# NeuroDiffGym/neurodiffeq

Measured on AMD Instinct MI355X. Metric: collocation-points/sec (residual+bwd), 2D Laplace 65k pts, 1/2/4/8 GPU, higher is better.
Workload: dtype f32; 1 GPU; C2: Solver2D 2D Laplace, DirichletBVP2D, FCNN(2-32-32-1, tanh), Generator2D 256x256 = 65536 noisy-grid points per GPU per step, Adam(1e-3), run_train_epoch() with n_batches_train=1, n_batches_valid=0; points_per_gpu=65536, global_batch=65536, parallelism=dp1 (shard-by-batch, one all-reduce of [P+1] fp32 per step), allreduce=none (single process), inputs=pre-sampled in the reference's RNG order, resident in HBM

## Files before the change

### include/ndq.h

```cpp
#ifndef NDQ_H
#define NDQ_H
#include <stddef.h>
#ifdef __cplusplus
extern "C" {
#endif

#define NDQ_EUNSUPPORTED (-1)
#define NDQ_EINVAL (-2)

#define NDQ_ACT_TANH 0
#define NDQ_ACT_SIN 1
#define NDQ_ACT_SIGMOID 2
#define NDQ_ACT_SWISH 3
#define NDQ_ACT_APTX 4
#define NDQ_ACT_ELU 5
#define NDQ_ACT_SOFTPLUS 6
#define NDQ_ACT_GELU 7

#define NDQ_MAX_HIDDEN 512
typedef struct ndq_mlp_desc {
  int d;
  int first;
  int mask2;
  int hidden;
  int layers;
  int act;
  int n_out;
  int lap;
  int skip;
  int mask3;
  int actp;
  int widths;
  int mono;
  int mask4;
} ndq_mlp_desc;

typedef struct ndq_mlp_kernels {
  ndq_mlp_desc desc;
  int n_streams, n_params;
  int bwd_waves;
  int lds_bytes;
  int (*fwd)(const float* coords, int ldc, int n, const float* params, float* jets, int ldj, void* stream);
  int (*bwd)(const float* coords, int ldc, int n, const float* params, const float* gbar, int ldj, float* partials,
             int blocks, void* stream);
} ndq_mlp_kernels;
int ndq_mlp_register(const ndq_mlp_kernels* kernels);

int ndq_mlp_supported(const ndq_mlp_desc* desc);
int ndq_mlp_num_streams(const ndq_mlp_desc* desc);
int ndq_mlp_num_params(const ndq_mlp_desc* desc);
int ndq_mlp_bwd_blocks(const ndq_mlp_desc* desc, int n);

int ndq_mlp_jet_fwd(const ndq_mlp_desc* desc, const float* coords, int ldc, int n, const float* params, float* jets,
                    int ldj, void* stream);

int ndq_mlp_jet_bwd(const ndq_mlp_desc* desc, const float* coords, int ldc, int n, const float* params,
                    const float* gbar, int ldj, float* partials, void* stream);

int ndq_reduce_partials(const float* partials, int nparts, int len, float* out, int accumulate, float scale,
                        void* stream);

int ndq_adam_step(float* params, const float* grad, float* exp_avg, float* exp_avg_sq, int len, float lr, float beta1,
                  float beta2, float eps, float weight_decay, int step, void* stream);

int ndq_reduce_grad_loss(const float* partials, int nparts, int len, float* out, int accumulate,
                         const float* loss_partials, int n_loss_parts, float* loss_out, float loss_scale, void* stream);

int ndq_epoch_tail(float* params, const float* grad, float* exp_avg, float* exp_avg_sq, int len, float lr, float beta1,
                   float beta2, float eps, float weight_decay, int step, const float* loss_slots, int n_batches,
                   float* loss_hist, int hist_index, float* best_loss, int parity, float* best_flat, int write_scalars,
                   void* stream);

#define NDQ_SAMPLE_UNIFORM 0
#define NDQ_SAMPLE_GRID 1
#define NDQ_SAMPLE_SPHERICAL 2
typedef struct ndq_sampler_desc {
  int kind;
  int d;
  int n[3];
  float lo[3], hi[3];
  float noise_std[3];
  int radial;
} ndq_sampler_desc;
int ndq_sample(const ndq_sampler_desc* desc, unsigned long long seed, unsigned long long draw, unsigned stream_id,
               float* coords, int ldc, void* stream);

#define NDQ_TABLE_MAX_AXES 6
#define NDQ_AXIS_NORMAL 0
#define NDQ_AXIS_CHEB2_NOISY 1
typedef struct ndq_table_sampler_desc {
  int d;
  int n[NDQ_TABLE_MAX_AXES];
  int law[NDQ_TABLE_MAX_AXES];
  int abs_value;
  const float* mean[NDQ_TABLE_MAX_AXES];
  const float* std[NDQ_TABLE_MAX_AXES];
  float lo[NDQ_TABLE_MAX_AXES], hi[NDQ_TABLE_MAX_AXES];
} ndq_table_sampler_desc;
int ndq_sample_table(const ndq_table_sampler_desc* desc, unsigned long long seed, unsigned long long draw,
                     unsigned stream_id, float* coords , int ldc, void* stream);

#define NDQ_PLAN_MAX_LEAVES 8
#define NDQ_LEAF_SIMPLE 0
#define NDQ_LEAF_TABLE 1
#define NDQ_LEAF_DATA 2
#define NDQ_SEG_LEAF 0
#define NDQ_SEG_ENSEMBLE 1
#define NDQ_SEG_MESH 2
typedef struct ndq_plan_leaf {
  int kind;
  int row0;
  int rows;
  int n;
  union {
    ndq_sampler_desc simple;
    ndq_table_sampler_desc table;
    const float* data[NDQ_TABLE_MAX_AXES];
  } u;
} ndq_plan_leaf;
typedef struct ndq_plan_segment {
  int mode;
  int first, count;
  int offset, size;
} ndq_plan_segment;
typedef struct ndq_plan_sampler_desc {
  int d;
  int n_leaves;
  int n_segments;
  int reserved;
  ndq_plan_leaf leaf[NDQ_PLAN_MAX_LEAVES];
  ndq_plan_segment seg[NDQ_PLAN_MAX_LEAVES];
} ndq_plan_sampler_desc;
int ndq_sample_plan(const ndq_plan_sampler_desc* desc, unsigned long long seed, unsigned long long draw,
                    unsigned stream_id, float* coords , int ldc, void* stream);

#define NDQ_INDEX_NONE 0
#define NDQ_INDEX_PERMUTE 1
#define NDQ_INDEX_REPLACE 2
typedef struct ndq_plan_index_desc {
  int mode;
  int m;
  int batch;
  int reserved;
} ndq_plan_index_desc;
int ndq_sample_plan_indexed(const ndq_plan_sampler_desc* desc, const ndq_plan_index_desc* index, unsigned long long seed,
                            unsigned long long draw, unsigned stream_id, float* coords , int ldc, void* stream);

typedef int (*ndq_fused_launch_fn)(const float* coords, int ldc, int n, const float* params, float* partials,
                                   float* loss_partials, float* funcs, float* resid, int ldj, float seed, int train,
                                   void* stream);

typedef int (*ndq_allreduce_fn)(const void* sendbuf, void* recvbuf, size_t count, int dtype, int op, void* comm,
                                void* stream);

typedef struct ndq_fused_step {
  ndq_fused_launch_fn launch;
  int n, ldc, ldj, blocks, n_params;
  float seed;
  float* params;
  float* partials;
  float* loss_partials;
  float* grad;
  float* loss_slot;
  float* adam_m;
  float* adam_v;
  float lr, beta1, beta2, eps, weight_decay;
  float* loss_hist;
  float* best_loss;
  float* best_flat;
  ndq_allreduce_fn allreduce;
  void* comm;
  const struct ndq_sampler_desc* next_sampler;
  unsigned long long next_seed, next_draw;
  unsigned next_stream;
  float* next_coords;
  int next_ldc;
} ndq_fused_step;
int ndq_fused_step_run(const ndq_fused_step* s, const float* coords, int adam_step, int hist_index, int parity,
                       void* stream);

typedef int (*ndq_fused_launch_multi_fn)(const float* coords, int ldc, int n, const float* const* params,
                                         float* const* partials, float* loss_partials, float* funcs, float* resid,
                                         int ldj, float seed, int train, void* stream);
int ndq_fused_multi_step_run(const ndq_fused_step* steps, int n_nets, ndq_fused_launch_multi_fn launch,
                             const float* coords, int adam_step, int hist_index, int parity, void* stream);

typedef int (*ndq_fused_launch_tv_fn)(const float* coords, int ldc, int n, const float* const* params,
                                      float* const* partials, float* loss_partials, float seed,
                                      const float* valid_coords, int valid_ldc, int valid_n,
                                      float* valid_loss_partials, const void* pull, void* stream);
typedef int (*ndq_fused_launch_loop_fn)(const float* coords, int ldc, int n, float seed, const float* vcoords, int vldc,
                                        int vn, const void* loop, void* stream);
typedef struct ndq_fused_fit {
  ndq_fused_launch_tv_fn launch;
  int n_nets;
  ndq_fused_step net[4];
  const float* valid_coords;
  int valid_n, valid_ldc, valid_blocks;
  float valid_scale;
  float* valid_loss_partials;
  float* valid_hist;
  int track_best;
  int pull_ok;
  float* alt_params[4];
  float* alt_m[4];
  float* alt_v[4];
  float* alt_partials[4];
  float* alt_loss_partials;
  float* alt_valid_loss_partials;
  ndq_fused_launch_loop_fn launch_loop;
  int loop_ok;
} ndq_fused_fit;
int ndq_fused_fit_run(const ndq_fused_fit* f, int n_epochs, const float* const* train_coords, int adam_step,
                      int hist_index, int valid_index, int parity, void* stream);

typedef int (*ndq_pointwise_fn)(const float* coords, int ldc, int n, const float* const* jets,
                                float* const* gbar, int ldj, float* funcs, float* resid, float* loss_partials,
                                float seed_scale, void* stream);
typedef int (*ndq_pw_blocks_fn)(int n);
typedef void (*ndq_bind_theta_fn)(const float* theta, float* theta_partials);

typedef struct ndq64_mlp_kernels {
  ndq_mlp_desc desc;
  int n_streams, n_params;
  int bwd_waves;
  int lds_bytes;
  int (*fwd)(const double* coords, int ldc, int n, const double* params, double* jets, int ldj, void* stream);
  int (*bwd)(const double* coords, int ldc, int n, const double* params, const double* gbar, int ldj, double* partials,
             int blocks, void* stream);
} ndq64_mlp_kernels;
int ndq64_mlp_register(const ndq64_mlp_kernels* kernels);
int ndq64_mlp_supported(const ndq_mlp_desc* desc);
int ndq64_mlp_num_streams(const ndq_mlp_desc* desc);
int ndq64_mlp_num_params(const ndq_mlp_desc* desc);
int ndq64_mlp_bwd_blocks(const ndq_mlp_desc* desc, int n);
int ndq64_mlp_jet_fwd(const ndq_mlp_desc* desc, const double* coords, int ldc, int n, const double* params, double* jets,
                      int ldj, void* stream);
int ndq64_mlp_jet_bwd(const ndq_mlp_desc* desc, const double* coords, int ldc, int n, const double* params,
                      const double* gbar, int ldj, double* partials, void* stream);
int ndq64_reduce_partials(const double* partials, int nparts, int len, double* out, int accumulate, double scale,
                          void* stream);
int ndq64_adam_step(double* params, const double* grad, double* exp_avg, double* exp_avg_sq, int len, double lr,
                    double beta1, double beta2, double eps, double weight_decay, int step, void* stream);

int ndq64_epoch_tail(double* params, const double* grad, double* exp_avg, double* exp_avg_sq, int len, double lr,
                     double beta1, double beta2, double eps, double weight_decay, int step, const double* loss_slots,
                     int n_batches, double* loss_hist, int hist_index, double* best_loss, int parity, double* best_flat,
                     int write_scalars, void* stream);

typedef int (*ndq64_fused_launch_multi_fn)(const double* coords, int ldc, int n, const double* const* params,
                                           double* const* partials, double* loss_partials, double* funcs, double* resid,
                                           int ldj, double seed, int train, void* stream);
typedef struct ndq64_fused_step {
  int n, ldc, ldj, blocks, n_params;
  double seed;
  double* params;
  double* partials;
  double* loss_partials;
  double* grad;
  double* loss_slot;
  double* adam_m;
  double* adam_v;
  double lr, beta1, beta2, eps, weight_decay;
  double* loss_hist;
  double* best_loss;
  double* best_flat;
} ndq64_fused_step;
int ndq64_fused_step_bytes(void);
int ndq64_reduce_tail(const ndq64_fused_step* steps, int n_nets, int adam_step, int hist_index, int parity, void* stream);
int ndq64_fused_step_run(const ndq64_fused_step* steps, int n_nets, ndq64_fused_launch_multi_fn launch,
                         const double* coords, int adam_step, int hist_index, int parity, void* stream);

int ndq_oneshot_create(int rank, int world_size, int max_len, void** ctx, unsigned char* handle64);
int ndq_oneshot_connect(void* ctx, const unsigned char* handles);
int ndq_oneshot_allreduce(const void* send, void* recv, size_t count, int dtype, int op, void* ctx, void* stream);
int ndq_oneshot_status(void* ctx);
int ndq_oneshot_destroy(void* ctx);

#ifdef __cplusplus
}
#endif
#endif
```

### neurodiffeq_amd/_build.py

```python
import os

from . import _hipcc

HERE = os.path.dirname(os.path.abspath(__file__))
CSRC = os.path.join(HERE, "csrc")
LIB = os.path.join(HERE, "libndq.so")
SOURCES = [os.path.join(CSRC, "ndq_api.hip")]
HEADERS = [os.path.join(CSRC, h) for h in ("ndq_mlp.h", "ndq_tail.h", "ndq_launch.h", "ndq_wide.h", "ndq_deep.h", "ndq_sample.h", "ndq_oneshot.h")] + \
    [os.path.join(HERE, "..", "include", "ndq.h"), os.path.join(HERE, "_hipcc.py")]
LIB64 = os.path.join(HERE, "libndq64.so")
SOURCES64 = [os.path.join(CSRC, "ndq_api64.hip")]
FLAGS = []
_EXTRA = os.environ.get("NDQ_LIB_FLAGS", "").split()
if _EXTRA:
    import hashlib
    LIB = os.path.join(HERE, "libndq_" + hashlib.sha1(" ".join(_EXTRA).encode()).hexdigest()[:8] + ".so")
    FLAGS = FLAGS + _EXTRA


def is_stale():
    if not os.path.exists(LIB):
        return True
    t = os.path.getmtime(LIB)
    return any(os.path.exists(p) and os.path.getmtime(p) > t for p in SOURCES + HEADERS)


def build_lib(force=False, verbose=False):
    if not force and not is_stale():
        return LIB
    _hipcc.compile_shared(SOURCES, LIB, FLAGS, verbose=verbose)
    return LIB


def is_stale64():
    if not os.path.exists(LIB64):
        return True
    t = os.path.getmtime(LIB64)
    return any(os.path.exists(p) and os.path.getmtime(p) > t for p in SOURCES64 + HEADERS)


def build_lib64(force=False, verbose=False):
    if not force and not is_stale64():
        return LIB64
    _hipcc.compile_shared(SOURCES64, LIB64, [], verbose=verbose)
    return LIB64


if __name__ == "__main__":
    print(build_lib(force=True, verbose=True))
```

### neurodiffeq_amd/_lib.py

```python
import ctypes
import os

from . import _build

NDQ_ACT_TANH, NDQ_ACT_SIN, NDQ_ACT_SIGMOID, NDQ_ACT_SWISH, NDQ_ACT_APTX = 0, 1, 2, 3, 4
NDQ_ACT_ELU, NDQ_ACT_SOFTPLUS, NDQ_ACT_GELU = 5, 6, 7


class MlpDesc(ctypes.Structure):
    _fields_ = [("d", ctypes.c_int), ("first", ctypes.c_int), ("mask2", ctypes.c_int), ("hidden", ctypes.c_int),
                ("layers", ctypes.c_int), ("act", ctypes.c_int), ("n_out", ctypes.c_int), ("lap", ctypes.c_int),
                ("skip", ctypes.c_int), ("mask3", ctypes.c_int), ("actp", ctypes.c_int), ("widths", ctypes.c_int), ("mono", ctypes.c_int),
                ("mask4", ctypes.c_int)]

    def key(self):
        return (self.d, self.first, self.mask2, self.hidden, self.layers, self.act, self.n_out, self.lap, self.skip,
                self.mask3, self.actp, self.widths, self.mono, self.mask4)


NDQ_SAMPLE_UNIFORM, NDQ_SAMPLE_GRID, NDQ_SAMPLE_SPHERICAL = 0, 1, 2


class SamplerDesc(ctypes.Structure):
    _fields_ = [("kind", ctypes.c_int), ("d", ctypes.c_int), ("n", ctypes.c_int * 3), ("lo", ctypes.c_float * 3),
                ("hi", ctypes.c_float * 3), ("noise_std", ctypes.c_float * 3), ("radial", ctypes.c_int)]


NDQ_TABLE_MAX_AXES = 6
NDQ_AXIS_NORMAL, NDQ_AXIS_CHEB2_NOISY = 0, 1


class TableSamplerDesc(ctypes.Structure):
    _fields_ = [("d", ctypes.c_int), ("n", ctypes.c_int * 6), ("law", ctypes.c_int * 6), ("abs_value", ctypes.c_int),
                ("mean", ctypes.c_void_p * 6), ("std", ctypes.c_void_p * 6), ("lo", ctypes.c_float * 6),
                ("hi", ctypes.c_float * 6)]


NDQ_PLAN_MAX_LEAVES = 8
NDQ_LEAF_SIMPLE, NDQ_LEAF_TABLE, NDQ_LEAF_DATA = 0, 1, 2
NDQ_SEG_LEAF, NDQ_SEG_ENSEMBLE, NDQ_SEG_MESH = 0, 1, 2
NDQ_INDEX_NONE, NDQ_INDEX_PERMUTE, NDQ_INDEX_REPLACE = 0, 1, 2


class _PlanLaw(ctypes.Union):
    _fields_ = [("simple", SamplerDesc), ("table", TableSamplerDesc), ("data", ctypes.c_void_p * 6)]


class PlanLeaf(ctypes.Structure):
    _fields_ = [("kind", ctypes.c_int), ("row0", ctypes.c_int), ("rows", ctypes.c_int), ("n", ctypes.c_int), ("u", _PlanLaw)]


class PlanSegment(ctypes.Structure):
    _fields_ = [("mode", ctypes.c_int), ("first", ctypes.c_int), ("count", ctypes.c_int), ("offset", ctypes.c_int),
                ("size", ctypes.c_int)]


class PlanSamplerDesc(ctypes.Structure):
    _fields_ = [("d", ctypes.c_int), ("n_leaves", ctypes.c_int), ("n_segments", ctypes.c_int), ("reserved", ctypes.c_int),
                ("leaf", PlanLeaf * 8), ("seg", PlanSegment * 8)]


class PlanIndexDesc(ctypes.Structure):
    _fields_ = [("mode", ctypes.c_int), ("m", ctypes.c_int), ("batch", ctypes.c_int), ("reserved", ctypes.c_int)]


FUSED_LAUNCH_FN = ctypes.CFUNCTYPE(ctypes.c_int, ctypes.c_void_p, ctypes.c_int, ctypes.c_int, ctypes.c_void_p,
                                   ctypes.c_void_p, ctypes.c_void_p, ctypes.c_void_p, ctypes.c_void_p, ctypes.c_int,
                                   ctypes.c_float, ctypes.c_int, ctypes.c_void_p)


class FusedStep(ctypes.Structure):
    _fields_ = [("launch", ctypes.c_void_p),
                ("n", ctypes.c_int), ("ldc", ctypes.c_int), ("ldj", ctypes.c_int), ("blocks", ctypes.c_int),
                ("n_params", ctypes.c_int), ("seed", ctypes.c_float),
                ("params", ctypes.c_void_p), ("partials", ctypes.c_void_p), ("loss_partials", ctypes.c_void_p),
                ("grad", ctypes.c_void_p), ("loss_slot", ctypes.c_void_p), ("adam_m", ctypes.c_void_p),
                ("adam_v", ctypes.c_void_p),
                ("lr", ctypes.c_float), ("beta1", ctypes.c_float), ("beta2", ctypes.c_float), ("eps", ctypes.c_float),
                ("weight_decay", ctypes.c_float),
                ("loss_hist", ctypes.c_void_p), ("best_loss", ctypes.c_void_p), ("best_flat", ctypes.c_void_p),
                ("allreduce", ctypes.c_void_p), ("comm", ctypes.c_void_p),
                ("next_sampler", ctypes.c_void_p), ("next_seed", ctypes.c_ulonglong), ("next_draw", ctypes.c_ulonglong),
                ("next_stream", ctypes.c_uint), ("next_coords", ctypes.c_void_p), ("next_ldc", ctypes.c_int)]


class FusedStep64(ctypes.Structure):
    _fields_ = [("n", ctypes.c_int), ("ldc", ctypes.c_int), ("ldj", ctypes.c_int), ("blocks", ctypes.c_int),
                ("n_params", ctypes.c_int), ("seed", ctypes.c_double),
                ("params", ctypes.c_void_p), ("partials", ctypes.c_void_p), ("loss_partials", ctypes.c_void_p),
                ("grad", ctypes.c_void_p), ("loss_slot", ctypes.c_void_p), ("adam_m", ctypes.c_void_p),
                ("adam_v", ctypes.c_void_p),
                ("lr", ctypes.c_double), ("beta1", ctypes.c_double), ("beta2", ctypes.c_double), ("eps", ctypes.c_double),
                ("weight_decay", ctypes.c_double),
                ("loss_hist", ctypes.c_void_p), ("best_loss", ctypes.c_void_p), ("best_flat", ctypes.c_void_p)]


class FusedFit(ctypes.Structure):
    _fields_ = [("launch", ctypes.c_void_p), ("n_nets", ctypes.c_int), ("net", FusedStep * 4),
                ("valid_coords", ctypes.c_void_p), ("valid_n", ctypes.c_int), ("valid_ldc", ctypes.c_int),
                ("valid_blocks", ctypes.c_int), ("valid_scale", ctypes.c_float),
                ("valid_loss_partials", ctypes.c_void_p), ("valid_hist", ctypes.c_void_p), ("track_best", ctypes.c_int),
                ("pull_ok", ctypes.c_int), ("alt_params", ctypes.c_void_p * 4), ("alt_m", ctypes.c_void_p * 4),
                ("alt_v", ctypes.c_void_p * 4), ("alt_partials", ctypes.c_void_p * 4),
                ("alt_loss_partials", ctypes.c_void_p), ("alt_valid_loss_partials", ctypes.c_void_p),
                ("launch_loop", ctypes.c_void_p), ("loop_ok", ctypes.c_int)]


class NdqError(RuntimeError):
    pass


_LIB = None


def lib():
    global _LIB
    if _LIB is not None:
        return _LIB
    path = _build.LIB
    if _build.is_stale():
        try:
            _build.build_lib()
        except Exception as e:
            if not os.path.exists(path):
                raise NdqError(f"libndq.so is missing and could not be built: {e}") from e
    L = ctypes.CDLL(path)
    vp, ci, cf = ctypes.c_void_p, ctypes.c_int, ctypes.c_float
    dp = ctypes.POINTER(MlpDesc)
    L.ndq_mlp_supported.argtypes = [dp]
    L.ndq_mlp_num_streams.argtypes = [dp]
    L.ndq_mlp_num_params.argtypes = [dp]
    L.ndq_mlp_bwd_blocks.argtypes = [dp, ci]
    L.ndq_mlp_jet_fwd.argtypes = [dp, vp, ci, ci, vp, vp, ci, vp]
    L.ndq_mlp_jet_bwd.argtypes = [dp, vp, ci, ci, vp, vp, ci, vp, vp]
    L.ndq_reduce_partials.argtypes = [vp, ci, ci, vp, ci, cf, vp]
    L.ndq_adam_step.argtypes = [vp, vp, vp, vp, ci, cf, cf, cf, cf, cf, ci, vp]
    L.ndq_reduce_grad_loss.argtypes = [vp, ci, ci, vp, ci, vp, ci, vp, cf, vp]
    L.ndq_epoch_tail.argtypes = [vp, vp, vp, vp, ci, cf, cf, cf, cf, cf, ci, vp, ci, vp, ci, vp, ci, vp, ci, vp]
    L.ndq_fused_step_run.argtypes = [ctypes.POINTER(FusedStep), vp, ci, ci, ci, vp]
    L.ndq_fused_multi_step_run.argtypes = [ctypes.POINTER(FusedStep), ci, vp, vp, ci, ci, ci, vp]
    L.ndq_fused_fit_run.argtypes = [ctypes.POINTER(FusedFit), ci, vp, ci, ci, ci, ci, vp]
    L.ndq_mlp_register.argtypes = [vp]
    L.ndq_sample.argtypes = [ctypes.POINTER(SamplerDesc), ctypes.c_ulonglong, ctypes.c_ulonglong, ctypes.c_uint, vp, ci, vp]
    L.ndq_sample_table.argtypes = [ctypes.POINTER(TableSamplerDesc), ctypes.c_ulonglong, ctypes.c_ulonglong, ctypes.c_uint, vp, ci,
                                   vp]
    L.ndq_sample_plan.argtypes = [ctypes.POINTER(PlanSamplerDesc), ctypes.c_ulonglong, ctypes.c_ulonglong, ctypes.c_uint, vp, ci, vp]
    L.ndq_sample_plan_indexed.argtypes = [ctypes.POINTER(PlanSamplerDesc), ctypes.POINTER(PlanIndexDesc), ctypes.c_ulonglong,
                                          ctypes.c_ulonglong, ctypes.c_uint, vp, ci, vp]
    L.ndq_oneshot_create.argtypes = [ci, ci, ci, ctypes.POINTER(vp), ctypes.c_char_p]
    L.ndq_oneshot_connect.argtypes = [vp, ctypes.c_char_p]
    L.ndq_oneshot_allreduce.argtypes = [vp, vp, ctypes.c_size_t, ci, ci, vp, vp]
    L.ndq_oneshot_status.argtypes = [vp]
    L.ndq_oneshot_destroy.argtypes = [vp]
    for name in ("ndq_mlp_supported", "ndq_mlp_num_streams", "ndq_mlp_num_params", "ndq_mlp_bwd_blocks",
                 "ndq_mlp_jet_fwd", "ndq_mlp_jet_bwd", "ndq_reduce_partials", "ndq_adam_step", "ndq_reduce_grad_loss",
                 "ndq_epoch_tail", "ndq_fused_step_run", "ndq_sample", "ndq_sample_table", "ndq_sample_plan", "ndq_sample_plan_indexed", "ndq_mlp_register",
                 "ndq_fused_multi_step_run", "ndq_fused_fit_run", "ndq_oneshot_create", "ndq_oneshot_connect",
                 "ndq_oneshot_allreduce", "ndq_oneshot_status",
                 "ndq_oneshot_destroy"):
        getattr(L, name).restype = ci
    _LIB = L
    return L


_LIB64 = None


def lib64():
    global _LIB64
    if _LIB64 is not None:
        return _LIB64
    if _build.is_stale64():
        try:
            _build.build_lib64()
        except Exception as e:
            if not os.path.exists(_build.LIB64):
                raise NdqError(f"libndq64.so is missing and could not be built: {e}") from e
    L = ctypes.CDLL(_build.LIB64)
    vp, ci = ctypes.c_void_p, ctypes.c_int
    dp = ctypes.POINTER(MlpDesc)
    L.ndq64_mlp_supported.argtypes = [dp]
    L.ndq64_mlp_num_streams.argtypes = [dp]
    L.ndq64_mlp_num_params.argtypes = [dp]
    L.ndq64_mlp_bwd_blocks.argtypes = [dp, ci]
    L.ndq64_mlp_jet_fwd.argtypes = [dp, vp, ci, ci, vp, vp, ci, vp]
    L.ndq64_mlp_jet_bwd.argtypes = [dp, vp, ci, ci, vp, vp, ci, vp, vp]
    L.ndq64_reduce_partials.argtypes = [vp, ci, ci, vp, ci, ctypes.c_double, vp]
    L.ndq64_mlp_register.argtypes = [vp]
    cd = ctypes.c_double
    L.ndq64_adam_step.argtypes = [vp, vp, vp, vp, ci, cd, cd, cd, cd, cd, ci, vp]
    L.ndq64_epoch_tail.argtypes = [vp, vp, vp, vp, ci, cd, cd, cd, cd, cd, ci, vp, ci, vp, ci, vp, ci, vp, ci, vp]
    L.ndq64_fused_step_bytes.argtypes = []
    L.ndq64_reduce_tail.argtypes = [ctypes.POINTER(FusedStep64), ci, ci, ci, ci, vp]
    L.ndq64_fused_step_run.argtypes = [ctypes.POINTER(FusedStep64), ci, vp, vp, ci, ci, ci, vp]
    for name in EXPORTS64:
        getattr(L, name).restype = ci
    _LIB64 = L
    return L


EXPORTS64 = ("ndq64_mlp_register", "ndq64_mlp_supported", "ndq64_mlp_num_streams", "ndq64_mlp_num_params",
             "ndq64_mlp_bwd_blocks", "ndq64_mlp_jet_fwd", "ndq64_mlp_jet_bwd", "ndq64_reduce_partials", "ndq64_adam_step",
             "ndq64_epoch_tail", "ndq64_fused_step_bytes", "ndq64_reduce_tail", "ndq64_fused_step_run")

EXPORTS = ("ndq_mlp_supported", "ndq_mlp_num_streams", "ndq_mlp_num_params", "ndq_mlp_bwd_blocks", "ndq_mlp_jet_fwd",
           "ndq_mlp_jet_bwd", "ndq_reduce_partials", "ndq_adam_step", "ndq_reduce_grad_loss", "ndq_epoch_tail",
           "ndq_fused_step_run", "ndq_sample", "ndq_sample_table", "ndq_sample_plan", "ndq_sample_plan_indexed", "ndq_mlp_register",
           "ndq_fused_multi_step_run", "ndq_fused_fit_run", "ndq_oneshot_create", "ndq_oneshot_connect", "ndq_oneshot_allreduce", "ndq_oneshot_status",
           "ndq_oneshot_destroy")


def check(rc, what):
    if rc != 0:
        raise NdqError(f"{what} failed with code {rc}" + (" (no kernel for this descriptor)" if rc == -1 else ""))
```

### neurodiffeq_amd/csrc/ndq_api.hip

```cpp
#include <cstdlib>
#include <vector>
#include "ndq_launch.h"
#include "ndq_sample.h"
#include "ndq_oneshot.h"
#include "ndq_tail.h"

extern "C" int ndq_oneshot_allreduce(const void* send, void* recv, size_t count, int dtype, int op, void* comm, void* stream);

namespace ndq {

#ifndef NDQ_CFG_TABLE
#define NDQ_CFG_TABLE(X)      \
  X(1, 0, 0, 2, 2, ACT_SIN, 1, 0)   \
  X(1, 1, 0, 2, 2, ACT_SIN, 1, 0)   \
  X(1, 1, 1, 2, 2, ACT_SIN, 1, 0)   \
  X(1, 0, 0, 2, 2, ACT_TANH, 1, 0)  \
  X(1, 1, 0, 2, 2, ACT_TANH, 1, 0)  \
  X(1, 1, 1, 2, 2, ACT_TANH, 1, 0)  \
  X(2, 0, 0, 2, 2, ACT_TANH, 1, 0)  \
  X(2, 1, 0, 2, 2, ACT_TANH, 1, 0)  \
  X(2, 1, 1, 2, 2, ACT_TANH, 1, 0)  \
  X(2, 1, 5, 2, 2, ACT_TANH, 1, 0)  \
  X(2, 1, 7, 2, 2, ACT_TANH, 1, 0)  \
  X(2, 0, 0, 4, 3, ACT_TANH, 1, 0)  \
  X(2, 1, 0, 4, 3, ACT_TANH, 1, 0)  \
  X(2, 1, 1, 4, 3, ACT_TANH, 1, 0)  \
  X(2, 1, 5, 4, 3, ACT_TANH, 1, 0)  \
  X(1, 0, 0, 2, 2, ACT_TANH, 25, 0) \
  X(1, 1, 1, 2, 2, ACT_TANH, 25, 0) \
  X(2, 1, 5, 2, 2, ACT_TANH, 3, 0)  \
  X(2, 1, 5, 2, 2, ACT_TANH, 1, 1)  \
  X(2, 1, 5, 4, 3, ACT_TANH, 1, 1)  \
  X(3, 0, 0, 2, 2, ACT_TANH, 1, 0)  \
  X(3, 1, 0, 2, 2, ACT_TANH, 1, 0)  \
  X(3, 1, 1, 2, 2, ACT_TANH, 1, 0)  \
  X(3, 1, 41, 2, 2, ACT_TANH, 1, 0) \
  X(3, 1, 41, 2, 2, ACT_TANH, 1, 1) \
  X(3, 1, 63, 2, 2, ACT_TANH, 1, 0)  \
  X(1, 0, 0, 2, 2, ACT_SIGMOID, 1, 0) \
  X(1, 1, 0, 2, 2, ACT_SIGMOID, 1, 0) \
  X(1, 1, 1, 2, 2, ACT_SIGMOID, 1, 0) \
  X(2, 0, 0, 2, 2, ACT_SIGMOID, 1, 0) \
  X(2, 1, 0, 2, 2, ACT_SIGMOID, 1, 0) \
  X(2, 1, 1, 2, 2, ACT_SIGMOID, 1, 0) \
  X(2, 1, 5, 2, 2, ACT_SIGMOID, 1, 0) \
  X(2, 1, 7, 2, 2, ACT_SIGMOID, 1, 0) \
  X(2, 1, 5, 2, 2, ACT_SIGMOID, 1, 1) \
  X(1, 0, 0, 2, 2, ACT_SWISH, 1, 0) \
  X(1, 1, 0, 2, 2, ACT_SWISH, 1, 0) \
  X(1, 1, 1, 2, 2, ACT_SWISH, 1, 0) \
  X(2, 0, 0, 2, 2, ACT_SWISH, 1, 0) \
  X(2, 1, 0, 2, 2, ACT_SWISH, 1, 0) \
  X(2, 1, 1, 2, 2, ACT_SWISH, 1, 0) \
  X(2, 1, 5, 2, 2, ACT_SWISH, 1, 0) \
  X(2, 1, 7, 2, 2, ACT_SWISH, 1, 0) \
  X(2, 1, 5, 2, 2, ACT_SWISH, 1, 1)
#endif

#define NDQ_ENTRY(D, F, M, NB, L, A, O, LP) make_kernels<Cfg<D, F, M, NB, L, A, O, LP>>(),

static const ndq_mlp_kernels kTable[] = {NDQ_CFG_TABLE(NDQ_ENTRY)};
static std::vector<const ndq_mlp_kernels*> g_registered;

static const ndq_mlp_kernels* find(const ndq_mlp_desc* d) {
  if (!d || d->hidden < 1 || d->hidden > NDQ_MAX_HIDDEN) return nullptr;
  for (const ndq_mlp_kernels& e : kTable)
    if (same_desc(e.desc, *d)) return &e;
  for (const ndq_mlp_kernels* e : g_registered)
    if (same_desc(e->desc, *d)) return e;
  return nullptr;
}

__global__ __launch_bounds__(256) void reduce_partials_kernel(const float* __restrict__ part, int nparts, int len,
                                                              float* __restrict__ out, int accumulate, float scale) {
  const int i = blockIdx.x * blockDim.x + threadIdx.x;
  if (i >= len) return;
  double s0 = 0., s1 = 0., s2 = 0., s3 = 0.;
  int r = 0;
#pragma unroll 4
  for (; r + 3 < nparts; r += 4) {
    s0 += (double)part[(size_t)r * len + i];
    s1 += (double)part[(size_t)(r + 1) * len + i];
    s2 += (double)part[(size_t)(r + 2) * len + i];
    s3 += (double)part[(size_t)(r + 3) * len + i];
  }
  for (; r < nparts; ++r) s0 += (double)part[(size_t)r * len + i];
  const float s = (float)(((s0 + s1) + (s2 + s3)) * (double)scale);
  out[i] = accumulate ? out[i] + s : s;
}

struct Reduce2Args {
  const float* part; int nparts, len; float* out; int accumulate;
  const float* lpart; int nlparts; float* lout; float lscale;
};

struct ColumnRows {
  float v[16];
  __device__ __forceinline__ void issue(const float* __restrict__ part, int nparts, int len, int col, int rg) {
    const int cc = col < len ? col : len - 1;
#pragma unroll
    for (int j = 0; j < 16; ++j) {
      const int r = rg + 16 * j;
      v[j] = part[(size_t)(r < nparts ? r : nparts - 1) * len + cc];
    }
  }
  __device__ __forceinline__ float finish(const float* __restrict__ part, int nparts, int len, int col, int rg) const {
    float x[16];
#pragma unroll
    for (int j = 0; j < 16; ++j) x[j] = v[j];
    asm volatile("" : "+v"(x[0]), "+v"(x[1]), "+v"(x[2]), "+v"(x[3]), "+v"(x[4]), "+v"(x[5]), "+v"(x[6]), "+v"(x[7]), "+v"(x[8]),
                      "+v"(x[9]), "+v"(x[10]), "+v"(x[11]), "+v"(x[12]), "+v"(x[13]), "+v"(x[14]), "+v"(x[15]));
#pragma unroll
    for (int j = 0; j < 16; ++j) x[j] = (rg + 16 * j < nparts && col < len) ? x[j] : 0.f;
    float s0 = 0.f, s1 = 0.f, s2 = 0.f, s3 = 0.f;
#pragma unroll
    for (int it = 0; it < 4; ++it) {
      if (rg + 64 * it + 48 < nparts) { s0 += x[4 * it]; s1 += x[4 * it + 1]; s2 += x[4 * it + 2]; s3 += x[4 * it + 3]; }
      else { s0 += x[4 * it]; s0 += x[4 * it + 1]; s0 += x[4 * it + 2]; s0 += x[4 * it + 3]; }
    }
    if (nparts > 256 && col < len) {
      int r = rg + 256;
      for (; r + 48 < nparts; r += 64) {
        s0 += part[(size_t)r * len + col];
        s1 += part[(size_t)(r + 16) * len + col];
        s2 += part[(size_t)(r + 32) * len + col];
        s3 += part[(size_t)(r + 48) * len + col];
      }
      for (; r < nparts; r += 16) s0 += part[(size_t)r * len + col];
    }
    return (s0 + s1) + (s2 + s3);
  }
};

__device__ __forceinline__ float column_sum_1024(const float* __restrict__ part, int nparts, int len, int col, int rg,
                                                 float* sm ) {
  ColumnRows rows;
  rows.issue(part, nparts, len, col, rg);
  sm[rg * 64 + (threadIdx.x & 63)] = rows.finish(part, nparts, len, col, rg);
  __syncthreads();
  float s = 0.f;
  if (rg == 0) {
#pragma unroll
    for (int g = 0; g < 16; ++g) s += sm[g * 64 + (threadIdx.x & 63)];
  }
  return s;
}

__device__ __forceinline__ float block_sum_1024(const float* __restrict__ v, int n, float* sm16) {
  float x = 0.f;
  for (int r = threadIdx.x; r < n; r += 1024) x += v[r];
  for (int off = 32; off > 0; off >>= 1) x += __shfl_down(x, off);
  if ((threadIdx.x & 63) == 0) sm16[threadIdx.x >> 6] = x;
  __syncthreads();
  float s = 0.f;
  if (threadIdx.x == 0)
    for (int w = 0; w < 16; ++w) s += sm16[w];
  return s;
}

__global__ __launch_bounds__(1024) void reduce_grad_loss_kernel(Reduce2Args a) {
  __shared__ float sm[16 * 64];
  if (blockIdx.x + 1 < gridDim.x) {
    const int c = threadIdx.x & 63, rg = threadIdx.x >> 6;
    const int i = blockIdx.x * 64 + c;
    const float s = column_sum_1024(a.part, a.nparts, a.len, i, rg, sm);
    if (rg == 0 && i < a.len) a.out[i] = a.accumulate ? a.out[i] + s : s;
  } else {
    const float s = block_sum_1024(a.lpart, a.nlparts, sm);
    if (threadIdx.x == 0) *a.lout = s * a.lscale;
  }
}

using TailArgs = ndq::TailArgsT<float>;

struct ValidArgs {
  const float* part; int nparts; float scale; float* hist; int index;
  int best_on_valid;
};
struct ReduceTailArgs {
  Reduce2Args r;
  TailArgs t;
  int tail_blocks;
  ndq::SampleArgs smp;
  ValidArgs v;
};
#ifndef NDQ_TAIL_COLS
#define NDQ_TAIL_COLS 64
#endif
template <int TC>
__device__ __forceinline__ void reduce_tail_body(const ReduceTailArgs& a) {
  constexpr int TT = TC * 16, WAVES = TT / 64;
  __shared__ float sm[16 * TC];
  __shared__ float smw[16];
  __shared__ float smv[16];
  const int tid = threadIdx.x, c = tid % TC, rg = tid / TC, lane = tid & 63, wave = tid >> 6;
  const int i = blockIdx.x * TC + c;
  const bool col = i < a.r.len;
  const bool has_valid = a.v.part != nullptr;
  const bool has_train = a.r.nparts > 0;
  ColumnRows rows;
  if (has_train) rows.issue(a.r.part, a.r.nparts, a.r.len, i, rg);
  const float lp0 = tid < a.r.nlparts ? a.r.lpart[tid] : 0.f;
  const float vp0 = has_valid && tid < a.v.nparts ? a.v.part[tid] : 0.f;
  const bool upd = (rg == 0) && col;
  const float* p_in = a.t.p_in ? a.t.p_in : a.t.p;
  const float* m_in = a.t.m_in ? a.t.m_in : a.t.m;
  const float* v_in = a.t.v_in ? a.t.v_in : a.t.v;
  float pi = 0.f, m0 = 0.f, v0 = 0.f;
  if (upd) {
    pi = p_in[i];
    if (has_train || a.t.p_in) { m0 = m_in[i]; v0 = v_in[i]; }
  }
  const float best = a.t.best_loss[a.t.parity];
  float lp = lp0, vp = vp0;
  for (int r = tid + TT; r < a.r.nlparts; r += TT) lp += a.r.lpart[r];
  if (has_valid)
    for (int r = tid + TT; r < a.v.nparts; r += TT) vp += a.v.part[r];
  const float colsum = has_train ? rows.finish(a.r.part, a.r.nparts, a.r.len, i, rg) : 0.f;
  for (int off = 32; off > 0; off >>= 1) lp += __shfl_down(lp, off);
  if (has_valid)
    for (int off = 32; off > 0; off >>= 1) vp += __shfl_down(vp, off);
  if (lane == 0) { smw[wave] = lp; smv[wave] = vp; }
  sm[rg * TC + c] = colsum;
  __syncthreads();
  float loss = 0.f, vloss = 0.f;
#pragma unroll
  for (int w = 0; w < WAVES; ++w) loss += smw[w];
  loss *= a.r.lscale;
  if (has_valid) {
#pragma unroll
    for (int w = 0; w < WAVES; ++w) vloss += smv[w];
    vloss *= a.v.scale;
  }
  const bool on_valid = has_valid && a.v.best_on_valid != 0;
  const float cmp = on_valid ? vloss : loss;
  const bool better = (a.t.best_flat != nullptr) && (on_valid || has_train) && (cmp < best);
  if (upd) {
    if (better) a.t.best_flat[i] = pi;
    if (has_train) {
      float g = 0.f;
#pragma unroll
      for (int k = 0; k < 16; ++k) g += sm[k * TC + c];
      a.r.out[i] = g;
      float pn, mi, vi;
      ndq::adam_value(a.t.adam, pi, g, m0, v0, pn, mi, vi);
      a.t.m[i] = mi;
      a.t.v[i] = vi;
      a.t.p[i] = pn;
    } else if (a.t.p_in) {
      a.t.p[i] = pi; a.t.m[i] = m0; a.t.v[i] = v0;
    }
  }
  if (blockIdx.x == 0 && tid == 0 && a.t.write_scalars) {
    if (has_train) {
      *a.r.lout = loss;
      a.t.loss_hist[a.t.hist_index] = loss;
    }
    if (has_valid) a.v.hist[a.v.index] = vloss;
    a.t.best_loss[a.t.parity ^ 1] = better ? cmp : best;
  }
}
__global__ __launch_bounds__(1024) void reduce_tail_kernel(ReduceTailArgs a) {
  if ((int)blockIdx.x >= a.tail_blocks) {
    ndq::sample_point_store(a.smp, ((int)blockIdx.x - a.tail_blocks) * 1024 + (int)threadIdx.x);
    return;
  }
  reduce_tail_body<64>(a);
}

__global__ __launch_bounds__(1024) void reduce_tail_dp_kernel(ReduceTailArgs a, ndq::OneshotDev c, unsigned step) {
  __shared__ float sm[16 * 64];
  __shared__ float smw[16];
  __shared__ float sloss;
  __shared__ int timed_out;
  if (threadIdx.x == 0) timed_out = 0;
  const int tid = threadIdx.x, col = tid & 63, rg = tid >> 6, blk = blockIdx.x;
  const int i = blk * 64 + col;
  const bool incol = i < a.r.len;
  ColumnRows rows;
  rows.issue(a.r.part, a.r.nparts, a.r.len, i, rg);
  const float lp0 = tid < a.r.nlparts ? a.r.lpart[tid] : 0.f;
  const bool upd = (rg == 0) && incol;
  float pi = 0.f, m0 = 0.f, v0 = 0.f;
  if (upd) { pi = a.t.p[i]; m0 = a.t.m[i]; v0 = a.t.v[i]; }
  const float best = a.t.best_loss[a.t.parity];
  float lp = lp0;
  for (int r = tid + 1024; r < a.r.nlparts; r += 1024) lp += a.r.lpart[r];
  const float colsum = rows.finish(a.r.part, a.r.nparts, a.r.len, i, rg);
  for (int off = 32; off > 0; off >>= 1) lp += __shfl_down(lp, off);
  if (col == 0) smw[rg] = lp;
  sm[rg * 64 + col] = colsum;
  __syncthreads();
  const int parity = step & 1u;
  const size_t slot = ((size_t)parity * c.world + c.rank) * c.max_len + (size_t)blk * 65;
  if (rg == 0) {
    float g = 0.f;
#pragma unroll
    for (int k = 0; k < 16; ++k) g += sm[k * 64 + col];
    for (int q = 0; q < c.world; ++q)
      __hip_atomic_store(c.inbox[q] + slot + col, incol ? g : 0.f, __ATOMIC_RELAXED, __HIP_MEMORY_SCOPE_SYSTEM);
    if (col == 0) {
      float loss = 0.f;
#pragma unroll
      for (int w = 0; w < 16; ++w) loss += smw[w];
      loss *= a.r.lscale;
      for (int q = 0; q < c.world; ++q)
        __hip_atomic_store(c.inbox[q] + slot + 64, loss, __ATOMIC_RELAXED, __HIP_MEMORY_SCOPE_SYSTEM);
    }
  }
  __threadfence_system();
  __syncthreads();
  if (tid < c.world) {
    unsigned* f = c.flags[tid] + ((size_t)parity * c.world + c.rank) * c.max_blocks + blk;
    __hip_atomic_store(f, step, __ATOMIC_RELEASE, __HIP_MEMORY_SCOPE_SYSTEM);
    const unsigned* mine = c.flags[c.rank] + ((size_t)parity * c.world + tid) * c.max_blocks + blk;
    if (!ndq::oneshot_wait(mine, step, c.spin_limit, c.status)) timed_out = 1;
  }
  __syncthreads();
  const bool bad = timed_out != 0;
  const float* inbox = c.inbox[c.rank] + (size_t)parity * c.world * c.max_len + (size_t)blk * 65;
  if (tid == 0) {
    float loss = 0.f;
    for (int q = 0; q < c.world; ++q)
      loss += __hip_atomic_load(inbox + (size_t)q * c.max_len + 64, __ATOMIC_RELAXED, __HIP_MEMORY_SCOPE_SYSTEM);
    sloss = bad ? __builtin_nanf("") : loss;
  }
  __syncthreads();
  const float loss = sloss;
  const bool better = (a.t.best_flat != nullptr) && (loss < best);
  if (upd && !bad) {
    float g = 0.f;
    for (int q = 0; q < c.world; ++q)
      g += __hip_atomic_load(inbox + (size_t)q * c.max_len + col, __ATOMIC_RELAXED, __HIP_MEMORY_SCOPE_SYSTEM);
    a.r.out[i] = g;
    if (better) a.t.best_flat[i] = pi;
    float pn, mi, vi;
    ndq::adam_value(a.t.adam, pi, g, m0, v0, pn, mi, vi);
    a.t.m[i] = mi;
    a.t.v[i] = vi;
    a.t.p[i] = pn;
  }
  if (blk == 0 && tid == 0 && a.t.write_scalars) {
    *a.r.lout = loss;
    a.t.loss_hist[a.t.hist_index] = loss;
    a.t.best_loss[a.t.parity ^ 1] = better ? loss : best;
  }
}

struct ReduceTailMultiArgs {
  ReduceTailArgs net[4];
};
template <int TC>
__global__ __launch_bounds__(TC * 16) void reduce_tail_multi_kernel(ReduceTailMultiArgs a) {
  const ReduceTailArgs& mine = a.net[blockIdx.y];
  if ((int)blockIdx.x * TC >= mine.r.len) return;
  reduce_tail_body<TC>(mine);
}
static int launch_tail_multi(ReduceTailMultiArgs& a, int max_params, int n_nets, int max_lparts, void* stream) {
  hipStream_t st = static_cast<hipStream_t>(stream);
  for (int k = n_nets; k < 4; ++k) a.net[k] = a.net[0];
  if (NDQ_TAIL_COLS < 64 && max_lparts <= NDQ_TAIL_COLS * 16)
    hipLaunchKernelGGL(reduce_tail_multi_kernel<NDQ_TAIL_COLS>, dim3((max_params + NDQ_TAIL_COLS - 1) / NDQ_TAIL_COLS, n_nets),
                       dim3(NDQ_TAIL_COLS * 16), 0, st, a);
  else
    hipLaunchKernelGGL(reduce_tail_multi_kernel<64>, dim3((max_params + 63) / 64, n_nets), dim3(1024), 0, st, a);
  return (int)hipGetLastError();
}

}

using namespace ndq;

extern "C" {

int ndq_mlp_supported(const ndq_mlp_desc* desc) { return find(desc) ? 1 : 0; }

int ndq_mlp_register(const ndq_mlp_kernels* k) {
  if (!k || !k->fwd || !k->bwd || k->desc.hidden < 1 || k->desc.hidden > NDQ_MAX_HIDDEN || k->n_streams < 1 || k->n_params < 1 || k->bwd_waves < 1 ||
      k->lds_bytes > 160 * 1024)
    return NDQ_EINVAL;
  if (!find(&k->desc)) g_registered.push_back(k);
  return 0;
}

int ndq_mlp_num_streams(const ndq_mlp_desc* desc) {
  const ndq_mlp_kernels* e = find(desc);
  return e ? e->n_streams : NDQ_EUNSUPPORTED;
}

int ndq_mlp_num_params(const ndq_mlp_desc* desc) {
  const ndq_mlp_kernels* e = find(desc);
  return e ? e->n_params : NDQ_EUNSUPPORTED;
}

int ndq_mlp_bwd_blocks(const ndq_mlp_desc* desc, int n) {
  const ndq_mlp_kernels* e = find(desc);
  if (!e) return NDQ_EUNSUPPORTED;
  if (n <= 0) return NDQ_EINVAL;
  return bwd_blocks(e->bwd_waves, n);
}

int ndq_mlp_jet_fwd(const ndq_mlp_desc* desc, const float* coords, int ldc, int n, const float* params, float* jets,
                    int ldj, void* stream) {
  const ndq_mlp_kernels* e = find(desc);
  if (!e) return NDQ_EUNSUPPORTED;
  if (!coords || !params || !jets || n <= 0 || ldc < n || ldj < n) return NDQ_EINVAL;
  return e->fwd(coords, ldc, n, params, jets, ldj, stream);
}

int ndq_mlp_jet_bwd(const ndq_mlp_desc* desc, const float* coords, int ldc, int n, const float* params,
                    const float* gbar, int ldj, float* partials, void* stream) {
  const ndq_mlp_kernels* e = find(desc);
  if (!e) return NDQ_EUNSUPPORTED;
  if (!coords || !params || !gbar || !partials || n <= 0 || ldc < n || ldj < n) return NDQ_EINVAL;
  return e->bwd(coords, ldc, n, params, gbar, ldj, partials, bwd_blocks(e->bwd_waves, n), stream);
}

int ndq_reduce_partials(const float* partials, int nparts, int len, float* out, int accumulate, float scale,
                        void* stream) {
  if (!partials || !out || nparts <= 0 || len <= 0) return NDQ_EINVAL;
  hipLaunchKernelGGL(reduce_partials_kernel, dim3((len + 255) / 256), dim3(256), 0, static_cast<hipStream_t>(stream),
                     partials, nparts, len, out, accumulate, scale);
  return (int)hipGetLastError();
}

int ndq_reduce_grad_loss(const float* partials, int nparts, int len, float* out, int accumulate,
                         const float* loss_partials, int n_loss_parts, float* loss_out, float loss_scale, void* stream) {
  if (!partials || !out || !loss_partials || !loss_out || nparts <= 0 || len <= 0 || n_loss_parts <= 0) return NDQ_EINVAL;
  Reduce2Args a{partials, nparts, len, out, accumulate, loss_partials, n_loss_parts, loss_out, loss_scale};
  hipLaunchKernelGGL(reduce_grad_loss_kernel, dim3((len + 63) / 64 + 1), dim3(1024), 0, static_cast<hipStream_t>(stream), a);
  return (int)hipGetLastError();
}

int ndq_epoch_tail(float* params, const float* grad, float* exp_avg, float* exp_avg_sq, int len, float lr, float beta1,
                   float beta2, float eps, float weight_decay, int step, const float* loss_slots, int n_batches,
                   float* loss_hist, int hist_index, float* best_loss, int parity, float* best_flat, int write_scalars,
                   void* stream) {
  const bool adam = exp_avg != nullptr;
  if (!params || len <= 0 || !loss_slots || n_batches <= 0 || !loss_hist || !best_loss || hist_index < 0 ||
      (parity != 0 && parity != 1) || (adam && (!grad || !exp_avg_sq || step <= 0)))
    return NDQ_EINVAL;
  TailArgs a{};
  a.p = params; a.g = grad; a.m = exp_avg; a.v = exp_avg_sq; a.len = len;
  a.adam = adam_consts(lr, beta1, beta2, eps, weight_decay, adam ? step : 0);
  a.loss_slots = loss_slots; a.nb = n_batches; a.loss_hist = loss_hist; a.hist_index = hist_index;
  a.best_loss = best_loss; a.parity = parity; a.best_flat = best_flat; a.write_scalars = write_scalars;
  hipLaunchKernelGGL(epoch_tail_kernel<float>, dim3((len + 255) / 256), dim3(256), 0, static_cast<hipStream_t>(stream), a);
  return (int)hipGetLastError();
}

}

static ReduceTailArgs reduce_tail_args(const ndq_fused_step& s, const ndq_fused_step& s0, const float* part, const float* lpart,
                                       int nparts, int adam_step, int hist_index, int parity, int write_scalars,
                                       float* best_flat, const ValidArgs& v = ValidArgs{}, const float* p_in = nullptr,
                                       const float* m_in = nullptr, const float* v_in = nullptr) {
  ReduceTailArgs a{};
  a.r = Reduce2Args{part, nparts, s.n_params, s.grad, 0, lpart, nparts, s.loss_slot, s0.seed};
  a.t.p = s.params; a.t.g = s.grad; a.t.m = s.adam_m; a.t.v = s.adam_v; a.t.len = s.n_params;
  a.t.adam = adam_consts(s.lr, s.beta1, s.beta2, s.eps, s.weight_decay, adam_step);
  a.t.p_in = p_in; a.t.m_in = m_in; a.t.v_in = v_in;
  a.t.loss_slots = s.loss_slot; a.t.nb = 1; a.t.loss_hist = s0.loss_hist; a.t.hist_index = hist_index;
  a.t.best_loss = s0.best_loss; a.t.parity = parity; a.t.best_flat = best_flat; a.t.write_scalars = write_scalars;
  a.tail_blocks = 0x7fffffff;
  a.v = v;
  return a;
}

extern "C" {

int ndq_fused_step_run(const ndq_fused_step* s, const float* coords, int adam_step, int hist_index, int parity,
                       void* stream) {
  if (!s || !s->launch || !coords) return NDQ_EINVAL;
  int rc = s->launch(coords, s->ldc, s->n, s->params, s->partials, s->loss_partials, nullptr, nullptr, s->ldj, s->seed,
                     1, stream);
  if (rc) return rc;
  if (!s->adam_m)
    return ndq_reduce_grad_loss(s->partials, s->blocks, s->n_params, s->grad, 0, s->loss_partials, s->blocks,
                                s->loss_slot, s->seed, stream);
  if (adam_step <= 0 || hist_index < 0 || (parity != 0 && parity != 1) || !s->loss_hist || !s->best_loss) return NDQ_EINVAL;
  const bool oneshot = s->allreduce == reinterpret_cast<ndq_allreduce_fn>(&ndq_oneshot_allreduce) && s->comm &&
                       ((s->n_params + 63) / 64) * 65 <= static_cast<ndq::Oneshot*>(s->comm)->dev.max_len &&
                       (s->n_params + 63) / 64 <= static_cast<ndq::Oneshot*>(s->comm)->dev.max_blocks;
  if (s->allreduce && !oneshot) {
    if (s->loss_slot != s->grad + s->n_params) return NDQ_EINVAL;
    rc = ndq_reduce_grad_loss(s->partials, s->blocks, s->n_params, s->grad, 0, s->loss_partials, s->blocks, s->loss_slot,
                              s->seed, stream);
    if (rc) return rc;
    rc = s->allreduce(s->grad, s->grad, (size_t)s->n_params + 1,  7,  0, s->comm, stream);
    if (rc) return 1000 + rc;
    return ndq_epoch_tail(s->params, s->grad, s->adam_m, s->adam_v, s->n_params, s->lr, s->beta1, s->beta2, s->eps,
                          s->weight_decay, adam_step, s->loss_slot, 1, s->loss_hist, hist_index, s->best_loss, parity,
                          s->best_flat, 1, stream);
  }
  ReduceTailArgs a = reduce_tail_args(*s, *s, s->partials, s->loss_partials, s->blocks, adam_step, hist_index, parity, 1,
                                      s->best_flat);
  int blocks = (s->n_params + 63) / 64;
  if (oneshot) {
    ndq::Oneshot* c = static_cast<ndq::Oneshot*>(s->comm);
    const unsigned step = ++c->step;
    hipLaunchKernelGGL(reduce_tail_dp_kernel, dim3(blocks), dim3(1024), 0, static_cast<hipStream_t>(stream), a, c->dev, step);
    return (int)hipGetLastError();
  }
  a.tail_blocks = blocks;
  if (s->next_sampler) {
    rc = ndq::fill_sample_args(a.smp, s->next_sampler, s->next_seed, s->next_draw, s->next_stream, s->next_coords,
                               s->next_ldc);
    if (rc) return rc;
    blocks += (a.smp.total + 1023) / 1024;
  }
  hipLaunchKernelGGL(reduce_tail_kernel, dim3(blocks), dim3(1024), 0, static_cast<hipStream_t>(stream), a);
  return (int)hipGetLastError();
}

int ndq_fused_multi_step_run(const ndq_fused_step* steps, int n_nets, ndq_fused_launch_multi_fn launch,
                             const float* coords, int adam_step, int hist_index, int parity, void* stream) {
  if (!steps || !launch || !coords || n_nets < 1 || n_nets > 4 || adam_step <= 0 || hist_index < 0 ||
      (parity != 0 && parity != 1))
    return NDQ_EINVAL;
  const ndq_fused_step& s0 = steps[0];
  if (!s0.loss_hist || !s0.best_loss || !s0.loss_partials) return NDQ_EINVAL;
  const float* params[4];
  float* partials[4];
  for (int k = 0; k < n_nets; ++k) {
    if (!steps[k].params || !steps[k].partials || !steps[k].grad || !steps[k].adam_m || !steps[k].adam_v ||
        !steps[k].loss_slot)
      return NDQ_EINVAL;
    params[k] = steps[k].params;
    partials[k] = steps[k].partials;
  }
  int rc = launch(coords, s0.ldc, s0.n, params, partials, s0.loss_partials, nullptr, nullptr, s0.ldj, s0.seed, 1, stream);
  if (rc) return rc;
  ReduceTailMultiArgs a{};
  int max_params = 0;
  for (int k = 0; k < n_nets; ++k) {
    a.net[k] = reduce_tail_args(steps[k], s0, steps[k].partials, s0.loss_partials, s0.blocks, adam_step, hist_index, parity,
                                k == 0 ? 1 : 0, steps[k].best_flat);
    if (steps[k].n_params > max_params) max_params = steps[k].n_params;
  }
  return launch_tail_multi(a, max_params, n_nets, s0.blocks, stream);
}

}

struct FitCall {
  const ndq_fused_fit* f;
  int n_epochs; const float* const* train_coords;
  int adam_step, hist_index, valid_index;
  void* stream;
  bool valid;
  int max_params, max_lparts;
  float* P[2][4]; float* M[2][4]; float* V[2][4]; float* PART[2][4]; float* LP[2]; float* VP[2];
};

static bool fit_tracks(const ndq_fused_fit* f, bool with_train, bool with_valid) {
  return (f->track_best == 1 && with_train) || (f->track_best == 2 && with_valid);
}

static int fit_tail(const FitCall& c, int set, bool with_train, bool with_valid, int adam_step, int hist_index, int vindex,
                    int parity) {
  const ndq_fused_fit* f = c.f;
  const ndq_fused_step& s0 = f->net[0];
  ValidArgs v{};
  if (with_valid) v = ValidArgs{c.VP[set], f->valid_blocks, f->valid_scale, f->valid_hist, vindex, f->track_best == 2 ? 1 : 0};
  const bool track = fit_tracks(f, with_train, with_valid);
  ReduceTailMultiArgs a{};
  for (int k = 0; k < f->n_nets; ++k) {
    const ndq_fused_step& s = f->net[k];
    a.net[k] = reduce_tail_args(s, s0, c.PART[set][k], c.LP[set], with_train ? s0.blocks : 0, with_train ? adam_step : 0,
                                hist_index, parity, k == 0 ? 1 : 0, track ? s.best_flat : nullptr, v,
                                set ? c.P[set][k] : nullptr, set ? c.M[set][k] : nullptr, set ? c.V[set][k] : nullptr);
  }
  return launch_tail_multi(a, c.max_params, f->n_nets, c.max_lparts, c.stream);
}

static int fit_two_launch(const FitCall& c, int parity) {
  const ndq_fused_fit* f = c.f;
  const ndq_fused_step& s0 = f->net[0];
  for (int e = 0; e < c.n_epochs; ++e, parity ^= 1) {
    if (!c.train_coords[e]) return NDQ_EINVAL;
    const bool with_valid = c.valid && e > 0;
    int rc = f->launch(c.train_coords[e], s0.ldc, s0.n, c.P[0], c.PART[0], c.LP[0], s0.seed,
                       with_valid ? f->valid_coords : nullptr, f->valid_ldc, with_valid ? f->valid_n : 0, c.VP[0], nullptr,
                       c.stream);
    if (rc) return rc;
    rc = fit_tail(c, 0, true, with_valid, c.adam_step + e, c.hist_index + e, c.valid_index + e - 1, parity);
    if (rc) return rc;
  }
  if (!c.valid) return 0;
  int rc = f->launch(nullptr, 0, 0, c.P[0], nullptr, nullptr, 0.f, f->valid_coords, f->valid_ldc, f->valid_n, c.VP[0], nullptr,
                     c.stream);
  if (rc) return rc;
  return fit_tail(c, 0, false, true, 0, c.hist_index + c.n_epochs, c.valid_index + (c.n_epochs > 0 ? c.n_epochs - 1 : 0), parity);
}

struct Finishes { int adam_step, hist_index, valid_index; bool with_valid; };
static Finishes launch_finishes(const FitCall& c, int e) {
  const int j = e - 1;
  return {c.adam_step + j, c.hist_index + j, c.valid_index + j - 1, c.valid && j >= 1};
}
static int fit_last_launch(const FitCall& c) { return c.valid ? c.n_epochs : c.n_epochs - 1; }

static int fit_closing_tail(const FitCall& c, int fin, int parity) {
  const Finishes w = launch_finishes(c, fit_last_launch(c) + 1);
  return fit_tail(c, fin, !c.valid, c.valid, w.adam_step, w.hist_index, w.valid_index, parity);
}

static int fit_pull(const FitCall& c, int parity) {
  const ndq_fused_fit* f = c.f;
  const ndq_fused_step& s0 = f->net[0];
  const int last = fit_last_launch(c);
  for (int e = 0; e <= last; ++e) {
    ndq::PullArgs pa{};
    if (e >= 1) {
      const Finishes w = launch_finishes(c, e);
      const int in = (e - 1) & 1, out = e & 1;
      pa.enabled = 1; pa.n_nets = f->n_nets; pa.nparts = s0.blocks;
      pa.lpart = c.LP[in]; pa.nlparts = s0.blocks; pa.lscale = s0.seed;
      pa.loss_hist = s0.loss_hist; pa.hist_index = w.hist_index; pa.loss_slot = s0.loss_slot;
      pa.vpart = w.with_valid ? c.VP[in] : nullptr; pa.nvparts = f->valid_blocks; pa.vscale = f->valid_scale;
      pa.valid_hist = f->valid_hist; pa.valid_index = w.valid_index; pa.best_on_valid = f->track_best == 2 ? 1 : 0;
      pa.best_loss = s0.best_loss; pa.parity = parity;
      const bool track = fit_tracks(f, true, w.with_valid);
      for (int k = 0; k < f->n_nets; ++k) {
        const ndq_fused_step& s = f->net[k];
        ndq::PullNet& n = pa.net[k];
        n.part = c.PART[in][k];
        n.p_in = c.P[in][k]; n.m_in = c.M[in][k]; n.v_in = c.V[in][k];
        n.p_out = c.P[out][k]; n.m_out = c.M[out][k]; n.v_out = c.V[out][k];
        n.grad = s.grad; n.best_flat = track ? s.best_flat : nullptr; n.len = s.n_params;
        n.adam = adam_consts(s.lr, s.beta1, s.beta2, s.eps, s.weight_decay, w.adam_step);
      }
      parity ^= 1;
    }
    const bool train_part = e < c.n_epochs, valid_part = c.valid && e >= 1;
    if (train_part && !c.train_coords[e]) return NDQ_EINVAL;
    int rc = f->launch(train_part ? c.train_coords[e] : nullptr, s0.ldc, train_part ? s0.n : 0, c.P[e & 1],
                       train_part ? c.PART[e & 1] : nullptr, c.LP[e & 1], s0.seed, valid_part ? f->valid_coords : nullptr,
                       f->valid_ldc, valid_part ? f->valid_n : 0, c.VP[e & 1], &pa, c.stream);
    if (rc) return rc;
  }
  return fit_closing_tail(c, last & 1, parity);
}

static int fit_loop(const FitCall& c, long long stride, int parity) {
  const ndq_fused_fit* f = c.f;
  const ndq_fused_step& s0 = f->net[0];
  const int last = fit_last_launch(c);
  int in = 0;
  for (int e0 = 0; e0 <= last; e0 += ndq::kLoopMaxLaunches, in ^= 1) {
    const int e1 = e0 + ndq::kLoopMaxLaunches <= last + 1 ? e0 + ndq::kLoopMaxLaunches : last + 1;
    const int out = in ^ 1;
    ndq::LoopArgs L{};
    L.e0 = e0; L.e1 = e1; L.n_epochs = c.n_epochs; L.has_valid = c.valid ? 1 : 0; L.track_best = f->track_best;
    L.hist_index = c.hist_index; L.valid_index = c.valid_index; L.parity = parity; L.coord_stride = stride;
    L.lp_in = c.LP[in]; L.vp_in = c.VP[in]; L.lp_out = c.LP[out]; L.vp_out = c.VP[out];
    L.lscale = s0.seed; L.vscale = f->valid_scale;
    L.loss_hist = s0.loss_hist; L.loss_slot = s0.loss_slot; L.valid_hist = f->valid_hist; L.best_loss = s0.best_loss;
    for (int k = 0; k < f->n_nets; ++k) {
      const ndq_fused_step& s = f->net[k];
      ndq::LoopNet& n = L.net[k];
      n.p_in = c.P[in][k]; n.m_in = c.M[in][k]; n.v_in = c.V[in][k]; n.part_in = c.PART[in][k];
      n.p_out = c.P[out][k]; n.m_out = c.M[out][k]; n.v_out = c.V[out][k]; n.part_out = c.PART[out][k];
      n.grad = s.grad; n.best_flat = s.best_flat;
      n.lr = s.lr; n.b1 = s.beta1; n.b2 = s.beta2; n.eps = s.eps; n.wd = s.weight_decay;
      for (int e = e0 > 1 ? e0 : 1; e < e1; ++e) {
        const ndq::AdamConsts a = adam_consts(s.lr, s.beta1, s.beta2, s.eps, s.weight_decay, launch_finishes(c, e).adam_step);
        n.bc1[e - e0] = a.bc1; n.bc2s[e - e0] = a.bc2s;
      }
    }
    int rc = f->launch_loop(c.train_coords[0], s0.ldc, s0.n, s0.seed, c.valid ? f->valid_coords : nullptr, f->valid_ldc,
                            c.valid ? f->valid_n : 0, &L, c.stream);
    if (rc) return rc;
  }
  return fit_closing_tail(c, in, parity ^ (last & 1));
}

extern "C" {

int ndq_fused_fit_run(const ndq_fused_fit* f, int n_epochs, const float* const* train_coords, int adam_step,
                      int hist_index, int valid_index, int parity, void* stream) {
  if (!f || !f->launch || f->n_nets < 1 || f->n_nets > 4 || n_epochs < 0 || (n_epochs > 0 && (!train_coords || adam_step <= 0)) ||
      hist_index < 0 || valid_index < 0 || (parity != 0 && parity != 1) || f->track_best < 0 || f->track_best > 2)
    return NDQ_EINVAL;
  const ndq_fused_step& s0 = f->net[0];
  const bool valid = f->valid_coords != nullptr;
  if (!valid && n_epochs == 0) return NDQ_EINVAL;
  if (!s0.best_loss || (n_epochs > 0 && (!s0.loss_hist || !s0.loss_partials || s0.n <= 0 || s0.blocks <= 0))) return NDQ_EINVAL;
  if (valid && (!f->valid_loss_partials || !f->valid_hist || f->valid_n <= 0 || f->valid_blocks <= 0)) return NDQ_EINVAL;
  if (f->track_best == 2 && !valid) return NDQ_EINVAL;
  FitCall c{f, n_epochs, train_coords, adam_step, hist_index, valid_index, stream, valid};
  c.max_lparts = s0.blocks > f->valid_blocks ? s0.blocks : f->valid_blocks;
  c.LP[0] = s0.loss_partials; c.LP[1] = f->alt_loss_partials;
  c.VP[0] = f->valid_loss_partials; c.VP[1] = f->alt_valid_loss_partials;
  bool pull = f->pull_ok != 0 && n_epochs >= 2 && s0.blocks * f->n_nets <= ndq::kPullMaxWork && f->alt_loss_partials &&
              (!valid || f->alt_valid_loss_partials);
  for (int k = 0; k < f->n_nets; ++k) {
    const ndq_fused_step& s = f->net[k];
    if (!s.params || s.n_params <= 0 || (f->track_best && !s.best_flat)) return NDQ_EINVAL;
    if (n_epochs > 0 && (!s.partials || !s.grad || !s.adam_m || !s.adam_v || !s.loss_slot)) return NDQ_EINVAL;
    if (s.n_params > c.max_params) c.max_params = s.n_params;
    c.P[0][k] = s.params; c.M[0][k] = s.adam_m; c.V[0][k] = s.adam_v; c.PART[0][k] = s.partials;
    c.P[1][k] = f->alt_params[k]; c.M[1][k] = f->alt_m[k]; c.V[1][k] = f->alt_v[k]; c.PART[1][k] = f->alt_partials[k];
    pull = pull && c.P[1][k] && c.M[1][k] && c.V[1][k] && c.PART[1][k];
  }
  if (!pull) return fit_two_launch(c, parity);
  bool loop = f->loop_ok != 0 && f->launch_loop && s0.blocks == 1 && (!valid || f->valid_blocks == 1) &&
              f->n_nets <= ndq::kLoopMaxNets;
  long long stride = 0;
  if (loop) {
    if (!train_coords[0] || !train_coords[1]) return NDQ_EINVAL;
    stride = train_coords[1] - train_coords[0];
    for (int e = 2; e < n_epochs && loop; ++e) {
      if (!train_coords[e]) return NDQ_EINVAL;
      loop = train_coords[e] - train_coords[0] == stride * e;
    }
  }
  return loop ? fit_loop(c, stride, parity) : fit_pull(c, parity);
}

int ndq_adam_step(float* params, const float* grad, float* exp_avg, float* exp_avg_sq, int len, float lr, float beta1,
                  float beta2, float eps, float weight_decay, int step, void* stream) {
  if (!params || !grad || !exp_avg || !exp_avg_sq || len <= 0 || step <= 0) return NDQ_EINVAL;
  hipLaunchKernelGGL(adam_kernel<float>, dim3((len + 255) / 256), dim3(256), 0, static_cast<hipStream_t>(stream), params, grad,
                     exp_avg, exp_avg_sq, len, adam_consts(lr, beta1, beta2, eps, weight_decay, step));
  return (int)hipGetLastError();
}

int ndq_sample(const ndq_sampler_desc* desc, unsigned long long seed, unsigned long long draw, unsigned stream_id,
               float* coords, int ldc, void* stream) {
  return ndq::launch_sample(desc, seed, draw, stream_id, coords, ldc, (hipStream_t)stream);
}

int ndq_sample_table(const ndq_table_sampler_desc* desc, unsigned long long seed, unsigned long long draw,
                     unsigned stream_id, float* coords, int ldc, void* stream) {
  return ndq::launch_sample_table(desc, seed, draw, stream_id, coords, ldc, (hipStream_t)stream);
}

int ndq_sample_plan(const ndq_plan_sampler_desc* desc, unsigned long long seed, unsigned long long draw,
                    unsigned stream_id, float* coords, int ldc, void* stream) {
  return ndq::launch_sample_plan(desc, seed, draw, stream_id, coords, ldc, (hipStream_t)stream);
}

int ndq_sample_plan_indexed(const ndq_plan_sampler_desc* desc, const ndq_plan_index_desc* index, unsigned long long seed,
                            unsigned long long draw, unsigned stream_id, float* coords, int ldc, void* stream) {
  return ndq::launch_sample_plan_indexed(desc, index, seed, draw, stream_id, coords, ldc, (hipStream_t)stream);
}

}

extern "C" {

int ndq_oneshot_create(int rank, int world, int max_len, void** out, unsigned char* handle64) {
  if (!out || !handle64 || world < 1 || world > ndq::kOneshotMaxRanks || rank < 0 || rank >= world || max_len < 1)
    return NDQ_EINVAL;
  ndq::Oneshot* c = new (std::nothrow) ndq::Oneshot();
  if (!c) return NDQ_EINVAL;
  std::memset(c, 0, sizeof(*c));
  int max_blocks = 0;
  const size_t bytes = ndq::oneshot_layout(world, max_len, &c->inbox_bytes, &c->flag_bytes, &max_blocks);
  hipError_t e = hipExtMallocWithFlags(&c->base, bytes, hipDeviceMallocUncached);
  if (e != hipSuccess) e = hipExtMallocWithFlags(&c->base, bytes, hipDeviceMallocFinegrained);
  if (e != hipSuccess) { delete c; return (int)e; }
  e = hipMemset(c->base, 0, bytes);
  if (e == hipSuccess) e = hipDeviceSynchronize();
  hipIpcMemHandle_t h;
  if (e == hipSuccess) e = hipIpcGetMemHandle(&h, c->base);
  if (e != hipSuccess) { (void)hipFree(c->base); delete c; return (int)e; }
  static_assert(sizeof(hipIpcMemHandle_t) == 64, "HIP IPC handles are 64 bytes");
  std::memcpy(handle64, &h, 64);
  c->dev.rank = rank; c->dev.world = world; c->dev.max_len = max_len; c->dev.max_blocks = max_blocks;
  c->dev.spin_limit = ndq::kOneshotSpinLimit;
  if (const char* e = std::getenv("NDQ_ONESHOT_SPIN_LIMIT")) c->dev.spin_limit = std::strtoull(e, nullptr, 10);
  c->dev.status = reinterpret_cast<unsigned*>(static_cast<char*>(c->base) + c->inbox_bytes + c->flag_bytes);
  c->step = 0;
  *out = c;
  return 0;
}

int ndq_oneshot_connect(void* ctx, const unsigned char* handles) {
  ndq::Oneshot* c = static_cast<ndq::Oneshot*>(ctx);
  if (!c || !handles) return NDQ_EINVAL;
  for (int q = 0; q < c->dev.world; ++q) {
    void* p = c->base;
    if (q != c->dev.rank) {
      hipIpcMemHandle_t h;
      std::memcpy(&h, handles + 64 * q, 64);
      hipError_t e = hipIpcOpenMemHandle(&p, h, hipIpcMemLazyEnablePeerAccess);
      if (e != hipSuccess) return (int)e;
      c->peer_base[q] = p;
    }
    c->dev.inbox[q] = static_cast<float*>(p);
    c->dev.flags[q] = reinterpret_cast<unsigned*>(static_cast<char*>(p) + c->inbox_bytes);
  }
  return 0;
}

int ndq_oneshot_allreduce(const void* send, void* recv, size_t count, int dtype, int op, void* comm, void* stream) {
  ndq::Oneshot* c = static_cast<ndq::Oneshot*>(comm);
  if (!c || !send || !recv || dtype != 7 || op != 0 || count == 0 || (long)count > c->dev.max_len) return NDQ_EINVAL;
  const unsigned step = ++c->step;
  const int blocks = ((int)count + ndq::kOneshotChunk - 1) / ndq::kOneshotChunk;
  hipLaunchKernelGGL(ndq::oneshot_allreduce_kernel, dim3(blocks), dim3(1024), 0, static_cast<hipStream_t>(stream), c->dev,
                     static_cast<const float*>(send), static_cast<float*>(recv), (int)count, step);
  return (int)hipGetLastError();
}

int ndq_oneshot_status(void* ctx) {
  ndq::Oneshot* c = static_cast<ndq::Oneshot*>(ctx);
  if (!c) return NDQ_EINVAL;
  unsigned v = 0;
  if (hipDeviceSynchronize() != hipSuccess) return -1;
  if (hipMemcpy(&v, c->dev.status, sizeof(v), hipMemcpyDeviceToHost) != hipSuccess) return -1;
  return (int)v;
}

int ndq_oneshot_destroy(void* ctx) {
  ndq::Oneshot* c = static_cast<ndq::Oneshot*>(ctx);
  if (!c) return NDQ_EINVAL;
  (void)hipDeviceSynchronize();
  for (int q = 0; q < c->dev.world; ++q)
    if (q != c->dev.rank && c->peer_base[q]) (void)hipIpcCloseMemHandle(c->peer_base[q]);
  (void)hipFree(c->base);
  delete c;
  return 0;
}

}
```

### neurodiffeq_amd/engine.py

```python
import ctypes
import functools
import os

import torch

from . import _lib, codegen, generators
from .networks import FlatParams, describe
from .symbolic import Graph, Sym, TraceUnsupported, trace_scope

_c_vp = ctypes.c_void_p


def _ptr(t):
    return _c_vp(t.data_ptr())


_raw_stream = getattr(torch._C, "_cuda_getCurrentRawStream", None) or \
    (lambda idx: torch.cuda.current_stream(idx).cuda_stream)


def _round_up(n, m):
    return (n + m - 1) // m * m


class _Lib64:

    def __init__(self):
        self._lib = _lib.lib64()

    def __getattr__(self, name):
        return getattr(self._lib, name.replace("ndq_", "ndq64_", 1))


def _ends(c):
    n = c.numel()
    if n == 0:
        return ()
    if c.is_contiguous():
        p, e = c.data_ptr(), c.element_size()
        return (ctypes.string_at(p, e), ctypes.string_at(p + (n - 1) * e, e))
    f = c.detach().reshape(-1)
    return (f[0].item(), f[-1].item())


class library_code:
    __slots__ = ("ctx",)

    def __enter__(self):
        self.ctx = torch._C.DisableTorchFunction() if torch._C._len_torch_function_stack() else None
        if self.ctx is not None:
            self.ctx.__enter__()
        return self

    def __exit__(self, *exc):
        if self.ctx is not None:
            self.ctx.__exit__(*exc)
            self.ctx = None
        return False

    def user_code(self):
        return _UserCode(self)


class _UserCode:
    __slots__ = ("lc", "was")

    def __init__(self, lc):
        self.lc = lc

    def __enter__(self):
        self.was = self.lc.ctx is not None
        if self.was:
            self.lc.ctx.__exit__(None, None, None)
            self.lc.ctx = None

    def __exit__(self, *exc):
        if self.was:
            self.lc.ctx = torch._C.DisableTorchFunction()
            self.lc.ctx.__enter__()
        return False


def trace_system(nets, conditions, diff_eqs, n_coords, compute_func_val=None, loss="l2", metrics=(), f64=False,
                 volatile=frozenset()):
    L = _Lib64() if f64 else _lib.lib()
    all_nets, conditions = list(nets), list(conditions)
    nets = []
    for n in all_nets:
        if not any(n is m for m in nets):
            nets.append(n)
    from .networks import track_structure
    for n in nets:
        track_structure(n)
    infos = [describe(n, dtype=torch.float64 if f64 else torch.float32) for n in nets]
    if any(i is None for i in infos):
        raise TraceUnsupported("a network is not an FCNN the gfx950 kernels support")
    g = Graph(n_coords)
    g.f64 = bool(f64)
    g.volatile = frozenset() if f64 else frozenset(volatile)
    if f64 and any(i.get("skip_sym") is not None for i in infos):
        raise TraceUnsupported("a skip connection above 64 hidden units on the fp64 pipeline (its weights are kernel arguments: fp32 only)")
    g.register_nets(nets, [i["n_out"] for i in infos], skips=[i.get("skip_sym") for i in infos])
    cfv = compute_func_val or (lambda net, cond, *coords: cond.enforce(net, *coords))
    with trace_scope(g):
        coords = [Sym(g, g.coord(i), leaf=True) for i in range(n_coords)]
        funcs = [cfv(n, c, *coords) for n, c in zip(all_nets, conditions)]
        res = diff_eqs(*funcs, *coords) if diff_eqs is not None else []
        if isinstance(res, Sym):
            res = [res]
        def column(r):
            if isinstance(r, Sym):
                return r
            try:
                return Sym(g, g.const(float(r)))
            except (TypeError, ValueError, RuntimeError):
                raise TraceUnsupported(f"an equation returned {type(r).__name__}, not a traced (N, 1) column or a scalar")
        res = [column(r) for r in res]
        eq_ext = list(g.ext_log)
        from .symbolic import SymMat
        func_columns = []
        for f in funcs:
            if isinstance(f, Sym):
                func_columns.append([f])
            elif isinstance(f, SymMat) and all(isinstance(c, Sym) for c in f.cols):
                func_columns.append(list(f.cols))
            else:
                raise TraceUnsupported(f"a condition returned {type(f).__name__}, not traced (N, k) values")
        eq_nodes = tuple(c.i for cols in func_columns for c in cols) + ("|",) + tuple(r.i for r in res)

        def eq_probe():
            n_captured = len(g.captured)
            twins_before = set(getattr(g, "twins", ()))
            n_vcoords, n_sites, known_sites = len(g.vcoords), len(g.site_net), dict(g._sites)
            g._vreplay = 0
            g.ext_log = []
            eq_probe.last_ext = None
            try:
                with trace_scope(g):
                    f2 = [cfv(n, c, *coords) for n, c in zip(all_nets, conditions)]
                    r2 = diff_eqs(*f2, *coords) if diff_eqs is not None else []
                    if isinstance(r2, Sym):
                        r2 = [r2]
                    r2 = [column(r) for r in r2]
                cols = []
                for f in f2:
                    if isinstance(f, Sym):
                        cols.append(f.i)
                    elif isinstance(f, SymMat) and all(isinstance(c, Sym) for c in f.cols):
                        cols.extend(c.i for c in f.cols)
                    else:
                        return False
                eq_probe.last_ext = list(g.ext_log)
                return tuple(cols) + ("|",) + tuple(r.i for r in r2) == eq_nodes
            except Exception as e:
                if not getattr(eq_probe, "warned", False):
                    eq_probe.warned = True
                    import warnings
                    warnings.warn(f"neurodiffeq_amd: re-tracing the equations raised {type(e).__name__}: {e}; the system is "
                                  "rebuilt from a fresh trace.  (On the fused path diff_eqs / the conditions run on symbolic "
                                  "columns, once per re-trace: they should be free of side effects.)", RuntimeWarning)
                return False
            finally:
                g._vreplay = None
                for idx in [i for i in g.vcoords if i >= n_coords + n_vcoords]:
                    del g.vcoords[idx]
                del g.site_net[n_sites:]
                for key in [k for k in g._sites if k not in known_sites]:
                    g.net_deps.pop(g._sites[key], None)
                    g.net_nout.pop(g._sites[key], None)
                    del g._sites[key]
                del g.captured[n_captured:]
                for key in [k for k in getattr(g, "twins", ()) if k not in twins_before]:
                    del g.twins[key]

        def suggest_volatile():
            last = getattr(eq_probe, "last_ext", None)
            if last is None or len(last) != len(eq_ext):
                return frozenset(g.volatile)
            return frozenset(g.volatile) | {i for i, (a, b) in enumerate(zip(eq_ext, last)) if a != b and (a == a or b == b)}

        loss_term = None
        loss_probe = None
        if callable(loss):
            from .symbolic import SymMat, SymScalar
            loss_callable = loss
            val = loss(SymMat(res) if res else Sym(g, g.const(0.0)), list(funcs), list(coords))
            if not isinstance(val, SymScalar):
                raise TraceUnsupported(f"the loss function returned {type(val).__name__}, not a batch mean of traced values")
            loss_term, loss = val.term.i, "custom"

            def loss_probe():
                with trace_scope(g):
                    again = loss_callable(SymMat(res) if res else Sym(g, g.const(0.0)), list(funcs), list(coords))
                return isinstance(again, SymScalar) and again.term.i == loss_term
        metric_terms = []
        for fn in metrics:
            from .symbolic import MetricTraceUnsupported, SymScalar
            try:
                val = fn(*funcs, *coords)
            except Exception as e:
                raise MetricTraceUnsupported(f"a metric could not be traced ({type(e).__name__}: {e})") from e
            if not isinstance(val, SymScalar):
                raise MetricTraceUnsupported(f"a metric returned {type(val).__name__}, not a batch mean of traced values")
            metric_terms.append(val.term)
        metric_fns = list(metrics)

        def metric_probe():
            with trace_scope(g):
                for fn, term in zip(metric_fns, metric_terms):
                    again = fn(*funcs, *coords)
                    if not (isinstance(again, SymScalar) and again.term.i == term.i):
                        return False
            return True
    for k, info in enumerate(infos):
        g.net_deps.setdefault(k, tuple(range(info["d"])))
        g.net_nout.setdefault(k, info["n_out"])
    descs = {}

    def allow_lap(k, coords):
        info = infos[g.site_net[k]]
        deps = g.net_deps[k]
        if os.environ.get("NDQ_NO_LAP") or any(c not in deps for c in coords) or info["n_out"] != 1:
            return False
        mask2 = 0
        for c in coords:
            a = deps.index(c)
            mask2 |= 1 << codegen.pair_list(len(deps)).index((a, a))
        d = _lib.MlpDesc(len(deps), 1, mask2, info["hidden"], info["layers"], info["act"], info["n_out"], 1, info["skip"], 0, info["actp"], info["widths"], info["mono"])
        return codegen.ensure_mlp_kernels(d, f64=f64)

    def widen(k, st):
        info = infos[g.site_net[k]]
        if st.d != info["d"]:
            raise TraceUnsupported("network input width differs from the number of coordinates fed to it")
        if st.lap:
            descs[k] = _lib.MlpDesc(st.d, 1, st.mask2, info["hidden"], info["layers"], info["act"], info["n_out"], 1, info["skip"], 0, info["actp"], info["widths"], info["mono"])
            codegen.ensure_mlp_kernels(descs[k], f64=f64)
            return
        exact = _lib.MlpDesc(st.d, 1 if (st.first or st.mask2) else 0, st.mask2, info["hidden"], info["layers"],
                             info["act"], info["n_out"], 0, info["skip"], st.mask3, info["actp"], info["widths"], info["mono"],
                             getattr(st, "mask4", 0))
        if codegen.ensure_mlp_kernels(exact, f64=f64):
            st.first, st.mask2 = exact.first, exact.mask2
            descs[k] = exact
            return
        if st.mask3 or getattr(st, "mask4", 0):
            raise TraceUnsupported(f"no gfx950 kernel for third- / fourth-order streams of FCNN d={st.d} hidden={info['hidden']} "
                                   f"layers={info['layers']} act={info['act']} (mask3={st.mask3:#b})")
        npair = st.d * (st.d + 1) // 2
        best = None
        for first in ((1,) if st.first else (0, 1)):
            for mask2 in range(1 << npair):
                if (mask2 & st.mask2) != st.mask2 or (mask2 and not first):
                    continue
                d = _lib.MlpDesc(st.d, first, mask2, info["hidden"], info["layers"], info["act"], info["n_out"], 0,
                                 info["skip"], 0, info["actp"], info["widths"], info["mono"])
                if L.ndq_mlp_supported(ctypes.byref(d)):
                    cost = first * st.d + bin(mask2).count("1")
                    if best is None or cost < best[0]:
                        best = (cost, d)
        if best is None:
            raise TraceUnsupported(f"no gfx950 kernel for FCNN d={st.d} hidden={info['hidden']} layers="
                                   f"{info['layers']} streams(first={st.first}, mask2={st.mask2:#b})")
        st.first, st.mask2 = best[1].first, best[1].mask2
        descs[k] = best[1]

    unify = functools.partial(codegen.unify, site_net=g.site_net, n_coords=n_coords, vcoords=g.vcoords, infos=infos, f64=f64)
    program = codegen.PointwiseProgram(g, [r.i for r in res],
                                       [c.i for cols in func_columns for c in cols] + [m.i for m in metric_terms],
                                       len(nets), widen=widen, allow_lap=allow_lap, unify=unify, loss=loss,
                                       loss_term=loss_term)
    program.n_metrics = len(metric_terms)
    program.func_widths = [len(cols) for cols in func_columns]
    program.loss_probe = loss_probe
    program.metric_probe = metric_probe if metric_terms else None
    program.eq_probe = eq_probe
    program.suggest_volatile = suggest_volatile
    program.unique_nets = nets
    return program, descs


def wants_closure(program, descs, f64):
    if not f64:
        return codegen.can_fuse(program, descs)
    if os.environ.get("NDQ_F64_CLOSURE", "1") == "0":
        return False
    return codegen.can_fuse_f64(program, descs) or codegen.can_fuse_multi_f64(program, descs)


def f64_fused_tail_switch(environ=None):
    environ = os.environ if environ is None else environ
    return environ.get("NDQ_F64_FUSED_TAIL", "0") == "1"


class FusedSystem:
    def __init__(self, nets, conditions, diff_eqs, n_coords, device, compute_func_val=None, single_kernel=True,
                 loss="l2", metrics=(), dtype=torch.float32, volatile=frozenset()):
        self.device = torch.device(device)
        if self.device.type != "cuda":
            raise _lib.NdqError("the fused path needs an MI355X (device 'cuda'); no CPU fallback exists for it")
        from . import _canary
        _canary.check()
        self.dt = dtype
        self.f64 = dtype == torch.float64
        self.esize = 8 if self.f64 else 4
        self.L = _Lib64() if self.f64 else _lib.lib()
        self.f64_fused_tail = self.f64 and f64_fused_tail_switch()
        self.nets, self.conditions, self.n_coords = list(nets), list(conditions), n_coords
        self.program, self.descs = trace_system(self.nets, self.conditions, diff_eqs, n_coords, compute_func_val, loss,
                                                metrics, f64=self.f64, volatile=volatile)
        self.nets = list(self.program.unique_nets)
        self.n_eq, self.n_funcs = len(self.program.residuals), len(self.program.funcs)
        self.n_metrics = self.program.n_metrics
        self.n_user_funcs = self.n_funcs - self.n_metrics
        self.loss_norm = self.program.loss_norm
        self.theta_params = list(self.program.g.params)
        self.theta_frozen = sorted(self.program.g.frozen)
        self._theta_trainable = [j for j in range(len(self.theta_params)) if j not in self.program.g.frozen]
        self._theta_frozen_seen = None
        self.data_cols = list(self.program.g.data)
        self.n_theta, self.n_data = len(self.theta_params), len(self.data_cols)
        self.n_rows = n_coords + self.n_data
        if (self.n_theta or self.n_data) and self.f64:
            raise TraceUnsupported("trainable equation coefficients / data columns on the fp64 pipeline")
        from . import _hipcc
        want_fused = single_kernel and wants_closure(self.program, self.descs, self.f64)
        with _hipcc.deferred():
            pw_so = codegen.build(self.program, f64=self.f64)
            fused_so = codegen.build_fused(self.program, self.descs[0], f64=self.f64) if want_fused else None
        self.kernel = codegen.PointwiseKernel(pw_so, self.f64)
        self.fusedk = None
        self.fusedk_wide = None if (os.environ.get("NDQ_FUSED_WIDE", "1") != "0" and not _canary.STATUS["refuse_two_waves"]
                                    and not self.f64) else False
        self._self_check = os.environ.get("NDQ_SELF_CHECK", "1") != "0"
        self._verified = set()
        if fused_so is not None:
            fk = codegen.FusedKernel(fused_so, self.f64)
            if fk.lib.ndq_fused_lds_bytes() <= 160 * 1024:
                self.fusedk = fk
        self.flat = [FlatParams(n, self.device, dtype) for n in self.nets]
        self.site_net = list(self.program.site_net)
        self.n_sites = len(self.site_net)
        self.vcoords = dict(self.program.g.vcoords)
        self.ns = [self.program.streams[k].n_streams * self.program.streams[k].n_out for k in range(self.n_sites)]
        self.site_deps = [tuple(self.program.streams[k].deps) for k in range(self.n_sites)]
        self.coord0 = [d[0] if all(c < n_coords for c in d) and list(d) == list(range(d[0], d[0] + len(d))) else None
                       for d in self.site_deps]
        for k in range(self.n_sites):
            assert self.L.ndq_mlp_num_params(ctypes.byref(self.descs[k])) == self.flat[self.site_net[k]].numel
        self._bufs = {}
        self._resident_cache = {}
        self._static, self._static_seen = {}, {}
        self._dev_index = self.device.index if self.device.index is not None else torch.cuda.current_device()
        self.loss_buf = torch.zeros(64, dtype=dtype, device=self.device)
        if self.n_theta:
            self.theta_buf = torch.zeros(self.n_theta, dtype=dtype, device=self.device)
            self.gtheta = torch.zeros(self.n_theta, dtype=dtype, device=self.device)
            self.kernel.lib.ndq_pw_bind_theta.argtypes = [_c_vp, _c_vp]
            self.kernel.lib.ndq_pw_bind_theta.restype = None

    def set_batch_size(self, n_global):
        t = getattr(self.program.g, "_nbatch_t", None)
        if t is not None:
            t.fill_(float(n_global))

    def refresh_theta(self):
        if self.n_theta:
            with torch.no_grad():
                def value(p):
                    v = p[0].detach().reshape(-1)[p[1]] if isinstance(p, tuple) else p.detach().reshape(())
                    return v.to(self.device, self.dt)
                if not self.theta_frozen:
                    self.theta_buf.copy_(torch.stack([value(p) for p in self.theta_params]))
                    return
                if self._theta_trainable:
                    live = torch.stack([value(self.theta_params[j]) for j in self._theta_trainable])
                    self.theta_buf[self._theta_trainable] = live
                values = tuple(float(self.theta_params[j]) for j in self.theta_frozen)
                if values != self._theta_frozen_seen:
                    self._theta_frozen_seen = values
                    self.theta_buf[self.theta_frozen] = torch.tensor(values, dtype=self.dt).to(self.device)

    def _bind_theta(self, b, lib, fused):
        if self.n_theta:
            fn = lib.ndq_fused_bind_theta if fused else lib.ndq_pw_bind_theta
            fn(_ptr(self.theta_buf), _ptr(b["theta_partials"]))

    def reduce_theta(self, b, blocks, stream, accumulate):
        if self.n_theta:
            rc = self.L.ndq_reduce_partials(_ptr(b["theta_partials"]), blocks, self.n_theta, _ptr(self.gtheta),
                                            1 if accumulate else 0, 1.0, stream)
            _lib.check(rc, "ndq_reduce_partials(theta)")

    def attach_theta_grads(self):
        for j, p in enumerate(self.theta_params):
            if j in self.program.g.frozen:
                continue
            if isinstance(p, tuple):
                t, k = p
                if t.grad is None:
                    t.grad = torch.zeros_like(t)
                t.grad.reshape(-1)[k] = self.gtheta[j].to(t.device, t.dtype)
                continue
            g = self.gtheta[j].reshape(p.shape).to(p.device, p.dtype)
            if p.grad is not None and p.grad.shape == g.shape and p.grad.data_ptr() != self.gtheta[j].data_ptr():
                p.grad.copy_(g)
            else:
                p.grad = g.clone()

    def _resident_ld(self, batch):
        if self.n_data or any(c.dtype != self.dt or not c.is_contiguous() for c in batch):
            return 0
        p0 = batch[0].data_ptr()
        if len(batch) == 1:
            return _round_up(batch[0].numel(), 64) if p0 % 16 == 0 else 0
        step = batch[1].data_ptr() - p0
        if step <= 0 or step % self.esize or step // self.esize < batch[0].numel():
            return 0
        if any(c.data_ptr() != p0 + i * step for i, c in enumerate(batch)):
            return 0
        return step // self.esize

    MAX_BUFFER_SETS = 8
    WIDE_MIN_POINTS = int(os.environ.get("NDQ_FUSED_WIDE_MIN", 0))

    def _wide_possible(self):
        mode = codegen.MODES.get(codegen.fuse_mode(self.program, self.descs))
        if mode is not None and not mode.eight_wave:
            return False
        if mode is not None and mode.eight_wave_opt_in:
            return os.environ.get(mode.eight_wave_opt_in, "0") == "1"
        d = self.descs[0]
        nb, layers = (d.hidden + 15) // 16, d.layers
        ns = self.L.ndq_mlp_num_streams(ctypes.byref(d))
        return nb * nb * (layers - 1) + nb * ns * layers <= 40

    @staticmethod
    def prefers_wide(n):
        tiles = (n + 15) // 16
        r4, r8 = -(-tiles // 1024), -(-tiles // 2048)
        return 0.37 + 1.63 * r8 < r4

    def needs_check(self, n):
        fk = self.fused_variant(n) if self._self_check else None
        return fk is not None and id(fk) not in self._verified

    select_n = None

    def fused_variant(self, n):
        if self.fusedk is None:
            return None
        n = self.select_n or n
        memo = self.__dict__.get("_variant_memo")
        if memo is not None and memo[0] == n and memo[1] is self.fusedk_wide:
            return memo[2]
        fk = self._fused_variant(n)
        if self.fusedk_wide is not None:
            self._variant_memo = (n, self.fusedk_wide, fk)
        return fk

    def _fused_variant(self, n):
        if n >= self.WIDE_MIN_POINTS and self.prefers_wide(n) and self.fusedk_wide is not False:
            if self.fusedk_wide is None and not self._wide_possible():
                self.fusedk_wide = False
            if self.fusedk_wide is None:
                wide = codegen.FusedKernel(codegen.build_fused(self.program, self.descs[0], threads=512))
                ok = wide.threads > self.fusedk.threads and wide.lib.ndq_fused_lds_bytes() <= 160 * 1024
                self.fusedk_wide = wide if ok else False
            if self.fusedk_wide is not False:
                return self.fusedk_wide
        return self.fusedk

    def buffers(self, n, ld=None):
        key = (n, ld)
        b = self._bufs.get(key)
        if b is not None:
            self._bufs[key] = self._bufs.pop(key)
            return b
        while len(self._bufs) >= self.MAX_BUFFER_SETS:
            old = self._bufs.pop(next(iter(self._bufs)))
            fs = getattr(self, "_fast", None)
            if fs is not None:
                for k in [k for k in fs["structs"] if k[2] == id(old)]:
                    del fs["structs"][k]
            self._resident_cache = {k: v for k, v in self._resident_cache.items() if v[1] is not old}
        ld = ld or _round_up(n, 64)
        dev, f32 = self.device, self.dt
        b = dict(ld=ld,
                 coords_own=torch.zeros(self.n_rows, ld, dtype=f32, device=dev),
                 pinned=[torch.zeros(self.n_rows, ld, dtype=f32, device="cpu").pin_memory() for _ in range(4)],
                 pin_events=[None] * 4, pin_next=0,
                 jets=[torch.zeros(ns, ld, dtype=f32, device=dev) for ns in self.ns],
                 gbar=[torch.zeros(ns, ld, dtype=f32, device=dev) for ns in self.ns],
                 funcs=torch.zeros(self.n_funcs, ld, dtype=f32, device=dev),
                 resid=torch.zeros(max(self.n_eq, 1), ld, dtype=f32, device=dev),
                 pw_blocks=self.kernel.blocks(n))
        b["loss_partials"] = torch.zeros(b["pw_blocks"], dtype=f32, device=dev)
        b["bwd_blocks"] = [self.L.ndq_mlp_bwd_blocks(ctypes.byref(self.descs[k]), n) for k in range(self.n_sites)]
        b["partials"] = [torch.empty(nb, self.flat[self.site_net[k]].numel, dtype=f32, device=dev)
                         for k, nb in enumerate(b["bwd_blocks"])]
        b["site_coords"] = {}
        for k, deps in enumerate(self.site_deps):
            if self.coord0[k] is None:
                blk = torch.zeros(len(deps), ld, dtype=f32, device=dev)
                for row, c in enumerate(deps):
                    if c in self.vcoords:
                        blk[row].fill_(self.vcoords[c])
                b["site_coords"][k] = blk
        fk = b["fusedk"] = self.fused_variant(n)
        if fk is not None:
            b["fused_launch"] = ctypes.cast(fk.lib.ndq_fused_launch, ctypes.c_void_p).value
            b["fused_launch_multi"] = ctypes.cast(fk.lib.ndq_fused_launch_multi, ctypes.c_void_p).value
            b["fused_blocks"] = fk.blocks(n)
            b["fused_partials_all"] = [torch.empty(b["fused_blocks"], fp.numel, dtype=f32, device=dev) for fp in self.flat]
            b["fused_partials"] = b["fused_partials_all"][0]
            b["fused_partials_pp"] = (_c_vp * len(self.nets))(*[t.data_ptr() for t in b["fused_partials_all"]])
            b["fused_loss_partials"] = torch.zeros(b["fused_blocks"], dtype=f32, device=dev)
        if self.n_theta:
            rows = max(b["pw_blocks"], b.get("fused_blocks", 0))
            b["theta_partials"] = torch.zeros(rows, self.n_theta, dtype=f32, device=dev)
        b["jets_pp"] = (_c_vp * self.n_sites)(*[t.data_ptr() for t in b["jets"]])
        b["gbar_pp"] = (_c_vp * self.n_sites)(*[t.data_ptr() for t in b["gbar"]])
        b["coords"], b["coords_rows"] = b["coords_own"], None
        self._bufs[key] = b
        return b

    def upload(self, batch, lo=0, hi=None):
        n_all = batch[0].numel()
        hi = n_all if hi is None else hi
        n = hi - lo
        if batch[0].device.type == "cuda" and lo == 0 and hi == n_all:
            hit = self._resident_cache.get(id(batch))
            if hit is not None and hit[0] is batch:
                b = hit[1]
                b["coords_rows"] = hit[2]
                return b, n
            ld = self._resident_ld(batch)
            if ld:
                b = self.buffers(n, ld=ld)
                b["coords"] = batch[0].reshape(-1)
                b["coords_rows"] = [c.reshape(-1) for c in batch]
                if len(self._resident_cache) < 64:
                    self._resident_cache[id(batch)] = (batch, b, b["coords_rows"])
                return b, n
        if batch[0].device.type != "cuda" and not self.n_data:
            hit = self._static_batch(batch, lo, hi, n)
            if hit is not None:
                return hit, n
        b = self.buffers(n)
        b["coords"], b["coords_rows"] = b["coords_own"], None
        if self.n_data:
            for col in self.data_cols:
                if col.numel() != n_all:
                    raise _lib.NdqError(f"a per-point data column of the equations has {col.numel()} entries, the batch "
                                        f"{n_all} points: data columns must be aligned with the generator's points")
            batch = list(batch) + [col.detach().to(batch[0].device) for col in self.data_cols]
        if batch[0].device.type == "cuda":
            for i, c in enumerate(batch):
                b["coords_own"][i, :n].copy_(c.detach().reshape(-1)[lo:hi])
        else:
            k = b["pin_next"]
            b["pin_next"] = (k + 1) % len(b["pinned"])
            if b["pin_events"][k] is not None:
                b["pin_events"][k].synchronize()
            pinned = b["pinned"][k]
            for i, c in enumerate(batch):
                pinned[i, :n].copy_(c.detach().reshape(-1)[lo:hi])
            b["coords_own"].copy_(pinned, non_blocking=True)
            ev = b["pin_events"][k] or torch.cuda.Event()
            ev.record(self._stream_obj())
            b["pin_events"][k] = ev
        return b, n

    def _stream(self):
        return _c_vp(_raw_stream(self._dev_index))

    def _stream_obj(self):
        raw = _raw_stream(self._dev_index)
        c = self.__dict__.get("_stream_cache")
        if c is None or c[0] != raw:
            c = self._stream_cache = (raw, torch.cuda.current_stream(self.device))
        return c[1]

    @staticmethod
    def static_key(batch):
        if batch[0].device.type == "cuda":
            return None
        return tuple((c.untyped_storage().data_ptr(), c.storage_offset(), c.numel(), c._version) + _ends(c) for c in batch)

    def _static_batch(self, batch, lo, hi, n):
        key = self.static_key(batch) + (lo, hi)
        hit = self._static.get(key)
        if hit is not None:
            b = self.buffers(n, ld=hit[1].shape[1])
            b["coords"], b["coords_rows"] = hit[2][0], hit[2]
            return b
        if key in self._static_seen and len(self._static) < 16:
            ld = _round_up(n, 64)
            block = torch.zeros(self.n_coords, ld, dtype=self.dt, device=self.device)
            host = torch.stack([c.detach().reshape(-1)[lo:hi].to(self.dt) for c in batch])
            block[:, :n].copy_(host)
            rows = [block[i] for i in range(self.n_coords)]
            self._static[key] = (list(batch), block, rows)
            b = self.buffers(n, ld=ld)
            b["coords"], b["coords_rows"] = rows[0], rows
            return b
        self._static_seen[key] = list(batch)
        while len(self._static_seen) > 8:
            self._static_seen.pop(next(iter(self._static_seen)))
        return None

    def static_block(self, batch):
        n = batch[0].numel()
        key = self.static_key(batch) + (0, n)
        hit = self._static.get(key)
        if hit is None:
            while len(self._static) >= 16:
                self._static.pop(next(iter(self._static)))
            ld = _round_up(n, 64)
            block = torch.zeros(self.n_coords, ld, dtype=self.dt, device=self.device)
            block[:, :n].copy_(torch.stack([c.detach().reshape(-1).to(self.dt) for c in batch]))
            hit = self._static[key] = (list(batch), block, [block[i] for i in range(self.n_coords)])
        return hit[2][0].data_ptr(), n, hit[1].shape[1]

    def _coord_ptr(self, b, row):
        if b["coords_rows"] is not None:
            return _c_vp(b["coords_rows"][row].data_ptr())
        return _c_vp(b["coords_own"][row].data_ptr())

    def coord_columns(self, b, n):
        if b["coords_rows"] is not None:
            return [c[:n].view(-1, 1) for c in b["coords_rows"]]
        return [b["coords_own"][i, :n].view(-1, 1) for i in range(self.n_coords)]

    def split_functions(self, rows):
        out, r = [], 0
        for k in self.program.func_widths:
            out.append(rows[r].reshape(-1, 1) if k == 1 else rows[r:r + k].t())
            r += k
        return out

    def func_columns(self, b, n):
        return self.split_functions(b["funcs"][:self.n_user_funcs, :n])

    def metric_sums(self, b, n):
        return b["funcs"][self.n_user_funcs:self.n_funcs, :n].sum(dim=1)

    def _site_coords(self, b, k, n, refresh):
        if self.coord0[k] is not None:
            return self._coord_ptr(b, self.coord0[k])
        blk = b["site_coords"][k]
        if refresh:
            for row, c in enumerate(self.site_deps[k]):
                if c not in self.vcoords:
                    src = b["coords_rows"][c] if b["coords_rows"] is not None else b["coords_own"][c]
                    blk[row, :n].copy_(src[:n])
        return _c_vp(blk.data_ptr())

    def forward(self, b, n, stream):
        for fp in self.flat:
            fp.sync()
        for k in range(self.n_sites):
            fp = self.flat[self.site_net[k]]
            rc = self.L.ndq_mlp_jet_fwd(ctypes.byref(self.descs[k]), self._site_coords(b, k, n, True), b["ld"], n,
                                        _ptr(fp.flat), _ptr(b["jets"][k]), b["ld"], stream)
            _lib.check(rc, "ndq_mlp_jet_fwd")

    def evaluate(self, coords):
        b, n = self.upload([c.reshape(-1) for c in coords])
        stream = self._stream()
        self.set_batch_size(n)
        self.refresh_theta()
        self.forward(b, n, stream)
        self.pointwise(b, n, stream, False, n, want_funcs=True)
        return b["funcs"][:self.n_user_funcs, :n]

    def residuals(self, coords):
        b, n = self.upload([c.reshape(-1) for c in coords])
        stream = self._stream()
        self.set_batch_size(n)
        self.refresh_theta()
        self.forward(b, n, stream)
        self.pointwise(b, n, stream, False, n, want_resid=True)
        return b["resid"][:, :n]

    def pointwise(self, b, n, stream, train, n_global, want_funcs=False, want_resid=False):
        seed = 1.0 / (float(n_global) * self.loss_norm)
        self._bind_theta(b, self.kernel.lib, False)
        rc = self.kernel.lib.ndq_pw_launch(self._coord_ptr(b, 0), b["ld"], n, b["jets_pp"],
                                           b["gbar_pp"] if train else None, b["ld"],
                                           _ptr(b["funcs"]) if want_funcs else None,
                                           _ptr(b["resid"]) if want_resid else None,
                                           _ptr(b["loss_partials"]), seed, stream)
        _lib.check(rc, "ndq_pw_launch")
        return seed

    def backward(self, b, n, stream, accumulate, after_forward=False):
        seen = set()
        for k in range(self.n_sites):
            net = self.site_net[k]
            fp = self.flat[net]
            ext = codegen.mlp_ext_module(self.descs[k], self.f64) if after_forward else None
            hint = getattr(ext, "ndq_ext_reuse_forward", None) if ext is not None else None
            if hint is not None:
                hint(1)
            rc = self.L.ndq_mlp_jet_bwd(ctypes.byref(self.descs[k]), self._site_coords(b, k, n, False), b["ld"], n,
                                        _ptr(fp.flat), _ptr(b["gbar"][k]), b["ld"], _ptr(b["partials"][k]), stream)
            if hint is not None:
                hint(0)
            _lib.check(rc, "ndq_mlp_jet_bwd")
            rc = self.L.ndq_reduce_partials(_ptr(b["partials"][k]), b["bwd_blocks"][k], fp.numel, _ptr(fp.grad),
                                            1 if (accumulate or net in seen) else 0, 1.0, stream)
            _lib.check(rc, "ndq_reduce_partials")
            seen.add(net)

    def reduce_loss(self, b, stream, seed, slot):
        rc = self.L.ndq_reduce_partials(_ptr(b["loss_partials"]), b["pw_blocks"], 1,
                                        _c_vp(self.loss_buf.data_ptr() + self.esize * slot), 0, seed, stream)
        _lib.check(rc, "ndq_reduce_partials(loss)")

    def verify_fused(self, b, n, n_global=None):
        fk = b.get("fusedk")
        if fk is None or not self._self_check or id(fk) in self._verified:
            return True
        self._verified.add(id(fk))
        n_global = n if n_global is None else n_global
        stream = self._stream()
        keep = [fp.grad_loss.clone() for fp in self.flat], self.loss_buf[:1].clone()

        def grads():
            return (torch.cat([fp.grad for fp in self.flat] + ([self.gtheta] if self.n_theta else [])).clone(),
                    self.loss_buf[:1].clone())
        runs = []
        for _ in range(2):
            self.fused_closure(b, n, stream, True, n_global, 0, False)
            runs.append(grads())
        tv_same = self._tv_matches_plain(b, n, n_global, stream) if (self.FIT_RUN and not self.n_theta and not self.f64) else True
        pipe = []
        for _ in range(2):
            self.forward(b, n, stream)
            seed = self.pointwise(b, n, stream, True, n_global, False, False)
            self.backward(b, n, stream, False)
            self.reduce_theta(b, b["pw_blocks"], stream, False)
            self.reduce_loss(b, stream, seed, 0)
            pipe.append(grads())
        for fp, g in zip(self.flat, keep[0]):
            fp.grad_loss.copy_(g)
        self.loss_buf[:1].copy_(keep[1])
        if not all(bool(torch.isfinite(x).all()) for pair in runs + pipe for x in pair):
            self._verified.discard(id(fk))
            self.fused_check = dict(inconclusive="non-finite gradients / loss on the batch at hand")
            return True
        same = bool(torch.equal(runs[0][0], runs[1][0]) and torch.equal(runs[0][1], runs[1][1]))
        pipe_same = bool(torch.equal(pipe[0][0], pipe[1][0]) and torch.equal(pipe[0][1], pipe[1][1]))
        ref = pipe[0][0].double()
        err = float((runs[0][0].double() - ref).norm() / ref.norm().clamp_min(1e-30))
        lerr = float((runs[0][1] - pipe[0][1]).abs() / pipe[0][1].abs().clamp_min(1e-30))
        self.fused_check = dict(reproducible=same, pipeline_reproducible=pipe_same, grad_rel_l2=err, loss_rel=lerr,
                                train_valid_launch_identical=tv_same)
        same = same and tv_same
        if os.environ.get("NDQ_SELF_CHECK_LOG"):
            import json
            with open(os.environ["NDQ_SELF_CHECK_LOG"], "a") as fh:
                fh.write(json.dumps(dict(self.fused_check, n=n, threads=fk.threads, nets=len(self.flat))) + "\n")
        if not pipe_same:
            raise _lib.NdqError(f"the three-kernel pipeline of this system is not bit-reproducible ({self.fused_check}); "
                                "refusing to train on it")
        if same and err < self.SELF_CHECK_TOL and lerr < self.SELF_CHECK_TOL:
            return True
        import warnings
        if fk is self.fusedk_wide:
            warnings.warn(f"8-wave closure kernel rejected by its self-check ({self.fused_check}); large batches of this "
                          "system use the 4-wave build as well", RuntimeWarning)
        else:
            warnings.warn(f"single-launch closure kernel rejected by its self-check ({self.fused_check}); this system "
                          "continues on the three-kernel pipeline", RuntimeWarning)
            self.fusedk = None
        self.fusedk_wide = False
        self._bufs.clear()
        self._resident_cache.clear()
        self._fast = None
        return False

    def _tv_matches_plain(self, b, n, n_global, stream):
        fk = b["fusedk"]
        dev, f32 = self.device, self.dt
        seed = 1.0 / (float(n_global) * self.loss_norm)
        params_pp = (_c_vp * len(self.flat))(*[fp.flat.data_ptr() for fp in self.flat])
        want_parts = [t.clone() for t in b["fused_partials_all"]]
        want_loss = b["fused_loss_partials"].clone()
        blocks = b["fused_blocks"]
        ev = torch.zeros(blocks, dtype=f32, device=dev)
        rc = fk.lib.ndq_fused_launch_multi(self._coord_ptr(b, 0), b["ld"], n, params_pp, None, _ptr(ev), None, None, b["ld"],
                                           seed, 0, stream)
        _lib.check(rc, "ndq_fused_launch_multi")
        ok = True
        for with_train, with_valid in ((True, True), (True, False), (False, True)):
            parts = [torch.full_like(t, float("nan")) for t in want_parts]
            lp = torch.full_like(want_loss, float("nan"))
            vp = torch.full_like(ev, float("nan"))
            parts_pp = (_c_vp * len(parts))(*[t.data_ptr() for t in parts])
            rc = fk.lib.ndq_fused_launch_tv(self._coord_ptr(b, 0) if with_train else None, b["ld"], n if with_train else 0,
                                            params_pp, parts_pp if with_train else None, _ptr(lp) if with_train else None,
                                            seed, self._coord_ptr(b, 0) if with_valid else None, b["ld"],
                                            n if with_valid else 0, _ptr(vp) if with_valid else None, None, stream)
            _lib.check(rc, "ndq_fused_launch_tv")
            if with_train:
                ok = ok and torch.equal(lp, want_loss) and all(torch.equal(a, w) for a, w in zip(parts, want_parts))
            if with_valid:
                ok = ok and torch.equal(vp, ev)
        return bool(ok)

    SELF_CHECK_TOL = 2e-5

    def reject_fused(self):
        self.fusedk, self.fusedk_wide, self._fast = None, False, None
        self._bufs.clear()
        self._resident_cache.clear()

    def verify_on(self, batch, n_global=None, lo=0, hi=None):
        b, n = self.upload(batch, lo, hi)
        self.set_batch_size(n if n_global is None else n_global)
        self.refresh_theta()
        ok = self.verify_fused(b, n, n_global)
        if batch[0].device.type != "cuda":
            self._static_seen.pop(self.static_key(batch) + (lo, batch[0].numel() if hi is None else hi), None)
        return ok

    def fused_closure(self, b, n, stream, train, n_global, slot, accumulate, want_funcs=False, want_resid=False):
        for fp in self.flat:
            fp.sync()
        seed = 1.0 / (float(n_global) * self.loss_norm)
        params_pp = (_c_vp * len(self.flat))(*[fp.flat.data_ptr() for fp in self.flat])
        self._bind_theta(b, b["fusedk"].lib, True)
        rc = b["fusedk"].lib.ndq_fused_launch_multi(self._coord_ptr(b, 0), b["ld"], n, params_pp,
                                                    b["fused_partials_pp"] if train else None,
                                                    _ptr(b["fused_loss_partials"]),
                                                    _ptr(b["funcs"]) if want_funcs else None,
                                                    _ptr(b["resid"]) if want_resid else None, b["ld"], seed,
                                                    1 if train else 0, stream)
        _lib.check(rc, "ndq_fused_launch_multi")
        if train:
            for fp, part in zip(self.flat, b["fused_partials_all"]):
                rc = self.L.ndq_reduce_partials(_ptr(part), b["fused_blocks"], fp.numel, _ptr(fp.grad),
                                                1 if accumulate else 0, 1.0, stream)
                _lib.check(rc, "ndq_reduce_partials")
            self.reduce_theta(b, b["fused_blocks"], stream, accumulate)
        rc = self.L.ndq_reduce_partials(_ptr(b["fused_loss_partials"]), b["fused_blocks"], 1,
                                        _c_vp(self.loss_buf.data_ptr() + self.esize * slot), 0, seed, stream)
        _lib.check(rc, "ndq_reduce_partials(loss)")

    HIST = 8192

    def fast_ready(self, dist=None):
        return self.fusedk is not None and (len(self.nets) == 1 or dist is None) and not self.f64 and not self.n_theta

    def f64_tail_ready(self):
        return self.f64 and self.f64_fused_tail and self.fusedk is not None and not self.n_theta

    def launches_per_step(self):
        if self.f64_tail_ready():
            return 2
        if self.fusedk is not None and self.f64:
            return 2 + 2 * len(self.flat)
        if self.fusedk is not None:
            return 2
        total = 1 + 1 + len(self.flat)
        for k in range(self.n_sites):
            d = self.descs[k]
            if d.hidden > 64 and d.layers >= 2:
                wide_head = 1 if d.hidden > 128 else 0
                total += (1 + (d.layers - 1) + wide_head) + (wide_head + 2 * (d.layers - 1) + 1) + 1
            else:
                total += 1 + 2
        return total

    def fast_state(self):
        if getattr(self, "_fast", None) is None:
            dev, f32 = self.device, self.dt
            self._fast = dict(loss_hist=torch.zeros(self.HIST, dtype=f32, device=dev),
                              valid_hist=torch.zeros(self.HIST, dtype=f32, device=dev),
                              best_loss=torch.full((2,), float("inf"), dtype=f32, device=dev),
                              best_flat=[torch.zeros_like(fp.grad) for fp in self.flat], parity=0, pending=0,
                              pending_valid=0, structs={})
        return self._fast

    def _fill_step(self, st, k, n, ld, blocks, partials, loss_partials):
        fs, fp = self.fast_state(), self.flat[k]
        st.n, st.ldc, st.ldj, st.blocks, st.n_params = n, ld, ld, blocks, fp.numel
        if partials is not None:
            st.partials, st.loss_partials = partials.data_ptr(), loss_partials.data_ptr()
        st.grad, st.loss_slot = fp.grad.data_ptr(), fp.grad_loss.data_ptr() + self.esize * fp.numel
        st.loss_hist, st.best_loss = fs["loss_hist"].data_ptr(), fs["best_loss"].data_ptr()

    @staticmethod
    def _set_adam(st, m, v, group):
        st.adam_m, st.adam_v = m.data_ptr(), v.data_ptr()
        (st.beta1, st.beta2), st.lr, st.eps, st.weight_decay = group["betas"], group["lr"], group["eps"], group["weight_decay"]

    @staticmethod
    def _tail_args(fp, adam_slot):
        if adam_slot is None:
            return _ptr(fp.flat), None, None, None, fp.numel, 0.0, 0.0, 0.0, 0.0, 0.0, 1
        m, v, group, step = adam_slot
        return (_ptr(fp.flat), _ptr(fp.grad), _ptr(m), _ptr(v), fp.numel, group["lr"], *group["betas"], group["eps"],
                group["weight_decay"], step)

    def epoch_tail(self, kind, n_batches, track_best, adam_slots=None):
        fs = self.fast_state()
        stream = self._stream()
        train = kind == "train"
        hist = fs["loss_hist"] if train else fs["valid_hist"]
        idx = fs["pending"] if train else fs["pending_valid"]
        parity = fs["parity"]
        for k, fp in enumerate(self.flat):
            fp.sync()
            args = self._tail_args(fp, adam_slots[k] if train else None)
            rc = self.L.ndq_epoch_tail(*args, _ptr(self.loss_buf), n_batches, _ptr(hist), idx, _ptr(fs["best_loss"]),
                                       parity, _ptr(fs["best_flat"][k]) if track_best else None, 1 if k == 0 else 0,
                                       stream)
            _lib.check(rc, "ndq_epoch_tail")
        if train:
            fs["pending"] += 1
        else:
            fs["pending_valid"] += 1
        fs["parity"] ^= 1

    def fast_train_epoch_multi(self, batch, adam_slots, track_best):
        fs = self.fast_state()
        b, n = self.upload(batch)
        K = len(self.flat)
        key = (n, b["ld"], id(b), "multi")
        arr = fs["structs"].get(key)
        if arr is None:
            arr = (_lib.FusedStep * K)()
            for k in range(K):
                self._fill_step(arr[k], k, n, b["ld"], b["fused_blocks"], b["fused_partials_all"][k], b["fused_loss_partials"])
            fs["structs"][key] = arr
        step = None
        for k, fp in enumerate(self.flat):
            fp.sync()
            m, v, group, step_k = adam_slots[k]
            step = step_k if step is None else step
            st = arr[k]
            st.params = fp.flat.data_ptr()
            st.seed = 1.0 / (float(n) * self.loss_norm)
            st.best_flat = fs["best_flat"][k].data_ptr() if track_best else None
            self._set_adam(st, m, v, group)
        rc = self.L.ndq_fused_multi_step_run(arr, K, _c_vp(b["fused_launch_multi"]), self._coord_ptr(b, 0), step,
                                             fs["pending"], fs["parity"], self._stream())
        _lib.check(rc, "ndq_fused_multi_step_run")
        fs["pending"] += 1
        fs["parity"] ^= 1

    def fast_train_epoch_f64(self, batch, adam_slots, track_best):
        fs = self.fast_state()
        b, n = self.upload(batch)
        K = len(self.flat)
        key = (n, b["ld"], id(b), "f64")
        arr = fs["structs"].get(key)
        if arr is None:
            arr = (_lib.FusedStep64 * K)()
            for k in range(K):
                self._fill_step(arr[k], k, n, b["ld"], b["fused_blocks"], b["fused_partials_all"][k], b["fused_loss_partials"])
            fs["structs"][key] = arr
        step = adam_slots[0][3]
        for k, fp in enumerate(self.flat):
            fp.sync()
            m, v, group, _ = adam_slots[k]
            st = arr[k]
            st.params = fp.flat.data_ptr()
            st.seed = 1.0 / (float(n) * self.loss_norm)
            st.loss_slot = self.loss_buf.data_ptr()
            st.best_flat = fs["best_flat"][k].data_ptr() if track_best else None
            self._set_adam(st, m, v, group)
        rc = self.L.ndq_fused_step_run(arr, K, _c_vp(b["fused_launch_multi"]), self._coord_ptr(b, 0), step, fs["pending"],
                                       fs["parity"], self._stream())
        _lib.check(rc, "ndq64_fused_step_run")
        fs["pending"] += 1
        fs["parity"] ^= 1

    def fast_train_epoch(self, batch, optimizer, adam_slot, track_best, n_global=None, dist=None):
        fs = self.fast_state()
        b, n = self.upload(batch)
        fp = self.flat[0]
        fp.sync()
        m, v, group, step = adam_slot
        key = (n, b["ld"], id(b))
        st = fs["structs"].get(key)
        if st is None:
            st = _lib.FusedStep()
            st.launch = b["fused_launch"]
            self._fill_step(st, 0, n, b["ld"], b["fused_blocks"], b["fused_partials"], b["fused_loss_partials"])
            fs["structs"][key] = st
        n_global = n if n_global is None else n_global
        st.params = fp.flat.data_ptr()
        st.seed = 1.0 / (float(n_global) * self.loss_norm)
        st.best_flat = fs["best_flat"][0].data_ptr() if track_best else None
        self._set_adam(st, m, v, group)
        stream = self._stream()
        coords = self._coord_ptr(b, 0)
        hist_index, parity = fs["pending"], fs["parity"]
        src = generators.device_source(batch) if dist is None else None
        if src is not None and src.prefetch and b["coords_rows"] is not None:
            st.next_sampler = ctypes.addressof(src.desc)
            st.next_seed, st.next_draw, st.next_stream = src.seed, src.draw, src.stream_id
            nxt = src.block_of(src.draw)
            st.next_coords, st.next_ldc = nxt.data_ptr(), nxt.shape[1]
        else:
            src, st.next_sampler = None, None
        direct = dist.direct(self.device, fp.numel + 1) if dist is not None else None
        if dist is None or direct is not None:
            st.allreduce, st.comm = direct if direct is not None else (None, None)
            rc = self.L.ndq_fused_step_run(ctypes.byref(st), coords, step, hist_index, parity, stream)
            _lib.check(rc, "ndq_fused_step_run")
            if src is not None:
                src.prefetched = src.draw
        else:
            st.adam_m = st.adam_v = None
            st.allreduce = st.comm = None
            rc = self.L.ndq_fused_step_run(ctypes.byref(st), coords, step, hist_index, parity, stream)
            _lib.check(rc, "ndq_fused_step_run")
            dist.all_reduce_flat(fp.grad_loss)
            rc = self.L.ndq_epoch_tail(*self._tail_args(fp, adam_slot), _c_vp(st.loss_slot), 1, _ptr(fs["loss_hist"]),
                                       hist_index, _ptr(fs["best_loss"]), parity,
                                       _ptr(fs["best_flat"][0]) if track_best else None, 1, stream)
            _lib.check(rc, "ndq_epoch_tail")
        fs["pending"] += 1
        fs["parity"] ^= 1

    FIT_RUN = os.environ.get("NDQ_FIT_RUN", "1") != "0"
    FIT_PULL = os.environ.get("NDQ_FIT_PULL", "1") != "0"
    FIT_LOOP = os.environ.get("NDQ_FIT_LOOP", "1") != "0"

    def fit_ready(self):
        return self.FIT_RUN and self.fusedk is not None and not self.f64 and not self.n_theta

    def resident_ptr(self, batch):
        if batch[0].device.type != "cuda" or len(batch) != self.n_coords:
            return None
        ld = self._resident_ld(batch)
        return (batch[0].data_ptr(), ld) if ld else None

    def stage_batches(self, host_block, n, reserve=0):
        K = host_block.shape[0]
        ld = _round_up(n, 64)
        st = self.__dict__.setdefault("_stage", dict(pinned=[None, None], events=[None, None], next=0, dev=[None, None]))
        i = st["next"]
        st["next"] ^= 1
        need = K * self.n_coords * ld
        if st["pinned"][i] is None or st["pinned"][i].numel() < need:
            if st["events"][i] is not None:
                st["events"][i].synchronize()
            size = max(need, reserve * self.n_coords * ld)
            for j in (0, 1):
                if st["pinned"][j] is None or st["pinned"][j].numel() < size:
                    if st["events"][j] is not None:
                        st["events"][j].synchronize()
                    st["pinned"][j] = torch.zeros(size, dtype=torch.float32, device="cpu", pin_memory=True)
                    st["dev"][j] = torch.zeros(size, dtype=torch.float32, device=self.device)
        elif st["events"][i] is not None:
            st["events"][i].synchronize()
        pinned = st["pinned"][i][:need].view(K, self.n_coords, ld)
        import numpy as np
        np.copyto(pinned.numpy()[:, :, :n], host_block.detach().numpy(), casting="same_kind")
        dev = st["dev"][i][:need].view(K, self.n_coords, ld)
        dev.copy_(pinned, non_blocking=True)
        ev = st["events"][i] or torch.cuda.Event()
        ev.record()
        st["events"][i] = ev
        return dev, ld

    def fit_run(self, train_ptrs, n, ld, adam_slots, valid=None, track_best=0, n_global=None):
        fs = self.fast_state()
        K = len(train_ptrs)
        if K:
            self._fit_last_n = n
        fk = self.fused_variant(n if K else (getattr(self, "_fit_last_n", None) or valid[1]))
        key = (id(fk), n if K else 0, ld if K else 0, (valid[1], valid[2]) if valid else None)
        cache = fs.setdefault("fit", {})
        ent = cache.get(key)
        if ent is None:
            if len(cache) >= 8:
                cache.pop(next(iter(cache)))
            dev, f32 = self.device, torch.float32
            ff = _lib.FusedFit()
            ff.launch = ctypes.cast(fk.lib.ndq_fused_launch_tv, ctypes.c_void_p).value
            ff.n_nets = len(self.flat)
            keep = []
            blocks = fk.blocks(n) if K else 0
            lparts = torch.zeros(max(blocks, 1), dtype=f32, device=dev)
            keep.append(lparts)
            for k, fp in enumerate(self.flat):
                part = torch.empty(blocks, fp.numel, dtype=f32, device=dev) if K else None
                keep.append(part)
                self._fill_step(ff.net[k], k, *((n, ld, blocks) if K else (0, 0, 0)), part, lparts)
                ff.net[k].best_flat = fs["best_flat"][k].data_ptr()
            if valid is not None:
                vparts = torch.zeros(fk.blocks(valid[1]), dtype=f32, device=dev)
                keep.append(vparts)
                ff.valid_n, ff.valid_ldc, ff.valid_blocks = valid[1], valid[2], vparts.numel()
                ff.valid_scale = 1.0 / (float(valid[1]) * self.loss_norm)
                ff.valid_loss_partials, ff.valid_hist = vparts.data_ptr(), fs["valid_hist"].data_ptr()
            ff.pull_ok = 0
            if K and self.FIT_PULL and 0 < blocks * len(self.flat) <= 16 and fk.lib.ndq_fused_pull_ok():
                ff.pull_ok = 1
                for k, fp in enumerate(self.flat):
                    alt = [torch.zeros(fp.numel, dtype=f32, device=dev) for _ in range(3)]
                    apart = torch.empty(blocks, fp.numel, dtype=f32, device=dev)
                    keep.extend(alt + [apart])
                    ff.alt_params[k], ff.alt_m[k], ff.alt_v[k] = (t.data_ptr() for t in alt)
                    ff.alt_partials[k] = apart.data_ptr()
                alp = torch.zeros(max(blocks, 1), dtype=f32, device=dev)
                keep.append(alp)
                ff.alt_loss_partials = alp.data_ptr()
                if valid is not None:
                    avp = torch.zeros(ff.valid_blocks, dtype=f32, device=dev)
                    keep.append(avp)
                    ff.alt_valid_loss_partials = avp.data_ptr()
                if self.FIT_LOOP and blocks == 1 and (valid is None or ff.valid_blocks == 1) and len(self.flat) <= 2 \
                        and fk.lib.ndq_fused_loop_ok():
                    ff.launch_loop = ctypes.cast(fk.lib.ndq_fused_launch_loop, ctypes.c_void_p).value
                    ff.loop_ok = 1
            ent = cache[key] = (ff, keep, fk, {}, (_c_vp * 1)(), ctypes.byref(ff))
        ff = ent[0]
        step0 = 1
        last = ent[3]
        for k, fp in enumerate(self.flat):
            fp.sync()
            if K:
                m, v, group, step0 = adam_slots[k]
                now = (fp.flat.data_ptr(), n if n_global is None else n_global, m.data_ptr(), v.data_ptr(), group["lr"],
                       group["betas"], group["eps"], group["weight_decay"])
            else:
                now = (fp.flat.data_ptr(),)
            if last.get(k) != now:
                last[k] = now
                st = ff.net[k]
                st.params = now[0]
                if K:
                    st.seed = 1.0 / (float(now[1]) * self.loss_norm)
                    self._set_adam(st, m, v, group)
        vc = valid[0] if valid is not None else None
        if last.get("v") != (vc, track_best):
            last["v"] = (vc, track_best)
            ff.valid_coords = vc
            ff.track_best = track_best
        if K == 1:
            coords = ent[4]
            coords[0] = train_ptrs[0]
        else:
            coords = (_c_vp * max(K, 1))(*train_ptrs) if K else None
        rc = self.L.ndq_fused_fit_run(ent[5], K, coords, step0, fs["pending"], fs["pending_valid"], fs["parity"],
                                      self._stream())
        _lib.check(rc, "ndq_fused_fit_run")
        tails = K + (1 if valid is not None else 0)
        fs["pending"] += K
        if valid is not None:
            fs["pending_valid"] += max(K, 1)
        fs["parity"] ^= tails & 1

    def fast_flush(self):
        fs = getattr(self, "_fast", None)
        if fs is None or (fs["pending"] == 0 and fs["pending_valid"] == 0):
            return [], [], None
        k, kv = fs["pending"], fs["pending_valid"]
        vals = torch.cat([fs["loss_hist"][:k], fs["valid_hist"][:kv],
                          fs["best_loss"][fs["parity"]:fs["parity"] + 1]]).tolist()
        fs["pending"] = fs["pending_valid"] = 0
        return vals[:k], vals[k:k + kv], vals[k + kv]

    def step(self, batch, train, slot=0, accumulate=False, n_global=None, lo=0, hi=None, want_funcs=False,
             want_resid=False):
        b, n = self.upload(batch, lo, hi)
        n_global = n if n_global is None else n_global
        stream = self._stream()
        self.set_batch_size(n_global)
        self.refresh_theta()
        if train and not accumulate and not self.verify_fused(b, n, n_global):
            b, n = self.upload(batch, lo, hi)
        if b["fusedk"] is not None:
            self.fused_closure(b, n, stream, train, n_global, slot, accumulate, want_funcs, want_resid)
            return b, n
        self.forward(b, n, stream)
        seed = self.pointwise(b, n, stream, train, n_global, want_funcs, want_resid)
        if train:
            self.backward(b, n, stream, accumulate, after_forward=True)
            self.reduce_theta(b, b["pw_blocks"], stream, accumulate)
        self.reduce_loss(b, stream, seed, slot)
        return b, n
```

### neurodiffeq_amd/solvers.py

```python
import inspect
import sys
import warnings
from abc import ABC, abstractmethod
from copy import deepcopy
from itertools import chain

import torch
import torch.nn as nn

from . import _lib
from .conditions import BaseCondition
from .generators import (Generator1D, Generator2D, GeneratorSpherical, SamplerGenerator, draws_are_static,
                         draws_have_fixed_size, device_source, on_default_device)
from . import autograd_ops
from .losses import _losses
from .networks import FCNN, describe
from .neurodiffeq import safe_diff as diff
from .optim import FusedAdam
from .symbolic import MetricTraceUnsupported, TraceUnsupported, captured_unchanged
from .networks import STRUCTURE as _net_structure
import os as _os
_QUICK_KEY = _os.environ.get("NDQ_QUICK_KEY", "1") != "0"
_LC = []


def _library_code():
    if not _LC:
        from .engine import library_code
        _LC.append(library_code)
    return _LC[0]


_CLOSURE_CACHE = {}


def _requires_closure(optimizer):
    cls = type(optimizer)
    r = _CLOSURE_CACHE.get(cls)
    if r is None:
        p = inspect.signature(optimizer.step).parameters.get("closure")
        r = _CLOSURE_CACHE[cls] = bool(p) and p.default == inspect._empty
    return r


def _unique_params(nets):
    seen, out = set(), []
    for p in chain.from_iterable(n.parameters() for n in nets):
        if id(p) not in seen:
            seen.add(id(p))
            out.append(p)
    return out


def sobolev_equations(diff_eqs, n_funcs, semi=False):
    def extended(*variables):
        res = list(diff_eqs(*variables))
        total = res[0]
        for r in res[1:]:
            total = total + r
        grads = [diff(total, x) for x in variables[n_funcs:]]
        return grads if semi else res + grads
    return extended


def _default_l2(residual, funcs, coords):
    return (residual ** 2).mean()


class BaseSolver(ABC):
    EQ_PROBE_EVERY = 1024
    LOSS_PROBE_EVERY = 1

    """See the module docstring; constructor arguments are the reference's (solvers.py:36-140)."""

    fused = "auto"

    def __init__(self, diff_eqs, conditions, nets=None, train_generator=None, valid_generator=None,
                 analytic_solutions=None, optimizer=None, loss_fn=None, n_batches_train=1, n_batches_valid=4,
                 metrics=None, n_input_units=None, n_output_units=None, shuffle=None, batch_size=None,
                 criterion=None):
        attrs_of_the_subclass = frozenset(self.__dict__)
        if criterion is not None:
            warnings.warn("`criterion` is deprecated; use `loss_fn`", FutureWarning)
            loss_fn = criterion if loss_fn is None else loss_fn
        if shuffle:
            warnings.warn("param `shuffle` is deprecated and ignored; shuffling should be performed by generators",
                          FutureWarning)
        if batch_size is not None:
            warnings.warn("param `batch_size` is deprecated and ignored; specify n_batches_train and "
                          "n_batches_valid instead", FutureWarning)
        self.diff_eqs = diff_eqs
        self.conditions = conditions
        self.n_funcs = len(conditions)
        if nets is None:
            self.nets = [FCNN(n_input_units=n_input_units, n_output_units=n_output_units, hidden_units=(32, 32),
                              actv=nn.Tanh) for _ in range(self.n_funcs)]
        else:
            self.nets = nets
        if train_generator is None:
            raise ValueError("train_generator must be specified")
        if valid_generator is None:
            raise ValueError("valid_generator must be specified")

        self.device = torch.device("cuda") if torch.cuda.is_available() else torch.device("cpu")
        if self.device.type == "cuda":
            for n in self.nets:
                n.to(self.device)

        self.metrics_fn = metrics if metrics else {}
        if analytic_solutions:
            warnings.warn("The `analytic_solutions` argument is deprecated and could lead to unstable behavior. "
                          "Pass a `metrics` dict instead.", FutureWarning)

            def analytic_mse(*args):
                x = args[-n_input_units:]
                u_hat = analytic_solutions(*x)
                u = args[:-n_input_units]
                u, u_hat = torch.stack(u), torch.stack(u_hat)
                return ((u - u_hat) ** 2).mean()

            if "analytic_mse" in self.metrics_fn:
                warnings.warn("Ignoring `analytic_solutions` in presence of key 'analytic_mse' in `metrics`",
                              FutureWarning)
            else:
                self.metrics_fn["analytic_mse"] = analytic_mse

        self._history = {"train_loss": [], "valid_loss": []}
        self._history.update({"train__" + name: [] for name in self.metrics_fn})
        self._history.update({"valid__" + name: [] for name in self.metrics_fn})

        self.optimizer = optimizer if optimizer else FusedAdam(_unique_params(self.nets))
        self._set_loss_fn(loss_fn)
        self.generator = {"train": SamplerGenerator(on_default_device(train_generator)),
                          "valid": SamplerGenerator(on_default_device(valid_generator))}
        self.n_batches = {"train": n_batches_train, "valid": n_batches_valid}
        self._batch = {"train": None, "valid": None}
        if self.n_batches["valid"] == 0 and _requires_closure(self.optimizer):
            warnings.warn(f"Setting n_batches_valid=0 will update lowest_loss and best_net with training loss "
                          f"instead of validation loss. This is a problem for {self.optimizer.__class__} optimizer "
                          f"because it updates the parameters before the training loss computed. "
                          f"This leads to potentially worse solution in `best_net`!", RuntimeWarning)
        self._best_nets = None
        self._best_flat = None
        self._lowest_loss = None
        self.local_epoch = 0
        self._max_local_epoch = 0
        self._stop_training = False
        self._phase = None
        self._fused_sys = None
        self._composite_plain = False
        self._loss_probe_count = 0
        self._loss_time_dependent = False
        self._eq_watch = None
        self._eq_probe_countdown = 1
        self._fused_key = None
        self._metrics_follow_state = False
        self._fused_quick = None
        self._fused_quick_parts = None
        self._fast_tracks_best = False
        self.dist = None
        self._own_attrs = (frozenset(self.__dict__) - attrs_of_the_subclass) | {"_own_attrs", "_best_nets_from_device", "_dtype_probe", "_eq_watch_warned", "_lc", "_volatile",
                                                       "_eval_key", "_eval_sys", "_host_metrics", "_resid_key", "_resid_sys", "_autocast_warned"}

    def _set_loss_fn(self, criterion):
        if criterion is None:
            self.loss_fn = _default_l2
        elif isinstance(criterion, nn.modules.loss._Loss):
            self.loss_fn = lambda r, f, x: criterion(r, torch.zeros_like(r))
        elif isinstance(criterion, str):
            self.loss_fn = _losses[criterion.lower()]
        elif callable(criterion):
            self.loss_fn = criterion
        else:
            raise TypeError(f"Unknown type of criterion {type(criterion)}")

    @property
    def metrics_history(self):
        self._flush_device_history()
        return self._history

    @metrics_history.setter
    def metrics_history(self, value):
        self._flush_device_history()
        self._history = value

    @property
    def lowest_loss(self):
        self._flush_device_history()
        return self._lowest_loss

    @lowest_loss.setter
    def lowest_loss(self, value):
        self._flush_device_history()
        self._lowest_loss = value
        if self._fused_sys is not None and getattr(self._fused_sys, "_fast", None) is not None:
            self._fused_sys._fast["best_loss"].fill_(float("inf") if value is None else float(value))

    def _flush_device_history(self):
        system = self._fused_sys
        fs = getattr(system, "_fast", None) if system is not None else None
        if fs is None or (fs["pending"] == 0 and fs["pending_valid"] == 0):
            return
        losses, vlosses, best = system.fast_flush()
        if self.dist is not None:
            self.dist.check()
        self._history["train_loss"].extend(losses)
        self._history["valid_loss"].extend(vlosses)
        if best < float("inf") and (self._lowest_loss is None or best < self._lowest_loss):
            self._lowest_loss = best
            self._best_flat = list(fs["best_flat"])
            self._best_nets = None

    @property
    def global_epoch(self):
        pending = 0
        if self._fused_sys is not None and getattr(self._fused_sys, "_fast", None) is not None:
            pending = self._fused_sys._fast["pending"]
        return len(self._history["train_loss"]) + pending

    @property
    def batch(self):
        return self._batch

    @property
    def _batch_examples(self):
        warnings.warn("`._batch_examples` has been deprecated in favor of `._batch` and will be removed in a future "
                      "version", FutureWarning)
        return self._batch

    @property
    def criterion(self):
        warnings.warn(f"`{self.__class__.__name__}`.criterion is a deprecated alias for `.loss_fn`")
        return self.loss_fn

    @criterion.setter
    def criterion(self, loss_fn):
        warnings.warn(f"`{self.__class__.__name__}`.criterion is a deprecated alias for `.loss_fn`")
        self.loss_fn = loss_fn

    @property
    def best_nets(self):
        self._flush_device_history()
        if self._best_flat is not None:
            nets = deepcopy(self.nets)
            distinct = []
            for n in nets:
                if not any(n is m for m in distinct):
                    distinct.append(n)
            with torch.no_grad():
                for net, flat in zip(distinct, self._best_flat):
                    off = 0
                    for p in describe(net, dtype=flat.dtype)["params"]:
                        p.copy_(flat[off:off + p.numel()].view(p.shape))
                        off += p.numel()
            self._best_nets = nets
            self._best_flat = None
            self._best_nets_from_device = True
        return self._best_nets

    @best_nets.setter
    def best_nets(self, nets):
        self._best_nets, self._best_flat = nets, None

    def compute_func_val(self, net, cond, *coordinates):
        return cond.enforce(net, *coordinates)

    def additional_loss(self, residual, funcs, coords):
        return 0.0

    def _do_optimizer_step(self, closure=None):
        if closure is None:
            self.optimizer.step()
        else:
            self.optimizer.step(closure=closure)

    def _update_history(self, value, metric_type, key):
        self._phase = key
        self._flush_device_history()
        if metric_type == "loss":
            self._history[f"{key}_{metric_type}"].append(value)
        elif metric_type in self.metrics_fn:
            self._history[f"{key}__{metric_type}"].append(value)
        else:
            raise KeyError(f"metric '{metric_type}' not specified")

    def _update_train_history(self, value, metric_type):
        self._update_history(value, metric_type, key="train")

    def _update_valid_history(self, value, metric_type):
        self._update_history(value, metric_type, key="valid")

    def _generate_batch(self, key):
        self._phase = key
        ex = self.generator[key].get_examples()
        if not (len(ex) and ex[0].dim() == 2 and ex[0].shape[1] == 1):
            ex = [v.reshape(-1, 1) for v in ex]
        self._batch[key] = ex
        return ex

    def _generate_train_batch(self):
        return self._generate_batch("train")

    def _generate_valid_batch(self):
        return self._generate_batch("valid")

    def _fused_system_key(self, cfv):
        reason = None
        loss_kind = "l2" if self.loss_fn is _default_l2 else \
            next((k for k in ("l2", "l1", "infinity", "h1", "h1 semi") if self.loss_fn is _losses[k]), None)
        extra_loss = type(self).additional_loss is not BaseSolver.additional_loss
        if loss_kind is None or extra_loss:
            if loss_kind in ("h1", "h1 semi"):
                reason = "additional_loss override together with a Sobolev loss"
            loss_kind = "custom"
        if _requires_closure(self.optimizer) and self.dist is not None:
            reason = "closure-based optimizer under data parallelism"
        net_ids = tuple(id(n) for n in self.nets)
        probe = self.__dict__.get("_dtype_probe")
        if probe is None or probe[0] != net_ids:
            probe = self._dtype_probe = (net_ids, [p for p in (next(iter(n.parameters()), None) for n in self.nets) if p is not None])
        dtypes = {p.dtype for p in probe[1]}
        sys_dtype = torch.float64 if dtypes == {torch.float64} else torch.float32
        if self._loss_time_dependent:
            reason = "epoch-dependent loss function"
        key = (id(self.diff_eqs), net_ids, tuple(id(c) for c in self.conditions),
               cfv, reason, loss_kind, sys_dtype,
               id(self.loss_fn) if loss_kind == "custom" else None,
               tuple((name, id(fn)) for name, fn in self.metrics_fn.items()), _net_structure[0])
        self._fused_quick_parts = (self.diff_eqs, list(self.nets), list(self.conditions), cfv, self.loss_fn, self.optimizer,
                                   dict(self.metrics_fn), _net_structure[0], self._loss_time_dependent, self.dist, type(self),
                                   [(p, p.dtype) for p in probe[1]])
        return key, reason, loss_kind, sys_dtype

    def _fused_system(self, n_coords):
        if self.fused == "off" or self.device.type != "cuda":
            if self.fused == "require":
                raise _lib.NdqError("fused='require' but no MI355X is visible")
            return None
        if torch.is_autocast_enabled():
            if self.fused == "require":
                raise _lib.NdqError("fused='require' but torch.autocast is enabled: the fused kernels do not change precision with it")
            if not self.__dict__.get("_autocast_warned"):
                self._autocast_warned = True
                warnings.warn("neurodiffeq_amd: torch.autocast is enabled; this solver runs the reference's closure on torch autograd "
                              "while it is (the fused MI355X kernels compute in the networks' own precision).", RuntimeWarning)
            self._flush_device_history()
            return None
        q = self.__dict__.get("_fused_quick") if _QUICK_KEY else None
        cfv = getattr(self.compute_func_val, "__func__", self.compute_func_val)
        if q is not None and self.diff_eqs is q[0] and self.nets == q[1] and self.conditions == q[2] and cfv is q[3] \
                and self.loss_fn is q[4] and self.optimizer is q[5] and self.metrics_fn == q[6] and _net_structure[0] == q[7] \
                and self._loss_time_dependent is q[8] and self.dist is q[9] and type(self) is q[10] and self._fused_key is q[11] \
                and all(p.dtype is dt for p, dt in q[12]):
            key = q[11]
            reason, loss_kind, sys_dtype = key[4], key[5], key[6]
        else:
            key, reason, loss_kind, sys_dtype = self._fused_system_key(cfv)
            self._fused_quick = None
            if key == self._fused_key:
                key = self._fused_key
                parts = self._fused_quick_parts
                self._fused_quick = parts[:11] + (key, parts[11])
        if key == self._fused_key and self._fused_sys is not None and \
                not all(fp.all_trainable() and (not fp.act_state or fp.act_unchanged()) for fp in self._fused_sys.flat):
            self._flush_device_history()
            self._fused_key = None
        if key == self._fused_key and self._fused_sys is not None and not self._equations_unchanged(self._fused_sys):
            self._note_volatile(self._fused_sys)
            self._fused_key = None
        if key == self._fused_key:
            sysm = self._fused_sys
            if sysm is not None and not captured_unchanged(sysm.program.g):
                if self._equations_unchanged(sysm, force=True):
                    sysm.program.g.captured[:] = [(t, t._version, t.item()) for t, _, _ in sysm.program.g.captured]
                else:
                    self._note_volatile(sysm)
            if sysm is None or captured_unchanged(sysm.program.g):
                mprobe = getattr(sysm.program, "metric_probe", None) if sysm is not None else None
                if mprobe is not None:
                    try:
                        same = mprobe()
                    except Exception:
                        same = False
                    if not same:
                        self._metrics_follow_state = True
                        self._flush_device_history()
                        self._fused_key = None
                        return self._fused_system(n_coords)
                probe = getattr(sysm.program, "loss_probe", None) if sysm is not None else None
                if probe is None:
                    return sysm
                self._loss_probe_count += 1
                if self._loss_probe_count != 1 and self._loss_probe_count % self.LOSS_PROBE_EVERY:
                    return sysm
                try:
                    same = probe()
                except Exception:
                    same = False
                if same:
                    return sysm
                self._flush_device_history()
                self._fused_key, self._fused_sys = key, None
                reason = ("the loss function / additional_loss changed between epochs (it depends on solver or Python state, "
                          "which a traced kernel freezes)")
                if self.fused == "require":
                    raise _lib.NdqError(f"fused='require' but the system is outside the fused path: {reason}")
                warnings.warn(f"neurodiffeq_amd: this solver is NOT on the fused MI355X path any more ({reason}); it runs "
                              "the reference's closure on torch autograd instead.", RuntimeWarning)
                self._loss_time_dependent = True
                return None
        self._flush_device_history()
        self._fused_key, self._fused_sys = key, None
        if reason is None:
            try:
                from .engine import FusedSystem
                eqs, kind = self.diff_eqs, loss_kind
                if loss_kind in ("h1", "h1 semi"):
                    eqs, kind = sobolev_equations(self.diff_eqs, len(self.nets), semi=(loss_kind == "h1 semi")), "l2"
                elif loss_kind == "custom":
                    kind = lambda r, f, x: self.loss_fn(r, f, x) + self.additional_loss(r, f, x)
                self._host_metrics = False
                try:
                    if self._metrics_follow_state and self.metrics_fn:
                        raise MetricTraceUnsupported("a metric reads Python state that changes between epochs")
                    self._fused_sys = FusedSystem(self.nets, self.conditions, eqs, n_coords, self.device,
                                                  compute_func_val=self.compute_func_val, loss=kind,
                                                  metrics=list(self.metrics_fn.values()), dtype=sys_dtype,
                                                  volatile=self._volatile_for(key))
                except MetricTraceUnsupported:
                    if self.dist is not None:
                        raise
                    self._fused_sys = FusedSystem(self.nets, self.conditions, eqs, n_coords, self.device,
                                                  compute_func_val=self.compute_func_val, loss=kind, metrics=(),
                                                  dtype=sys_dtype, volatile=self._volatile_for(key))
                    self._host_metrics = True
                self._watch_equations()
                self._refuse_self_mutating_equations()
                if isinstance(self.optimizer, FusedAdam):
                    self.optimizer.bind(self._fused_sys.flat)
            except TraceUnsupported as e:
                reason = str(e)
            except _lib.NdqError:
                raise
            except Exception as e:
                if self.fused == "require":
                    raise
                reason = f"tracing the equations failed with {type(e).__name__}: {e}"
        if self._fused_sys is None:
            if self.fused == "require":
                raise _lib.NdqError(f"fused='require' but the system is outside the fused path: {reason}")
            warnings.warn(f"neurodiffeq_amd: this solver is NOT on the fused MI355X path ({reason}); it runs the "
                          "reference's closure on torch autograd instead -- same results, typically 10-100x slower per "
                          "step.  Pass fused='require' to make this an error.", RuntimeWarning)
        return self._fused_sys

    def _note_volatile(self, sysm):
        suggest = getattr(sysm.program, "suggest_volatile", None)
        if suggest is not None and self._fused_key is not None:
            self._volatile = (self._fused_key[:4], suggest())

    def _volatile_for(self, key):
        held = self.__dict__.get("_volatile")
        return held[1] if held is not None and held[0] == key[:4] else frozenset()

    def _watch_equations(self):
        self._eq_watch = self._new_state_watch()
        self._eq_probe_countdown = 1

    def _refuse_self_mutating_equations(self):
        watch, sysm = self._eq_watch, self._fused_sys
        probe = getattr(sysm.program, "eq_probe", None) if sysm is not None else None
        if watch is None or probe is None or len(watch) == 0:
            return
        try:
            probe()
        except Exception:
            pass
        if watch.dirty():
            self._fused_sys, self._eq_watch = None, None
            raise TraceUnsupported("the equations / conditions change the Python state they read every time they are evaluated "
                                   "(a call counter, a list they append to, ...); only the reference's own closure evaluates "
                                   "them as often as the reference does")

    def _equations_unchanged(self, sysm, force=False):
        watch = self._eq_watch
        dirty = watch is None or watch.dirty()
        blind = watch is not None and not watch.complete
        self._eq_probe_countdown -= 1
        if not (dirty or blind or force or self._eq_probe_countdown <= 0):
            return True
        probe = getattr(sysm.program, "eq_probe", None)
        if probe is None:
            return True
        if blind and not self.__dict__.get("_eq_watch_warned"):
            self._eq_watch_warned = True
            warnings.warn("neurodiffeq_amd: the equations / conditions read state that cannot be compared between epochs ("
                          + "; ".join(watch.incomplete) + "). They are re-traced every epoch instead (about 0.1 - 0.7 ms of host "
                          "time per epoch) and fit() runs epoch by epoch; results are unaffected.", RuntimeWarning)
        if self._eq_probe_countdown <= 0:
            self._eq_probe_countdown = self.EQ_PROBE_EVERY
        same = probe()
        if dirty:
            self._watch_equations_refresh()
        return same

    def _eq_watch_blocks_chunks(self):
        return self._eq_watch is None or not self._eq_watch.complete

    def _watch_equations_refresh(self):
        countdown = self._eq_probe_countdown
        self._eq_watch = self._new_state_watch()
        self._eq_probe_countdown = countdown

    def _new_state_watch(self):
        from ._pystate import StateWatch
        try:
            return StateWatch([self.diff_eqs, self.compute_func_val] + list(self.conditions), skip_modules=self.nets)
        except Exception as e:
            if not self.__dict__.get("_eq_watch_warned"):
                self._eq_watch_warned = True
                warnings.warn(f"neurodiffeq_amd: the Python state read by the equations could not be indexed ({type(e).__name__}: "
                              f"{e}); the equations are re-traced every epoch instead.", RuntimeWarning)
            return None

    @property
    def fused_active(self):
        return self._fused_sys is not None

    def _run_epoch(self, key):
        if self.n_batches[key] <= 0:
            return
        self._phase = key
        library_code = _library_code()
        inner = getattr(self.generator[key], "generator", None)
        if type(inner).__module__ == "neurodiffeq_amd.generators" and type(inner).__name__ in ("DeviceGenerator", "ResidentBatchGenerator") \
                and type(self)._generate_batch is BaseSolver._generate_batch:
            with library_code():
                first_batch = self._generate_batch(key)
        else:
            first_batch = self._generate_batch(key)
        system = self._fused_system(len(first_batch))
        if system is None:
            return self._run_epoch_composite(key, first_batch)
        if self.dist is not None:
            n_all = first_batch[0].shape[0]
            if n_all < self.dist.world_size and not self.dist.presharded:
                raise ValueError(f"a batch of {n_all} points cannot be sharded over {self.dist.world_size} ranks")
            system.select_n = n_all if self.dist.presharded else -(-n_all // self.dist.world_size)
        nb = self.n_batches[key]
        with library_code() as lc:
            self._lc = lc
            empty = first_batch[0].shape[0] == 0
            done = False if empty else self._run_epoch_native(key, system, first_batch)
        if empty:
            return self._run_epoch_composite(key, first_batch)
        if done:
            return
        metric_values = {name: 0.0 for name in self.metrics_fn}
        if system.loss_buf.numel() < nb:
            system.loss_buf = torch.zeros(nb, dtype=system.dt, device=self.device)
        closure_opt = key == "train" and _requires_closure(self.optimizer)
        if key == "train" and not closure_opt:
            self.optimizer.zero_grad()
        shard = self.dist
        for batch_id in range(nb):
            batch = first_batch if batch_id == 0 else self._generate_batch(key)
            n_all = batch[0].shape[0]
            lo, hi = shard.bounds(n_all) if shard else (0, n_all)
            if closure_opt:
                last = {}

                def closure():
                    last["bn"] = system.step(batch, train=True, slot=batch_id, accumulate=False, n_global=n_all,
                                             want_funcs=bool(self.metrics_fn))
                    for fp in system.flat:
                        fp.attach_grads()
                    system.attach_theta_grads()
                    return system.loss_buf[batch_id].clone()
                self._do_optimizer_step(closure=closure)
                b, n = last["bn"]
            else:
                b, n = system.step(batch, train=(key == "train"), slot=batch_id, accumulate=(batch_id > 0),
                                   n_global=shard.global_n(n_all) if shard else n_all, lo=lo, hi=hi,
                                   want_funcs=bool(self.metrics_fn))
            if self.metrics_fn and getattr(self, "_host_metrics", False):
                funcs, coords = system.func_columns(b, n), system.coord_columns(b, n)
                for name, fn in self.metrics_fn.items():
                    metric_values[name] += float(fn(*funcs, *coords))
            elif self.metrics_fn:
                sums = system.metric_sums(b, n)
                if shard:
                    sums = sums.contiguous()
                    shard.all_reduce_flat(sums)
                vals = (sums / float(shard.global_n(n_all) if shard else n_all)).tolist()
                for name, v in zip(self.metrics_fn, vals):
                    metric_values[name] += v
        if key == "train":
            for fp in system.flat:
                fp.attach_grads()
        if shard:
            shard.all_reduce(system, nb, train=(key == "train"))
        if key == "train":
            system.attach_theta_grads()
        epoch_loss = system.loss_buf[:nb].sum().item() / nb
        self._update_history(epoch_loss, "loss", key)
        if key == "valid" or self.n_batches["valid"] == 0:
            self._update_best(key)
        if key == "train" and not closure_opt:
            self._do_optimizer_step()
        for name in self.metrics_fn:
            self._update_history(metric_values[name] / nb, name, key)

    def _native_ok(self):
        cls = type(self)
        return (not self.metrics_fn and isinstance(self.optimizer, FusedAdam)
                and cls._do_optimizer_step is BaseSolver._do_optimizer_step
                and cls._update_best is BaseSolver._update_best
                and cls._update_history is BaseSolver._update_history)

    def _run_epoch_native(self, key, system, first_batch):
        if not self._native_ok() or system._theta_trainable:
            return False
        train = key == "train"
        nb = self.n_batches[key]
        track_best = (not train) or self.n_batches["valid"] == 0
        if train and system.fusedk is not None:
            n_all = first_batch[0].shape[0]
            lo, hi = self.dist.bounds(n_all) if self.dist else (0, n_all)
            if system.needs_check(hi - lo):
                ok = system.verify_on(first_batch, self.dist.global_n(n_all) if self.dist else n_all, lo, hi)
                if self.dist and not self.dist.agree(ok, self.device) and ok:
                    system.reject_fused()
        fs = system.fast_state()
        if max(fs["pending"], fs["pending_valid"]) >= system.HIST:
            self._flush_device_history()
        if fs["pending"] == 0 and fs["pending_valid"] == 0:
            fs["best_loss"].fill_(float("inf") if self._lowest_loss is None else float(self._lowest_loss))
        slots = None
        if train:
            if not all(self.optimizer.bound(fp) for fp in system.flat):
                self.optimizer.bind(system.flat)
                if not all(self.optimizer.bound(fp) for fp in system.flat):
                    return False
            slots = [self.optimizer.fast_slot(fp) for fp in system.flat]
        shard = self.dist
        one_batch = nb == 1 or (not train and draws_are_static(self.generator["valid"]))
        if shard is None and one_batch and system.fit_ready() and self._fit_epoch(key, system, first_batch, slots):
            pass
        elif train and nb == 1 and len(system.flat) > 1 and system.fast_ready(shard) and len({s[3] for s in slots}) == 1:
            system.fast_train_epoch_multi(first_batch, slots, track_best)
        elif train and nb == 1 and shard is None and system.f64_tail_ready() and len({s[3] for s in slots}) == 1:
            system.fast_train_epoch_f64(first_batch, slots, track_best)
        elif train and nb == 1 and len(system.flat) == 1 and system.fast_ready(shard):
            batch = first_batch
            n_all = batch[0].shape[0]
            if shard is not None:
                lo, hi = shard.bounds(n_all)
                if (lo, hi) != (0, n_all):
                    batch = [c[lo:hi] for c in batch]
            system.fast_train_epoch(batch, self.optimizer, slots[0], track_best,
                                    n_global=shard.global_n(n_all) if shard else n_all, dist=shard)
        else:
            if system.loss_buf.numel() < nb:
                system.loss_buf = torch.zeros(nb, dtype=system.dt, device=self.device)
            batches = [first_batch]
            if nb > 1:
                with self._lc.user_code():
                    batches += [self._generate_batch(key) for _ in range(nb - 1)]
            if not train and nb > 1:
                if all(b is batches[0] for b in batches[1:]) and batches[0][0].device.type != "cuda":
                    batches = batches[:1]
                else:
                    k0 = system.static_key(batches[0])
                    if k0 is not None and all(system.static_key(b) == k0 for b in batches[1:]):
                        batches = batches[:1]
            for batch_id, batch in enumerate(batches):
                n_all = batch[0].shape[0]
                lo, hi = shard.bounds(n_all) if shard else (0, n_all)
                system.step(batch, train=train, slot=batch_id, accumulate=(batch_id > 0),
                            n_global=shard.global_n(n_all) if shard else n_all, lo=lo, hi=hi)
            if shard:
                shard.all_reduce(system, len(batches), train=train)
            system.epoch_tail(key, len(batches), track_best, slots)
        if train:
            for fp in system.flat:
                if not fp.grads_attached():
                    fp.attach_grads()
        self._phase = key
        return True

    def _fit_epoch(self, key, system, batch, slots):
        train = key == "train"
        if train:
            if len({s[3] for s in slots}) != 1:
                return False
            src = device_source(batch)
            if src is not None and src.prefetch:
                return False
        n_all = batch[0].shape[0]
        if system.needs_check(n_all):
            return False
        b, n = system.upload(batch)
        ptr = system._coord_ptr(b, 0).value
        if train:
            system.fit_run([ptr], n, b["ld"], slots, None, track_best=1 if self.n_batches["valid"] == 0 else 0)
        else:
            system.fit_run([], 0, 0, None, (ptr, n, b["ld"]), track_best=2)
        return True

    _PER_EPOCH_METHODS = ("run_train_epoch", "run_valid_epoch", "_run_epoch", "_generate_batch", "_generate_train_batch",
                          "_generate_valid_batch")

    FIT_CHUNK = 256

    def _fit_chunk(self, remaining):
        system = self._fused_sys
        if system is None or self.dist is not None or self.n_batches["train"] != 1 or remaining < 2:
            return 0
        if not self._native_ok() or not system.fit_ready() or getattr(system.program, "loss_probe", None) is not None:
            return 0
        if system.n_data:
            return 0
        cls = type(self)
        if any(getattr(cls, m) is not getattr(BaseSolver, m) for m in self._PER_EPOCH_METHODS):
            return 0
        nv = self.n_batches["valid"]
        tg, vg = self.generator["train"], self.generator["valid"]
        if not draws_have_fixed_size(tg) or (nv > 0 and not draws_are_static(vg)):
            return 0
        if type(tg.generator).__name__ == "DeviceGenerator":
            return 0
        if self._fused_system(system.n_coords) is not system:
            return 0
        if self._eq_watch_blocks_chunks():
            return 0
        if not self._equations_unchanged(system, force=True):
            self._fused_key = None
            return 0
        n = tg.size
        if system.needs_check(n):
            return 0
        if not all(self.optimizer.bound(fp) for fp in system.flat):
            return 0
        if len({self.optimizer._steps.get(id(fp)) for fp in system.flat}) != 1:
            return 0
        fs = system.fast_state()
        if max(fs["pending"], fs["pending_valid"]) + 2 > system.HIST:
            self._flush_device_history()
        k_max = min(self.FIT_CHUNK, max(2, (64 << 20) // (4 * system.n_coords * (n + 63))))
        K = min(remaining, k_max, system.HIST - max(fs["pending"], fs["pending_valid"]))
        if K < 2:
            return 0
        if fs["pending"] == 0 and fs["pending_valid"] == 0:
            fs["best_loss"].fill_(float("inf") if self._lowest_loss is None else float(self._lowest_loss))
        valid = None
        if nv > 0:
            vcols = self._generate_batch("valid")
            vres = system.resident_ptr(vcols)
            if vcols[0].shape[0] < 1 or (vres is None and vcols[0].device.type == "cuda"):
                return 0
            valid = (vres[0], vcols[0].shape[0], vres[1]) if vres is not None else system.static_block(vcols)
        self._phase = "train"
        trace = getattr(self, "_fit_trace", None)
        if trace is not None:
            import time
            t0 = time.perf_counter()
        block = tg.generator.bulk_examples(K)
        if trace is not None:
            t1 = time.perf_counter()
        if block is not None:
            tg._last = None
            dev, ld = system.stage_batches(block, n, reserve=k_max)
            stride = 4 * system.n_coords * ld
            ptrs = [dev.data_ptr() + e * stride for e in range(K)]
            self._batch["train"] = [block[-1, i].reshape(-1, 1).clone().requires_grad_(True) for i in range(block.shape[1])]
        else:
            draws = [self._generate_batch("train") for _ in range(K)]
            if any(len(d) != system.n_coords or d[0].shape[0] != n for d in draws):
                raise RuntimeError(f"{tg.generator!r} returned batches of different shapes although its class draws a "
                                   "fixed number of points")
            if all(d is draws[0] for d in draws[1:]) and draws[0][0].device.type != "cuda":
                ptr, _, ld = system.static_block(draws[0])
                ptrs = [ptr] * K
            elif draws[0][0].device.type == "cuda":
                res = [system.resident_ptr(d) for d in draws]
                if any(r is None or r[1] != res[0][1] for r in res):
                    block = torch.stack([torch.stack([c.detach().reshape(-1) for c in d]) for d in draws])
                    dev = block.to(torch.float32)
                    ld = (n + 63) // 64 * 64
                    pad = torch.zeros(K, system.n_coords, ld, dtype=torch.float32, device=dev.device)
                    pad[:, :, :n] = dev
                    system._fit_keep = pad
                    ptrs = [pad.data_ptr() + e * 4 * system.n_coords * ld for e in range(K)]
                else:
                    ld = res[0][1]
                    ptrs = [r[0] for r in res]
            else:
                block = torch.stack([torch.stack([c.detach().reshape(-1) for c in d]) for d in draws])
                dev, ld = system.stage_batches(block, n, reserve=k_max)
                stride = 4 * system.n_coords * ld
                ptrs = [dev.data_ptr() + e * stride for e in range(K)]
        slots = [self.optimizer.fast_slots(fp, K) for fp in system.flat]
        if len({s[3] for s in slots}) != 1:
            raise RuntimeError("the networks of this solver are at different Adam step counts; call fit() with "
                               "callbacks or run epochs one by one")
        if trace is not None:
            t2 = time.perf_counter()
        system.fit_run(ptrs, n, ld, slots, valid, track_best=2 if nv > 0 else 1)
        if trace is not None:
            trace.append((K, t1 - t0, t2 - t1, time.perf_counter() - t2))
        for fp in system.flat:
            if not fp.grads_attached():
                fp.attach_grads()
        self._phase = "valid" if nv > 0 else "train"
        return K

    def _run_epoch_composite(self, key, first_batch):
        epoch_loss, batch_loss = 0.0, 0.0
        metric_values = {name: 0.0 for name in self.metrics_fn}
        closure_opt = _requires_closure(self.optimizer)
        if key == "train" and not closure_opt:
            self.optimizer.zero_grad()
        dev = self.device
        for batch_id in range(self.n_batches[key]):
            batch = first_batch if batch_id == 0 else self._generate_batch(key)
            if batch[0].device != dev:
                batch = [c.detach().to(dev).requires_grad_(True) for c in batch]
                self._batch[key] = batch

            def closure(zero_grad=True):
                if self._composite_plain:
                    with autograd_ops.native_autograd(False):
                        return closure_body(zero_grad)
                try:
                    with autograd_ops.native_autograd(None, coordinate_grads=False):
                        return closure_body(zero_grad)
                except autograd_ops.JetOrderError:
                    self._composite_plain = True
                    with autograd_ops.native_autograd(False):
                        return closure_body(zero_grad)

            def closure_body(zero_grad=True):
                nonlocal batch_loss
                if key == "train" and zero_grad:
                    self.optimizer.zero_grad()
                funcs = [self.compute_func_val(n, c, *batch) for n, c in zip(self.nets, self.conditions)]
                for name in self.metrics_fn:
                    metric_values[name] += self.metrics_fn[name](*funcs, *batch).item()
                residuals = torch.cat(self.diff_eqs(*funcs, *batch), dim=1)
                try:
                    loss = self.loss_fn(residuals, funcs, batch) + self.additional_loss(residuals, funcs, batch)
                except TypeError as e:
                    warnings.warn("You might need to update your code. Since v0.4.0; both `criterion` and "
                                  "`additional_loss` requires three inputs: `residual`, `funcs`, and `coords`.",
                                  FutureWarning)
                    raise e
                if key == "train":
                    loss.backward()
                    batch_loss = loss.item()
                return loss

            if key == "train":
                if closure_opt:
                    self._do_optimizer_step(closure=closure)
                else:
                    closure(zero_grad=False)
                epoch_loss += batch_loss
            else:
                epoch_loss += closure().item()
        self._update_history(epoch_loss / self.n_batches[key], "loss", key)
        if key == "valid" or self.n_batches["valid"] == 0:
            self._update_best(key)
        if key == "train" and not closure_opt:
            self._do_optimizer_step()
        for name in self.metrics_fn:
            self._update_history(metric_values[name] / self.n_batches[key], name, key)

    def run_train_epoch(self):
        self._run_epoch("train")

    def run_valid_epoch(self):
        self._run_epoch("valid")

    def _update_best(self, key):
        current_loss = self.metrics_history[key + "_loss"][-1]
        if (self._lowest_loss is None) or current_loss < self._lowest_loss:
            self._lowest_loss = current_loss
            outside = self._fused_sys is not None and any(isinstance(p, tuple) for p in self._fused_sys.theta_params)
            if self._fused_sys is not None and not outside:
                for fp in self._fused_sys.flat:
                    fp.sync()
                self._best_flat = [fp.flat.clone() for fp in self._fused_sys.flat]
                self._best_nets = None
            else:
                if self._fused_sys is not None:
                    for fp in self._fused_sys.flat:
                        fp.sync()
                self.best_nets = deepcopy(self.nets)

    def fit(self, max_epochs, callbacks=(), tqdm_file=sys.stderr, **kwargs):
        self._stop_training = False
        self._max_local_epoch = max_epochs
        monitor = kwargs.pop("monitor", None)
        if monitor:
            warnings.warn("Passing `monitor` is deprecated, use a MonitorCallback and pass a list of callbacks instead")
            callbacks = [monitor.to_callback()] + list(callbacks)
        if kwargs:
            raise ValueError(f"Unknown keyword argument(s): {list(kwargs.keys())}")
        bar = None
        if tqdm_file is not None:
            try:
                from tqdm.auto import tqdm
                bar = tqdm(total=max_epochs, desc="Training Progress", colour="blue", file=tqdm_file, dynamic_ncols=True)
            except ImportError:
                pass
        done = 0
        try:
            while done < max_epochs and not self._stop_training:
                k = self._fit_chunk(max_epochs - done) if not callbacks else 0
                if k == 0:
                    self.local_epoch = done + 1
                    self.run_train_epoch()
                    self.run_valid_epoch()
                    for cb in callbacks:
                        cb(self)
                    k = 1
                done += k
                self.local_epoch = done
                if bar is not None:
                    bar.update(k)
        finally:
            if bar is not None:
                bar.close()
        self._flush_device_history()

    @abstractmethod
    def get_solution(self, copy=True, best=True):
        pass

    def _solution(self, cls, copy, best):
        nets = self.best_nets if best else self.nets
        conditions = self.conditions
        if copy:
            nets, conditions = deepcopy(nets), deepcopy(conditions)
        return cls(nets, conditions)

    def _get_internal_variables(self):
        return {
            "metrics": self.metrics_fn, "n_batches": self.n_batches, "best_nets": self.best_nets,
            "criterion": self.loss_fn, "loss_fn": self.loss_fn, "conditions": self.conditions,
            "global_epoch": self.global_epoch, "lowest_loss": self.lowest_loss, "n_funcs": self.n_funcs,
            "nets": self.nets, "optimizer": self.optimizer, "diff_eqs": self.diff_eqs, "generator": self.generator,
            "train_generator": self.generator["train"], "valid_generator": self.generator["valid"],
        }

    def get_internals(self, var_names=None, return_type="list", param_names=None):
        if param_names is not None:
            warnings.warn("`param_names` is deprecated; use `var_names`", FutureWarning)
            var_names = param_names
        available = self._get_internal_variables()
        if var_names == "all" or var_names is None:
            return available
        if isinstance(var_names, str):
            return available[var_names]
        if return_type == "list":
            return [available[name] for name in var_names]
        if return_type == "dict":
            return {name: available[name] for name in var_names}
        raise ValueError(f"unrecognized return_type = {return_type}")

    def _fused_residuals(self, coords, best):
        if self.device.type != "cuda" or self.fused == "off" or any(c.dtype not in (torch.float32, torch.float64)
                                                                    for c in coords):
            return None
        nets = self.best_nets if best else self.nets
        if nets is None:
            return None
        key = (tuple(id(n) for n in nets), id(self.diff_eqs), tuple(id(c) for c in self.conditions), len(coords), _net_structure[0])
        volatile = frozenset()
        held = self._resid_sys if getattr(self, "_resid_key", None) == key else None
        if held is not None and not held.program.eq_probe():
            volatile = held.program.suggest_volatile()
            self._resid_key = None
        if getattr(self, "_resid_key", None) != key:
            self._resid_key, self._resid_sys = key, None
            try:
                from .engine import FusedSystem
                self._resid_sys = FusedSystem(nets, self.conditions, self.diff_eqs, len(coords), self.device,
                                              compute_func_val=self.compute_func_val, single_kernel=False, volatile=volatile)
            except TraceUnsupported:
                pass
        if self._resid_sys is None:
            return None
        res = self._resid_sys.residuals([c.detach().to(torch.float32) for c in coords])
        return [res[e].clone() for e in range(res.shape[0])]

    def get_residuals(self, *coords, to_numpy=False, best=True, no_reshape=False):
        coords = [c if isinstance(c, torch.Tensor) else torch.tensor(c) for c in coords]
        original_shape = coords[0].shape
        fused = self._fused_residuals(coords, best)
        if fused is not None:
            residuals = [r.reshape(-1, 1) if no_reshape else r.reshape(*original_shape) for r in fused]
            if to_numpy:
                residuals = [r.cpu().numpy() for r in residuals]
            return residuals if len(residuals) > 1 else residuals[0]
        coords = [c.detach().to(self.device).reshape(-1, 1).requires_grad_() for c in coords]
        solution = self.get_solution(copy=False, best=best)
        funcs = solution(*coords, to_numpy=False, no_reshape=no_reshape)
        if isinstance(funcs, torch.Tensor):
            funcs = [funcs]
        residuals = self.diff_eqs(*funcs, *coords)
        if not no_reshape:
            residuals = [r.reshape(*original_shape) for r in residuals]
        if to_numpy:
            residuals = [r.detach().cpu().numpy() for r in residuals]
        return residuals if len(residuals) > 1 else residuals[0]


class BaseSolution(ABC):

    def __init__(self, nets, conditions):
        if nets is None:
            raise RuntimeError("The nets cannot be None, check if you disabled validation and used `best`=True with "
                               "`get_solution` / `get_residual`")
        self.nets = [nets] * len(conditions) if isinstance(nets, nn.Module) else nets
        self.conditions = conditions

    @abstractmethod
    def _compute_u(self, net, condition, *coords):
        pass

    def __call__(self, *coords, to_numpy=False, no_reshape=False, as_type=None):
        if as_type is not None:
            warnings.warn("`as_type` is deprecated; use `to_numpy`", FutureWarning)
            to_numpy = as_type
        coords = [c if isinstance(c, torch.Tensor) else torch.tensor(c) for c in coords]
        original_shape = coords[0].shape
        try:
            dev = next(self.nets[0].parameters()).device
        except StopIteration:
            dev = coords[0].device
        coords = [c.to(dev).reshape(-1, 1) for c in coords]
        if isinstance(to_numpy, str):
            if to_numpy in ("tf", "torch"):
                to_numpy = False
            elif to_numpy == "np":
                to_numpy = True
            else:
                raise ValueError(f"Unrecognized `as_type` option: '{to_numpy}'")
        us = self._fused_values(coords)
        if us is None:
            us = [self._compute_u(net, con, *coords) for con, net in zip(self.conditions, self.nets)]
        if not no_reshape:
            us = [u.reshape(*original_shape) for u in us]
        if to_numpy:
            us = [u.detach().cpu().numpy() for u in us]
        return us if len(self.nets) > 1 else us[0]


    def _fused_values(self, coords):
        if coords[0].device.type != "cuda" or coords[0].dtype != torch.float32 or coords[0].requires_grad \
                or len(set(id(n) for n in self.nets)) != len(self.nets):
            return None
        key = (tuple(id(n) for n in self.nets), tuple(id(c) for c in self.conditions), len(coords), _net_structure[0])
        volatile = frozenset()
        held = self._eval_sys if getattr(self, "_eval_key", None) == key else None
        if held is not None and not held.program.eq_probe():
            volatile = held.program.suggest_volatile()
            self._eval_key = None
        if getattr(self, "_eval_key", None) != key:
            self._eval_key, self._eval_sys = key, None
            try:
                from .engine import FusedSystem
                self._eval_sys = FusedSystem(self.nets, self.conditions, None, len(coords), coords[0].device,
                                             compute_func_val=self._compute_u, single_kernel=False, volatile=volatile)
            except (TraceUnsupported, _lib.NdqError):
                pass
        if self._eval_sys is None:
            return None
        return [v.clone() for v in self._eval_sys.split_functions(self._eval_sys.evaluate(coords))]


class GenericSolution(BaseSolution):
    def _compute_u(self, net, condition, *coords):
        return condition.enforce(net, *coords)


class Solution1D(GenericSolution):
    pass


class Solution2D(GenericSolution):
    pass


class SolutionSpherical(GenericSolution):
    """u(r, theta, phi) of a network that takes all three coordinates (solvers.py:971-980)."""


class SolutionSphericalHarmonics(SolutionSpherical):

    def __init__(self, nets, conditions, max_degree=None, harmonics_fn=None):
        super().__init__(nets, conditions)
        if harmonics_fn is None and max_degree is None:
            raise ValueError("harmonics_fn should be specified")
        if max_degree is not None:
            warnings.warn("`max_degree` is DEPRECATED; pass `harmonics_fn` instead, which takes precedence",
                          FutureWarning)
            from .function_basis import RealSphericalHarmonics
            self.harmonics_fn = RealSphericalHarmonics(max_degree=max_degree)
        if harmonics_fn is not None:
            self.harmonics_fn = harmonics_fn

    def _compute_u(self, net, condition, rs, thetas, phis):
        return torch.sum(condition.enforce(net, rs) * self.harmonics_fn(thetas, phis), dim=1)


class SolverSpherical(BaseSolver):

    def __init__(self, pde_system, conditions, r_min=None, r_max=None, nets=None, train_generator=None,
                 valid_generator=None, analytic_solutions=None, optimizer=None, loss_fn=None, n_batches_train=1,
                 n_batches_valid=4, metrics=None, enforcer=None, n_output_units=1, shuffle=None, batch_size=None):
        if (train_generator is None or valid_generator is None) and (r_min is None or r_max is None):
            raise ValueError(f"Either generator is not provided, r_min and r_max should be both provided: "
                             f"got r_min={r_min}, r_max={r_max}, train_generator={train_generator}, "
                             f"valid_generator={valid_generator}")
        if train_generator is None:
            train_generator = GeneratorSpherical(512, r_min, r_max, method="equally-spaced-noisy")
        if valid_generator is None:
            valid_generator = GeneratorSpherical(512, r_min, r_max, method="equally-spaced-noisy")
        self.r_min, self.r_max = r_min, r_max
        self.enforcer = enforcer
        super().__init__(diff_eqs=pde_system, conditions=conditions, nets=nets, train_generator=train_generator,
                         valid_generator=valid_generator, analytic_solutions=analytic_solutions, optimizer=optimizer,
                         loss_fn=loss_fn, n_batches_train=n_batches_train, n_batches_valid=n_batches_valid,
                         metrics=metrics, n_input_units=3, n_output_units=n_output_units, shuffle=shuffle,
                         batch_size=batch_size)

    def _auto_enforce(self, net, cond, *coordinates):
        if self.enforcer:
            return self.enforcer(net, cond, coordinates)
        fn = cond.parameterize if cond.__class__.enforce == BaseCondition.enforce else cond.enforce
        n_params = len(inspect.signature(fn).parameters)
        return cond.enforce(net, *coordinates[:n_params - 1])

    def compute_func_val(self, net, cond, *coordinates):
        return self._auto_enforce(net, cond, *coordinates)

    def get_solution(self, copy=True, best=True, harmonics_fn=None):
        nets = self.best_nets if best else self.nets
        conditions = self.conditions
        if copy:
            nets, conditions = deepcopy(nets), deepcopy(conditions)
        if harmonics_fn:
            return SolutionSphericalHarmonics(nets, conditions, harmonics_fn=harmonics_fn)
        return SolutionSpherical(nets, conditions)

    def _get_internal_variables(self):
        d = super()._get_internal_variables()
        d.update(r_min=self.r_min, r_max=self.r_max, enforcer=self.enforcer)
        return d


class GenericSolver(BaseSolver):
    def get_solution(self, copy=True, best=True):
        return self._solution(GenericSolution, copy, best)


class Solver1D(BaseSolver):

    def __init__(self, ode_system, conditions, t_min=None, t_max=None, nets=None, train_generator=None,
                 valid_generator=None, analytic_solutions=None, optimizer=None, loss_fn=None, n_batches_train=1,
                 n_batches_valid=4, metrics=None, n_output_units=1, batch_size=None, shuffle=None):
        if (train_generator is None or valid_generator is None) and (t_min is None or t_max is None):
            raise ValueError(f"Either generator is not provided, t_min and t_max should be both provided: \n"
                             f"got t_min={t_min}, t_max={t_max}, train_generator={train_generator}, "
                             f"valid_generator={valid_generator}")
        if train_generator is None:
            train_generator = Generator1D(32, t_min=t_min, t_max=t_max, method="equally-spaced-noisy")
        if valid_generator is None:
            valid_generator = Generator1D(32, t_min=t_min, t_max=t_max, method="equally-spaced")
        self.t_min, self.t_max = t_min, t_max
        super().__init__(diff_eqs=ode_system, conditions=conditions, nets=nets, train_generator=train_generator,
                         valid_generator=valid_generator, analytic_solutions=analytic_solutions, optimizer=optimizer,
                         loss_fn=loss_fn, n_batches_train=n_batches_train, n_batches_valid=n_batches_valid,
                         metrics=metrics, n_input_units=1, n_output_units=n_output_units, shuffle=shuffle,
                         batch_size=batch_size)

    def get_solution(self, copy=True, best=True):
        return self._solution(Solution1D, copy, best)

    def _get_internal_variables(self):
        d = super()._get_internal_variables()
        d.update(t_min=self.t_min, t_max=self.t_max)
        return d


class BundleSolution1D(GenericSolution):
    pass


class BundleSolver1D(BaseSolver):

    def __init__(self, ode_system, conditions, t_min=None, t_max=None, theta_min=None, theta_max=None,
                 eq_param_index=(), nets=None, train_generator=None, valid_generator=None, analytic_solutions=None,
                 optimizer=None, loss_fn=None, n_batches_train=1, n_batches_valid=4, metrics=None, n_output_units=1,
                 batch_size=None, shuffle=None):
        if (train_generator is None or valid_generator is None) and (t_min is None or t_max is None):
            raise ValueError(f"Either generator is not provided, t_min and t_max should be both provided: \n"
                             f"got t_min={t_min}, t_max={t_max}, train_generator={train_generator}, "
                             f"valid_generator={valid_generator}")
        theta_min = (theta_min,) if isinstance(theta_min, (float, int)) else tuple(theta_min or ())
        theta_max = (theta_max,) if isinstance(theta_max, (float, int)) else tuple(theta_max or ())
        if len(theta_min) != len(theta_max):
            raise ValueError(f"length of theta_min and theta_max must be equal, got {len(theta_min)} != {len(theta_max)}")
        r_min, r_max = (t_min,) + theta_min, (t_max,) + theta_max
        n_input_units = len(r_min)
        if train_generator is None:
            train_generator = Generator1D(32, t_min=t_min, t_max=t_max, method="equally-spaced-noisy")
            for lo, hi in zip(theta_min, theta_max):
                train_generator ^= Generator1D(32, t_min=lo, t_max=hi, method="equally-spaced-noisy")
        if valid_generator is None:
            valid_generator = Generator1D(32, t_min=t_min, t_max=t_max, method="equally-spaced")
            for lo, hi in zip(theta_min, theta_max):
                valid_generator ^= Generator1D(32, t_min=lo, t_max=hi, method="equally-spaced")
        self.r_min, self.r_max = r_min, r_max
        n_funcs, n_coords = len(conditions), 1
        picked = tuple(n_funcs + n_coords + idx for idx in eq_param_index)
        self.eq_param_index = picked

        def bundle_eqs(*variables):
            return ode_system(*variables[:n_funcs + n_coords], *(variables[i] for i in picked))

        super().__init__(diff_eqs=bundle_eqs, conditions=conditions, nets=nets, train_generator=train_generator,
                         valid_generator=valid_generator, analytic_solutions=analytic_solutions, optimizer=optimizer,
                         loss_fn=loss_fn, n_batches_train=n_batches_train, n_batches_valid=n_batches_valid,
                         metrics=metrics, n_input_units=n_input_units, n_output_units=n_output_units, shuffle=shuffle,
                         batch_size=batch_size)

    def get_solution(self, copy=True, best=True):
        return self._solution(BundleSolution1D, copy, best)

    def _get_internal_variables(self):
        d = super()._get_internal_variables()
        d.update(r_min=self.r_min, r_max=self.r_max, eq_param_index=self.eq_param_index)
        return d


class Solver2D(BaseSolver):

    def __init__(self, pde_system, conditions, xy_min=None, xy_max=None, nets=None, train_generator=None,
                 valid_generator=None, analytic_solutions=None, optimizer=None, loss_fn=None, n_batches_train=1,
                 n_batches_valid=4, metrics=None, n_output_units=1, batch_size=None, shuffle=None):
        if (train_generator is None or valid_generator is None) and (xy_min is None or xy_max is None):
            raise ValueError(f"Either generator is not provided, xy_min and xy_max should be both provided: \n"
                             f"got xy_min={xy_min}, xy_max={xy_max}, train_generator={train_generator}, "
                             f"valid_generator={valid_generator}")
        if train_generator is None:
            train_generator = Generator2D((32, 32), xy_min=xy_min, xy_max=xy_max, method="equally-spaced-noisy")
        if valid_generator is None:
            valid_generator = Generator2D((32, 32), xy_min=xy_min, xy_max=xy_max, method="equally-spaced")
        self.xy_min, self.xy_max = xy_min, xy_max
        super().__init__(diff_eqs=pde_system, conditions=conditions, nets=nets, train_generator=train_generator,
                         valid_generator=valid_generator, analytic_solutions=analytic_solutions, optimizer=optimizer,
                         loss_fn=loss_fn, n_batches_train=n_batches_train, n_batches_valid=n_batches_valid,
                         metrics=metrics, n_input_units=2, n_output_units=n_output_units, shuffle=shuffle,
                         batch_size=batch_size)

    def get_solution(self, copy=True, best=True):
        return self._solution(Solution2D, copy, best)

    def _get_internal_variables(self):
        d = super()._get_internal_variables()
        d.update(xy_min=self.xy_min, xy_max=self.xy_max)
        return d
```

Baseline: 3.277 billion collocation-points/s.

## Add persistent native epoch plan to cut per-epoch host dispatch overhead

Introduces an EpochPlan object that validates the fused-fit descriptor once and precomputes the tail kernel arguments and launch geometry. Each later epoch only patches the step, history and parity counters before launching the forward/backward and reduce-tail kernels. On the Python side, run_train_epoch routes single-network training through a cached plan keyed on parameter pointers and optimizer settings, and caches the resident batch pointers. The aim is to remove the repeated ctypes struct refresh, argument validation and batch upload work from each step. The cost is extra cache-invalidation logic that could go stale if the state changes in a way the key does not capture.

```diff
diff --git a/include/ndq.h b/include/ndq.h
--- a/include/ndq.h
+++ b/include/ndq.h
@@ -214,6 +214,12 @@
 int ndq_fused_fit_run(const ndq_fused_fit* f, int n_epochs, const float* const* train_coords, int adam_step,
                       int hist_index, int valid_index, int parity, void* stream);
 
+int ndq_epoch_plan_create(const ndq_fused_fit* f, void* stream, void** plan);
+int ndq_epoch_plan_run(void* plan, const float* train_coords);
+int ndq_epoch_plan_set_counters(void* plan, int adam_step, int hist_index, int parity);
+int ndq_epoch_plan_get_counters(const void* plan, int* adam_step, int* hist_index, int* parity);
+int ndq_epoch_plan_destroy(void* plan);
+
 typedef int (*ndq_pointwise_fn)(const float* coords, int ldc, int n, const float* const* jets,
                                 float* const* gbar, int ldj, float* funcs, float* resid, float* loss_partials,
                                 float seed_scale, void* stream);
diff --git a/neurodiffeq_amd/_build.py b/neurodiffeq_amd/_build.py
--- a/neurodiffeq_amd/_build.py
+++ b/neurodiffeq_amd/_build.py
@@ -6,7 +6,7 @@
 CSRC = os.path.join(HERE, "csrc")
 LIB = os.path.join(HERE, "libndq.so")
 SOURCES = [os.path.join(CSRC, "ndq_api.hip")]
-HEADERS = [os.path.join(CSRC, h) for h in ("ndq_mlp.h", "ndq_tail.h", "ndq_launch.h", "ndq_wide.h", "ndq_deep.h", "ndq_sample.h", "ndq_oneshot.h")] + \
+HEADERS = [os.path.join(CSRC, h) for h in ("ndq_mlp.h", "ndq_tail.h", "ndq_launch.h", "ndq_wide.h", "ndq_deep.h", "ndq_sample.h", "ndq_oneshot.h", "ndq_epoch_plan.h")] + \
     [os.path.join(HERE, "..", "include", "ndq.h"), os.path.join(HERE, "_hipcc.py")]
 LIB64 = os.path.join(HERE, "libndq64.so")
 SOURCES64 = [os.path.join(CSRC, "ndq_api64.hip")]
diff --git a/neurodiffeq_amd/_lib.py b/neurodiffeq_amd/_lib.py
--- a/neurodiffeq_amd/_lib.py
+++ b/neurodiffeq_amd/_lib.py
@@ -140,6 +140,11 @@
     L.ndq_fused_step_run.argtypes = [ctypes.POINTER(FusedStep), vp, ci, ci, ci, vp]
     L.ndq_fused_multi_step_run.argtypes = [ctypes.POINTER(FusedStep), ci, vp, vp, ci, ci, ci, vp]
     L.ndq_fused_fit_run.argtypes = [ctypes.POINTER(FusedFit), ci, vp, ci, ci, ci, ci, vp]
+    L.ndq_epoch_plan_create.argtypes = [ctypes.POINTER(FusedFit), vp, ctypes.POINTER(vp)]
+    L.ndq_epoch_plan_run.argtypes = [vp, vp]
+    L.ndq_epoch_plan_set_counters.argtypes = [vp, ci, ci, ci]
+    L.ndq_epoch_plan_get_counters.argtypes = [vp, ctypes.POINTER(ci), ctypes.POINTER(ci), ctypes.POINTER(ci)]
+    L.ndq_epoch_plan_destroy.argtypes = [vp]
     L.ndq_mlp_register.argtypes = [vp]
     L.ndq_sample.argtypes = [ctypes.POINTER(SamplerDesc), ctypes.c_ulonglong, ctypes.c_ulonglong, ctypes.c_uint, vp, ci, vp]
     L.ndq_sample_table.argtypes = [ctypes.POINTER(TableSamplerDesc), ctypes.c_ulonglong, ctypes.c_ulonglong, ctypes.c_uint, vp, ci,
@@ -152,12 +157,7 @@
     L.ndq_oneshot_allreduce.argtypes = [vp, vp, ctypes.c_size_t, ci, ci, vp, vp]
     L.ndq_oneshot_status.argtypes = [vp]
     L.ndq_oneshot_destroy.argtypes = [vp]
-    for name in ("ndq_mlp_supported", "ndq_mlp_num_streams", "ndq_mlp_num_params", "ndq_mlp_bwd_blocks",
-                 "ndq_mlp_jet_fwd", "ndq_mlp_jet_bwd", "ndq_reduce_partials", "ndq_adam_step", "ndq_reduce_grad_loss",
-                 "ndq_epoch_tail", "ndq_fused_step_run", "ndq_sample", "ndq_sample_table", "ndq_sample_plan", "ndq_sample_plan_indexed", "ndq_mlp_register",
-                 "ndq_fused_multi_step_run", "ndq_fused_fit_run", "ndq_oneshot_create", "ndq_oneshot_connect",
-                 "ndq_oneshot_allreduce", "ndq_oneshot_status",
-                 "ndq_oneshot_destroy"):
+    for name in EXPORTS:
         getattr(L, name).restype = ci
     _LIB = L
     return L
@@ -207,7 +207,8 @@
            "ndq_mlp_jet_bwd", "ndq_reduce_partials", "ndq_adam_step", "ndq_reduce_grad_loss", "ndq_epoch_tail",
            "ndq_fused_step_run", "ndq_sample", "ndq_sample_table", "ndq_sample_plan", "ndq_sample_plan_indexed", "ndq_mlp_register",
            "ndq_fused_multi_step_run", "ndq_fused_fit_run", "ndq_oneshot_create", "ndq_oneshot_connect", "ndq_oneshot_allreduce", "ndq_oneshot_status",
-           "ndq_oneshot_destroy")
+           "ndq_oneshot_destroy", "ndq_epoch_plan_create", "ndq_epoch_plan_run", "ndq_epoch_plan_set_counters",
+           "ndq_epoch_plan_get_counters", "ndq_epoch_plan_destroy")
 
 
 def check(rc, what):
diff --git a/neurodiffeq_amd/csrc/ndq_api.hip b/neurodiffeq_amd/csrc/ndq_api.hip
--- a/neurodiffeq_amd/csrc/ndq_api.hip
+++ b/neurodiffeq_amd/csrc/ndq_api.hip
@@ -4,6 +4,7 @@
 #include "ndq_sample.h"
 #include "ndq_oneshot.h"
 #include "ndq_tail.h"
+#include "ndq_epoch_plan.h"
 
 extern "C" int ndq_oneshot_allreduce(const void* send, void* recv, size_t count, int dtype, int op, void* comm, void* stream);
 
@@ -89,10 +90,6 @@
   out[i] = accumulate ? out[i] + s : s;
 }
 
-struct Reduce2Args {
-  const float* part; int nparts, len; float* out; int accumulate;
-  const float* lpart; int nlparts; float* lout; float lscale;
-};
 
 struct ColumnRows {
   float v[16];
@@ -171,22 +168,7 @@
   }
 }
 
-using TailArgs = ndq::TailArgsT<float>;
-
-struct ValidArgs {
-  const float* part; int nparts; float scale; float* hist; int index;
-  int best_on_valid;
-};
-struct ReduceTailArgs {
-  Reduce2Args r;
-  TailArgs t;
-  int tail_blocks;
-  ndq::SampleArgs smp;
-  ValidArgs v;
-};
-#ifndef NDQ_TAIL_COLS
-#define NDQ_TAIL_COLS 64
-#endif
+
 template <int TC>
 __device__ __forceinline__ void reduce_tail_body(const ReduceTailArgs& a) {
   constexpr int TT = TC * 16, WAVES = TT / 64;
@@ -347,24 +329,23 @@
   }
 }
 
-struct ReduceTailMultiArgs {
-  ReduceTailArgs net[4];
-};
 template <int TC>
 __global__ __launch_bounds__(TC * 16) void reduce_tail_multi_kernel(ReduceTailMultiArgs a) {
   const ReduceTailArgs& mine = a.net[blockIdx.y];
   if ((int)blockIdx.x * TC >= mine.r.len) return;
   reduce_tail_body<TC>(mine);
 }
+static int launch_tail_multi_at(const ReduceTailMultiArgs& a, const TailGeometry& g, void* stream) {
+  hipStream_t st = static_cast<hipStream_t>(stream);
+  if (g.cols == NDQ_TAIL_COLS)
+    hipLaunchKernelGGL(reduce_tail_multi_kernel<NDQ_TAIL_COLS>, dim3(g.grid_x, g.grid_y), dim3(g.threads), 0, st, a);
+  else
+    hipLaunchKernelGGL(reduce_tail_multi_kernel<64>, dim3(g.grid_x, g.grid_y), dim3(g.threads), 0, st, a);
+  return (int)hipGetLastError();
+}
 static int launch_tail_multi(ReduceTailMultiArgs& a, int max_params, int n_nets, int max_lparts, void* stream) {
-  hipStream_t st = static_cast<hipStream_t>(stream);
   for (int k = n_nets; k < 4; ++k) a.net[k] = a.net[0];
-  if (NDQ_TAIL_COLS < 64 && max_lparts <= NDQ_TAIL_COLS * 16)
-    hipLaunchKernelGGL(reduce_tail_multi_kernel<NDQ_TAIL_COLS>, dim3((max_params + NDQ_TAIL_COLS - 1) / NDQ_TAIL_COLS, n_nets),
-                       dim3(NDQ_TAIL_COLS * 16), 0, st, a);
-  else
-    hipLaunchKernelGGL(reduce_tail_multi_kernel<64>, dim3((max_params + 63) / 64, n_nets), dim3(1024), 0, st, a);
-  return (int)hipGetLastError();
+  return launch_tail_multi_at(a, tail_multi_geometry(max_params, n_nets, max_lparts), stream);
 }
 
 }
@@ -451,21 +432,6 @@
 
 }
 
-static ReduceTailArgs reduce_tail_args(const ndq_fused_step& s, const ndq_fused_step& s0, const float* part, const float* lpart,
-                                       int nparts, int adam_step, int hist_index, int parity, int write_scalars,
-                                       float* best_flat, const ValidArgs& v = ValidArgs{}, const float* p_in = nullptr,
-                                       const float* m_in = nullptr, const float* v_in = nullptr) {
-  ReduceTailArgs a{};
-  a.r = Reduce2Args{part, nparts, s.n_params, s.grad, 0, lpart, nparts, s.loss_slot, s0.seed};
-  a.t.p = s.params; a.t.g = s.grad; a.t.m = s.adam_m; a.t.v = s.adam_v; a.t.len = s.n_params;
-  a.t.adam = adam_consts(s.lr, s.beta1, s.beta2, s.eps, s.weight_decay, adam_step);
-  a.t.p_in = p_in; a.t.m_in = m_in; a.t.v_in = v_in;
-  a.t.loss_slots = s.loss_slot; a.t.nb = 1; a.t.loss_hist = s0.loss_hist; a.t.hist_index = hist_index;
-  a.t.best_loss = s0.best_loss; a.t.parity = parity; a.t.best_flat = best_flat; a.t.write_scalars = write_scalars;
-  a.tail_blocks = 0x7fffffff;
-  a.v = v;
-  return a;
-}
 
 extern "C" {
 
@@ -543,55 +509,10 @@
 
 }
 
-struct FitCall {
-  const ndq_fused_fit* f;
-  int n_epochs; const float* const* train_coords;
-  int adam_step, hist_index, valid_index;
-  void* stream;
-  bool valid;
-  int max_params, max_lparts;
-  float* P[2][4]; float* M[2][4]; float* V[2][4]; float* PART[2][4]; float* LP[2]; float* VP[2];
-};
-
-static bool fit_tracks(const ndq_fused_fit* f, bool with_train, bool with_valid) {
-  return (f->track_best == 1 && with_train) || (f->track_best == 2 && with_valid);
-}
-
 static int fit_tail(const FitCall& c, int set, bool with_train, bool with_valid, int adam_step, int hist_index, int vindex,
                     int parity) {
-  const ndq_fused_fit* f = c.f;
-  const ndq_fused_step& s0 = f->net[0];
-  ValidArgs v{};
-  if (with_valid) v = ValidArgs{c.VP[set], f->valid_blocks, f->valid_scale, f->valid_hist, vindex, f->track_best == 2 ? 1 : 0};
-  const bool track = fit_tracks(f, with_train, with_valid);
-  ReduceTailMultiArgs a{};
-  for (int k = 0; k < f->n_nets; ++k) {
-    const ndq_fused_step& s = f->net[k];
-    a.net[k] = reduce_tail_args(s, s0, c.PART[set][k], c.LP[set], with_train ? s0.blocks : 0, with_train ? adam_step : 0,
-                                hist_index, parity, k == 0 ? 1 : 0, track ? s.best_flat : nullptr, v,
-                                set ? c.P[set][k] : nullptr, set ? c.M[set][k] : nullptr, set ? c.V[set][k] : nullptr);
-  }
-  return launch_tail_multi(a, c.max_params, f->n_nets, c.max_lparts, c.stream);
-}
-
-static int fit_two_launch(const FitCall& c, int parity) {
-  const ndq_fused_fit* f = c.f;
-  const ndq_fused_step& s0 = f->net[0];
-  for (int e = 0; e < c.n_epochs; ++e, parity ^= 1) {
-    if (!c.train_coords[e]) return NDQ_EINVAL;
-    const bool with_valid = c.valid && e > 0;
-    int rc = f->launch(c.train_coords[e], s0.ldc, s0.n, c.P[0], c.PART[0], c.LP[0], s0.seed,
-                       with_valid ? f->valid_coords : nullptr, f->valid_ldc, with_valid ? f->valid_n : 0, c.VP[0], nullptr,
-                       c.stream);
-    if (rc) return rc;
-    rc = fit_tail(c, 0, true, with_valid, c.adam_step + e, c.hist_index + e, c.valid_index + e - 1, parity);
-    if (rc) return rc;
-  }
-  if (!c.valid) return 0;
-  int rc = f->launch(nullptr, 0, 0, c.P[0], nullptr, nullptr, 0.f, f->valid_coords, f->valid_ldc, f->valid_n, c.VP[0], nullptr,
-                     c.stream);
-  if (rc) return rc;
-  return fit_tail(c, 0, false, true, 0, c.hist_index + c.n_epochs, c.valid_index + (c.n_epochs > 0 ? c.n_epochs - 1 : 0), parity);
+  return launch_tail_multi_at(fit_tail_args(c, set, with_train, with_valid, adam_step, hist_index, vindex, parity),
+                              tail_multi_geometry(c.max_params, c.f->n_nets, c.max_lparts), c.stream);
 }
 
 struct Finishes { int adam_step, hist_index, valid_index; bool with_valid; };
@@ -680,31 +601,12 @@
 
 int ndq_fused_fit_run(const ndq_fused_fit* f, int n_epochs, const float* const* train_coords, int adam_step,
                       int hist_index, int valid_index, int parity, void* stream) {
-  if (!f || !f->launch || f->n_nets < 1 || f->n_nets > 4 || n_epochs < 0 || (n_epochs > 0 && (!train_coords || adam_step <= 0)) ||
-      hist_index < 0 || valid_index < 0 || (parity != 0 && parity != 1) || f->track_best < 0 || f->track_best > 2)
-    return NDQ_EINVAL;
+  FitCall c;
+  bool pull = false;
+  if (int rc = fit_call_init(c, pull, f, n_epochs, train_coords, adam_step, hist_index, valid_index, parity, stream)) return rc;
   const ndq_fused_step& s0 = f->net[0];
-  const bool valid = f->valid_coords != nullptr;
-  if (!valid && n_epochs == 0) return NDQ_EINVAL;
-  if (!s0.best_loss || (n_epochs > 0 && (!s0.loss_hist || !s0.loss_partials || s0.n <= 0 || s0.blocks <= 0))) return NDQ_EINVAL;
-  if (valid && (!f->valid_loss_partials || !f->valid_hist || f->valid_n <= 0 || f->valid_blocks <= 0)) return NDQ_EINVAL;
-  if (f->track_best == 2 && !valid) return NDQ_EINVAL;
-  FitCall c{f, n_epochs, train_coords, adam_step, hist_index, valid_index, stream, valid};
-  c.max_lparts = s0.blocks > f->valid_blocks ? s0.blocks : f->valid_blocks;
-  c.LP[0] = s0.loss_partials; c.LP[1] = f->alt_loss_partials;
-  c.VP[0] = f->valid_loss_partials; c.VP[1] = f->alt_valid_loss_partials;
-  bool pull = f->pull_ok != 0 && n_epochs >= 2 && s0.blocks * f->n_nets <= ndq::kPullMaxWork && f->alt_loss_partials &&
-              (!valid || f->alt_valid_loss_partials);
-  for (int k = 0; k < f->n_nets; ++k) {
-    const ndq_fused_step& s = f->net[k];
-    if (!s.params || s.n_params <= 0 || (f->track_best && !s.best_flat)) return NDQ_EINVAL;
-    if (n_epochs > 0 && (!s.partials || !s.grad || !s.adam_m || !s.adam_v || !s.loss_slot)) return NDQ_EINVAL;
-    if (s.n_params > c.max_params) c.max_params = s.n_params;
-    c.P[0][k] = s.params; c.M[0][k] = s.adam_m; c.V[0][k] = s.adam_v; c.PART[0][k] = s.partials;
-    c.P[1][k] = f->alt_params[k]; c.M[1][k] = f->alt_m[k]; c.V[1][k] = f->alt_v[k]; c.PART[1][k] = f->alt_partials[k];
-    pull = pull && c.P[1][k] && c.M[1][k] && c.V[1][k] && c.PART[1][k];
-  }
-  if (!pull) return fit_two_launch(c, parity);
+  const bool valid = c.valid;
+  if (!pull) return fit_two_launch(c, parity, launch_tail_multi_at);
   bool loop = f->loop_ok != 0 && f->launch_loop && s0.blocks == 1 && (!valid || f->valid_blocks == 1) &&
               f->n_nets <= ndq::kLoopMaxNets;
   long long stride = 0;
@@ -717,6 +619,41 @@
     }
   }
   return loop ? fit_loop(c, stride, parity) : fit_pull(c, parity);
+}
+
+int ndq_epoch_plan_create(const ndq_fused_fit* f, void* stream, void** plan) {
+  if (!plan) return NDQ_EINVAL;
+  *plan = nullptr;
+  EpochPlan* p = new (std::nothrow) EpochPlan();
+  if (!p) return (int)hipErrorOutOfMemory;
+  if (int rc = epoch_plan_init(*p, f, stream)) {
+    delete p;
+    return rc;
+  }
+  *plan = p;
+  return 0;
+}
+
+int ndq_epoch_plan_run(void* plan, const float* train_coords) {
+  if (!plan) return NDQ_EINVAL;
+  return epoch_plan_run(*static_cast<EpochPlan*>(plan), train_coords, launch_tail_multi_at);
+}
+
+int ndq_epoch_plan_set_counters(void* plan, int adam_step, int hist_index, int parity) {
+  if (!plan) return NDQ_EINVAL;
+  return epoch_plan_set_counters(*static_cast<EpochPlan*>(plan), adam_step, hist_index, parity);
+}
+
+int ndq_epoch_plan_get_counters(const void* plan, int* adam_step, int* hist_index, int* parity) {
+  if (!plan || !adam_step || !hist_index || !parity) return NDQ_EINVAL;
+  const EpochPlan* p = static_cast<const EpochPlan*>(plan);
+  *adam_step = p->adam_step; *hist_index = p->hist_index; *parity = p->parity;
+  return 0;
+}
+
+int ndq_epoch_plan_destroy(void* plan) {
+  delete static_cast<EpochPlan*>(plan);
+  return 0;
 }
 
 int ndq_adam_step(float* params, const float* grad, float* exp_avg, float* exp_avg_sq, int len, float lr, float beta1,
diff --git a/neurodiffeq_amd/csrc/ndq_epoch_plan.h b/neurodiffeq_amd/csrc/ndq_epoch_plan.h
--- /dev/null
+++ b/neurodiffeq_amd/csrc/ndq_epoch_plan.h
@@ -0,0 +1,194 @@
+#pragma once
+#include "../../include/ndq.h"
+#include "ndq_sample.h"
+#include "ndq_tail.h"
+
+namespace ndq {
+
+struct Reduce2Args {
+  const float* part; int nparts, len; float* out; int accumulate;
+  const float* lpart; int nlparts; float* lout; float lscale;
+};
+
+using TailArgs = ndq::TailArgsT<float>;
+
+struct ValidArgs {
+  const float* part; int nparts; float scale; float* hist; int index;
+  int best_on_valid;
+};
+struct ReduceTailArgs {
+  Reduce2Args r;
+  TailArgs t;
+  int tail_blocks;
+  ndq::SampleArgs smp;
+  ValidArgs v;
+};
+struct ReduceTailMultiArgs {
+  ReduceTailArgs net[4];
+};
+
+#ifndef NDQ_TAIL_COLS
+#define NDQ_TAIL_COLS 64
+#endif
+struct TailGeometry {
+  int cols;
+  unsigned grid_x, grid_y, threads;
+};
+inline TailGeometry tail_multi_geometry(int max_params, int n_nets, int max_lparts) {
+  const int cols = (NDQ_TAIL_COLS < 64 && max_lparts <= NDQ_TAIL_COLS * 16) ? NDQ_TAIL_COLS : 64;
+  return {cols, (unsigned)((max_params + cols - 1) / cols), (unsigned)n_nets, (unsigned)(cols * 16)};
+}
+
+inline ReduceTailArgs reduce_tail_args(const ndq_fused_step& s, const ndq_fused_step& s0, const float* part, const float* lpart,
+                                       int nparts, int adam_step, int hist_index, int parity, int write_scalars,
+                                       float* best_flat, const ValidArgs& v = ValidArgs{}, const float* p_in = nullptr,
+                                       const float* m_in = nullptr, const float* v_in = nullptr) {
+  ReduceTailArgs a{};
+  a.r = Reduce2Args{part, nparts, s.n_params, s.grad, 0, lpart, nparts, s.loss_slot, s0.seed};
+  a.t.p = s.params; a.t.g = s.grad; a.t.m = s.adam_m; a.t.v = s.adam_v; a.t.len = s.n_params;
+  a.t.adam = adam_consts(s.lr, s.beta1, s.beta2, s.eps, s.weight_decay, adam_step);
+  a.t.p_in = p_in; a.t.m_in = m_in; a.t.v_in = v_in;
+  a.t.loss_slots = s.loss_slot; a.t.nb = 1; a.t.loss_hist = s0.loss_hist; a.t.hist_index = hist_index;
+  a.t.best_loss = s0.best_loss; a.t.parity = parity; a.t.best_flat = best_flat; a.t.write_scalars = write_scalars;
+  a.tail_blocks = 0x7fffffff;
+  a.v = v;
+  return a;
+}
+inline void reduce_tail_set_epoch(ReduceTailArgs& a, const ndq_fused_step& s, int adam_step, int hist_index, int parity) {
+  a.t.adam = adam_consts(s.lr, s.beta1, s.beta2, s.eps, s.weight_decay, adam_step);
+  a.t.hist_index = hist_index;
+  a.t.parity = parity;
+}
+
+struct FitCall {
+  const ndq_fused_fit* f;
+  int n_epochs; const float* const* train_coords;
+  int adam_step, hist_index, valid_index;
+  void* stream;
+  bool valid;
+  int max_params, max_lparts;
+  float* P[2][4]; float* M[2][4]; float* V[2][4]; float* PART[2][4]; float* LP[2]; float* VP[2];
+};
+
+inline int fit_call_init(FitCall& c, bool& pull, const ndq_fused_fit* f, int n_epochs, const float* const* train_coords,
+                         int adam_step, int hist_index, int valid_index, int parity, void* stream) {
+  if (!f || !f->launch || f->n_nets < 1 || f->n_nets > 4 || n_epochs < 0 || (n_epochs > 0 && (!train_coords || adam_step <= 0)) ||
+      hist_index < 0 || valid_index < 0 || (parity != 0 && parity != 1) || f->track_best < 0 || f->track_best > 2)
+    return NDQ_EINVAL;
+  const ndq_fused_step& s0 = f->net[0];
+  const bool valid = f->valid_coords != nullptr;
+  if (!valid && n_epochs == 0) return NDQ_EINVAL;
+  if (!s0.best_loss || (n_epochs > 0 && (!s0.loss_hist || !s0.loss_partials || s0.n <= 0 || s0.blocks <= 0))) return NDQ_EINVAL;
+  if (valid && (!f->valid_loss_partials || !f->valid_hist || f->valid_n <= 0 || f->valid_blocks <= 0)) return NDQ_EINVAL;
+  if (f->track_best == 2 && !valid) return NDQ_EINVAL;
+  c = FitCall{f, n_epochs, train_coords, adam_step, hist_index, valid_index, stream, valid};
+  c.max_lparts = s0.blocks > f->valid_blocks ? s0.blocks : f->valid_blocks;
+  c.LP[0] = s0.loss_partials; c.LP[1] = f->alt_loss_partials;
+  c.VP[0] = f->valid_loss_partials; c.VP[1] = f->alt_valid_loss_partials;
+  pull = f->pull_ok != 0 && n_epochs >= 2 && s0.blocks * f->n_nets <= ndq::kPullMaxWork && f->alt_loss_partials &&
+         (!valid || f->alt_valid_loss_partials);
+  for (int k = 0; k < f->n_nets; ++k) {
+    const ndq_fused_step& s = f->net[k];
+    if (!s.params || s.n_params <= 0 || (f->track_best && !s.best_flat)) return NDQ_EINVAL;
+    if (n_epochs > 0 && (!s.partials || !s.grad || !s.adam_m || !s.adam_v || !s.loss_slot)) return NDQ_EINVAL;
+    if (s.n_params > c.max_params) c.max_params = s.n_params;
+    c.P[0][k] = s.params; c.M[0][k] = s.adam_m; c.V[0][k] = s.adam_v; c.PART[0][k] = s.partials;
+    c.P[1][k] = f->alt_params[k]; c.M[1][k] = f->alt_m[k]; c.V[1][k] = f->alt_v[k]; c.PART[1][k] = f->alt_partials[k];
+    pull = pull && c.P[1][k] && c.M[1][k] && c.V[1][k] && c.PART[1][k];
+  }
+  return 0;
+}
+
+inline bool fit_tracks(const ndq_fused_fit* f, bool with_train, bool with_valid) {
+  return (f->track_best == 1 && with_train) || (f->track_best == 2 && with_valid);
+}
+
+inline ReduceTailMultiArgs fit_tail_args(const FitCall& c, int set, bool with_train, bool with_valid, int adam_step,
+                                         int hist_index, int vindex, int parity) {
+  const ndq_fused_fit* f = c.f;
+  const ndq_fused_step& s0 = f->net[0];
+  ValidArgs v{};
+  if (with_valid) v = ValidArgs{c.VP[set], f->valid_blocks, f->valid_scale, f->valid_hist, vindex, f->track_best == 2 ? 1 : 0};
+  const bool track = fit_tracks(f, with_train, with_valid);
+  ReduceTailMultiArgs a{};
+  for (int k = 0; k < f->n_nets; ++k) {
+    const ndq_fused_step& s = f->net[k];
+    a.net[k] = reduce_tail_args(s, s0, c.PART[set][k], c.LP[set], with_train ? s0.blocks : 0, with_train ? adam_step : 0,
+                                hist_index, parity, k == 0 ? 1 : 0, track ? s.best_flat : nullptr, v,
+                                set ? c.P[set][k] : nullptr, set ? c.M[set][k] : nullptr, set ? c.V[set][k] : nullptr);
+  }
+  for (int k = f->n_nets; k < 4; ++k) a.net[k] = a.net[0];
+  return a;
+}
+
+template <class Tail>
+int fit_two_launch(const FitCall& c, int parity, Tail&& tail) {
+  const ndq_fused_fit* f = c.f;
+  const ndq_fused_step& s0 = f->net[0];
+  const TailGeometry g = tail_multi_geometry(c.max_params, f->n_nets, c.max_lparts);
+  for (int e = 0; e < c.n_epochs; ++e, parity ^= 1) {
+    if (!c.train_coords[e]) return NDQ_EINVAL;
+    const bool with_valid = c.valid && e > 0;
+    int rc = f->launch(c.train_coords[e], s0.ldc, s0.n, c.P[0], c.PART[0], c.LP[0], s0.seed,
+                       with_valid ? f->valid_coords : nullptr, f->valid_ldc, with_valid ? f->valid_n : 0, c.VP[0], nullptr,
+                       c.stream);
+    if (rc) return rc;
+    rc = tail(fit_tail_args(c, 0, true, with_valid, c.adam_step + e, c.hist_index + e, c.valid_index + e - 1, parity), g, c.stream);
+    if (rc) return rc;
+  }
+  if (!c.valid) return 0;
+  int rc = f->launch(nullptr, 0, 0, c.P[0], nullptr, nullptr, 0.f, f->valid_coords, f->valid_ldc, f->valid_n, c.VP[0], nullptr,
+                     c.stream);
+  if (rc) return rc;
+  return tail(fit_tail_args(c, 0, false, true, 0, c.hist_index + c.n_epochs, c.valid_index + (c.n_epochs > 0 ? c.n_epochs - 1 : 0), parity),
+              g, c.stream);
+}
+
+struct EpochPlan {
+  ndq_fused_fit f;
+  FitCall c;
+  const float* coords[1];
+  int adam_step, hist_index, parity;
+  ReduceTailMultiArgs tail;
+  TailGeometry geometry;
+  EpochPlan() = default;
+  EpochPlan(const EpochPlan&) = delete;
+  EpochPlan& operator=(const EpochPlan&) = delete;
+};
+
+inline int epoch_plan_init(EpochPlan& p, const ndq_fused_fit* f, void* stream) {
+  if (!f || f->valid_coords) return NDQ_EINVAL;
+  p.f = *f;
+  p.coords[0] = nullptr;
+  p.adam_step = 1; p.hist_index = 0; p.parity = 0;
+  bool pull = false;
+  int rc = fit_call_init(p.c, pull, &p.f, 1, p.coords, p.adam_step, p.hist_index, 0, p.parity, stream);
+  if (rc) return rc;
+  p.tail = fit_tail_args(p.c, 0, true, false, p.adam_step, p.hist_index, -1, p.parity);
+  p.geometry = tail_multi_geometry(p.c.max_params, p.f.n_nets, p.c.max_lparts);
+  return 0;
+}
+
+inline int epoch_plan_set_counters(EpochPlan& p, int adam_step, int hist_index, int parity) {
+  if (adam_step <= 0 || hist_index < 0 || (parity != 0 && parity != 1)) return NDQ_EINVAL;
+  p.adam_step = adam_step; p.hist_index = hist_index; p.parity = parity;
+  return 0;
+}
+
+template <class Tail>
+int epoch_plan_run(EpochPlan& p, const float* train_coords, Tail&& tail) {
+  if (!train_coords) return NDQ_EINVAL;
+  const ndq_fused_step& s0 = p.f.net[0];
+  p.coords[0] = train_coords;
+  for (int k = 0; k < p.f.n_nets; ++k) reduce_tail_set_epoch(p.tail.net[k], p.f.net[k], p.adam_step, p.hist_index, p.parity);
+  for (int k = p.f.n_nets; k < 4; ++k) reduce_tail_set_epoch(p.tail.net[k], p.f.net[0], p.adam_step, p.hist_index, p.parity);
+  int rc = p.f.launch(train_coords, s0.ldc, s0.n, p.c.P[0], p.c.PART[0], p.c.LP[0], s0.seed, nullptr, p.f.valid_ldc, 0, p.c.VP[0],
+                      nullptr, p.c.stream);
+  if (rc) return rc;
+  rc = tail(p.tail, p.geometry, p.c.stream);
+  if (rc) return rc;
+  ++p.adam_step; ++p.hist_index; p.parity ^= 1;
+  return 0;
+}
+
+}
diff --git a/neurodiffeq_amd/engine.py b/neurodiffeq_amd/engine.py
--- a/neurodiffeq_amd/engine.py
+++ b/neurodiffeq_amd/engine.py
@@ -291,6 +291,21 @@
 def f64_fused_tail_switch(environ=None):
     environ = os.environ if environ is None else environ
     return environ.get("NDQ_F64_FUSED_TAIL", "0") == "1"
+
+
+class _EpochPlan:
+
+    def __init__(self, L, ent, stream, now):
+        self.L, self.ent, self.now, self.counters, self.batches = L, ent, now, None, {}
+        self.run = L.ndq_epoch_plan_run
+        handle = ctypes.c_void_p()
+        _lib.check(L.ndq_epoch_plan_create(ent[5], _c_vp(stream), ctypes.byref(handle)), "ndq_epoch_plan_create")
+        self.handle = handle
+
+    def __del__(self):
+        handle, self.handle = getattr(self, "handle", None), None
+        if handle:
+            self.L.ndq_epoch_plan_destroy(handle)
 
 
 class FusedSystem:
@@ -1074,6 +1089,24 @@
     def fit_run(self, train_ptrs, n, ld, adam_slots, valid=None, track_best=0, n_global=None):
         fs = self.fast_state()
         K = len(train_ptrs)
+        ent = self._fit_entry(K, n, ld, valid)
+        step0 = self._fit_refresh(ent, K, n, adam_slots, valid, track_best, n_global)
+        if K == 1:
+            coords = ent[4]
+            coords[0] = train_ptrs[0]
+        else:
+            coords = (_c_vp * max(K, 1))(*train_ptrs) if K else None
+        rc = self.L.ndq_fused_fit_run(ent[5], K, coords, step0, fs["pending"], fs["pending_valid"], fs["parity"],
+                                      self._stream())
+        _lib.check(rc, "ndq_fused_fit_run")
+        tails = K + (1 if valid is not None else 0)
+        fs["pending"] += K
+        if valid is not None:
+            fs["pending_valid"] += max(K, 1)
+        fs["parity"] ^= tails & 1
+
+    def _fit_entry(self, K, n, ld, valid):
+        fs = self.fast_state()
         if K:
             self._fit_last_n = n
         fk = self.fused_variant(n if K else (getattr(self, "_fit_last_n", None) or valid[1]))
@@ -1123,6 +1156,9 @@
                     ff.launch_loop = ctypes.cast(fk.lib.ndq_fused_launch_loop, ctypes.c_void_p).value
                     ff.loop_ok = 1
             ent = cache[key] = (ff, keep, fk, {}, (_c_vp * 1)(), ctypes.byref(ff))
+        return ent
+
+    def _fit_refresh(self, ent, K, n, adam_slots, valid, track_best, n_global=None):
         ff = ent[0]
         step0 = 1
         last = ent[3]
@@ -1146,19 +1182,51 @@
             last["v"] = (vc, track_best)
             ff.valid_coords = vc
             ff.track_best = track_best
-        if K == 1:
-            coords = ent[4]
-            coords[0] = train_ptrs[0]
+        return step0
+
+    EPOCH_PLAN = os.environ.get("NDQ_EPOCH_PLAN", "1") != "0"
+
+    def plan_ready(self):
+        return self.EPOCH_PLAN and len(self.flat) == 1 and self.fit_ready()
+
+    def plan_epoch(self, batch, adam_slot, track_best):
+        fs = self.fast_state()
+        pl = fs.get("plan")
+        hit = pl.batches.get(id(batch)) if pl is not None else None
+        if hit is not None and hit[0] is batch:
+            _, ptr, n, ld = hit
+            resident = None
         else:
-            coords = (_c_vp * max(K, 1))(*train_ptrs) if K else None
-        rc = self.L.ndq_fused_fit_run(ent[5], K, coords, step0, fs["pending"], fs["pending_valid"], fs["parity"],
-                                      self._stream())
-        _lib.check(rc, "ndq_fused_fit_run")
-        tails = K + (1 if valid is not None else 0)
-        fs["pending"] += K
-        if valid is not None:
-            fs["pending_valid"] += max(K, 1)
-        fs["parity"] ^= tails & 1
+            b, n = self.upload(batch)
+            ptr, ld = self._coord_ptr(b, 0).value, b["ld"]
+            res = self._resident_cache.get(id(batch))
+            resident = res is not None and res[0] is batch
+        self._fit_last_n = n
+        fp = self.flat[0]
+        fp.sync()
+        m, v, group, step = adam_slot
+        stream = _raw_stream(self._dev_index)
+        now = (fp.flat.data_ptr(), n, m.data_ptr(), v.data_ptr(), group["lr"], group["betas"], group["eps"], group["weight_decay"],
+               ld, track_best, stream)
+        if pl is None or pl.now != now:
+            ent = self._fit_entry(1, n, ld, None)
+            self._fit_refresh(ent, 1, n, [adam_slot], None, track_best)
+            fs["plan"] = None
+            pl = fs["plan"] = _EpochPlan(self.L, ent, stream, now)
+        if resident:
+            if len(pl.batches) >= 64:
+                pl.batches.clear()
+            pl.batches[id(batch)] = (batch, ptr, n, ld)
+        ctr = (step, fs["pending"], fs["parity"])
+        if pl.counters != ctr:
+            _lib.check(self.L.ndq_epoch_plan_set_counters(pl.handle, *ctr), "ndq_epoch_plan_set_counters")
+        rc = pl.run(pl.handle, ptr)
+        if rc:
+            pl.counters = None
+            _lib.check(rc, "ndq_epoch_plan_run")
+        pl.counters = (step + 1, ctr[1] + 1, ctr[2] ^ 1)
+        fs["pending"] = ctr[1] + 1
+        fs["parity"] = ctr[2] ^ 1
 
     def fast_flush(self):
         fs = getattr(self, "_fast", None)
diff --git a/neurodiffeq_amd/solvers.py b/neurodiffeq_amd/solvers.py
--- a/neurodiffeq_amd/solvers.py
+++ b/neurodiffeq_amd/solvers.py
@@ -700,6 +700,9 @@
         n_all = batch[0].shape[0]
         if system.needs_check(n_all):
             return False
+        if train and system.plan_ready():
+            system.plan_epoch(batch, slots[0], 1 if self.n_batches["valid"] == 0 else 0)
+            return True
         b, n = system.upload(batch)
         ptr = system._coord_ptr(b, 0).value
         if train:
```

New measurement: 3.310 billion collocation-points/s, median of 2. No clear change (+1.0%).
